# wzx99/DCFP

Measured on AMD Instinct MI355X. Metric: training images/sec at 1024x2048 DeepLabv3-R101, higher is better.
Workload: dtype f32; 1 GPU; DeepLabv3-resnet101+ASPP os8, 4x3x1024x2048 per GPU, CE+0.4*deepsup CE (fused upsample), 3x3 stride-1 convs with >= 256 channels as fp32 Winograd F(2x2,3x3) (fwd / dgrad / wgrad), all other convs direct implicit GEMM, EIC step, SGD m0.9 wd5e-4; global_batch=4, parallelism=dp1

## Files before the change

### dcfp_amd/_lib.py

```python
import ctypes as C
import os
import subprocess
import threading

_HERE = os.path.dirname(os.path.abspath(__file__))
LIB_PATH = os.environ.get("DCFP_LIB") or os.path.join(_HERE, "libdcfp_hip.so")
CSRC = os.path.join(_HERE, "csrc")

_lib = None
_lock = threading.Lock()


class ConvDesc(C.Structure):
    _fields_ = [(n, C.c_int32) for n in
                ("N", "Cin", "H", "W", "Cout", "KH", "KW", "stride", "pad", "dil", "Hout", "Wout",
                 "x_pitch", "dy_pitch")]


class ConvF16Desc(C.Structure):
    _fields_ = [(n, C.c_int32) for n in
                ("N", "H", "W", "Cin8", "x_pitch", "Cout", "K", "stride", "pad", "dil", "Hout", "Wout",
                 "y_pitch", "y_off", "res_pitch", "res_off", "relu")]


class EicEntry(C.Structure):
    _fields_ = [("gamma", C.c_void_p), ("grad", C.c_void_p), ("eic", C.c_void_p),
                ("n", C.c_int32), ("pad_", C.c_int32)]


class SgdEntry(C.Structure):
    _fields_ = [("param", C.c_void_p), ("grad", C.c_void_p), ("momentum_buf", C.c_void_p),
                ("n", C.c_int64), ("first_chunk", C.c_int64),
                ("weight_decay", C.c_float), ("pad_", C.c_int32)]


class BnRunning(C.Structure):
    _fields_ = [("running_mean", C.c_void_p), ("running_var", C.c_void_p), ("num_batches_tracked", C.c_void_p),
                ("momentum", C.c_float), ("pad_", C.c_int32)]


class WpEntry(C.Structure):
    _fields_ = [("w", C.c_void_p), ("wp", C.c_void_p), ("first_block", C.c_int64), ("n_blocks", C.c_int64)] + \
               [(n, C.c_int32) for n in ("T", "Ck", "CkP", "M", "Mpad", "sAm", "sAc", "perm8")]


class AugTap(C.Structure):
    _fields_ = [(n, C.c_int32) for n in ("src", "c0", "c1", "lsrc")]


class AugSample(C.Structure):
    _fields_ = [("image", C.c_void_p), ("label", C.c_void_p)] + \
               [(n, C.c_int32) for n in ("src_h", "src_w", "col_off", "row_off", "lut_a_off", "lut_b_off",
                                         "hsv_flags", "hue_delta")] + \
               [("sat_alpha", C.c_float), ("pad_", C.c_int32)]


class CcSample(C.Structure):
    _fields_ = [("label", C.c_void_p)] + \
               [(n, C.c_int32) for n in ("src_h", "src_w", "dst_h", "dst_w", "Hp", "Wp", "row_off", "col_off", "cls",
                                         "pad_")] + \
               [("work_off", C.c_int64)]


AUG_SATURATION, AUG_HUE = 1, 2
SGD_CHUNK = 16384
CONV_FWD, CONV_DGRAD, CONV_WGRAD = 0, 1, 2
E_BADDESC, E_UNSUPPORTED, E_WORKSPACE = -1, -2, -3

_P, _I, _L, _F, _Z = C.c_void_p, C.c_int, C.c_int64, C.c_float, C.c_size_t
_D = C.POINTER(ConvDesc)
_R = C.POINTER(BnRunning)
_H = C.POINTER(ConvF16Desc)

SIGNATURES = {
    "dcfp_abi_version": (_I, []),
    "dcfp_conv2d_workspace_bytes": (_Z, [_D, _I]),
    "dcfp_conv2d_wp_layout": (_I, [_D, _I, C.POINTER(WpEntry)]),
    "dcfp_conv2d_permute_weights_multi_f32": (_I, [_P, _I, _L, _P]),
    "dcfp_conv2d_pitch_supported": (_I, [_D]),
    "dcfp_conv2d_kernel_name": (_I, [_D, _I, C.c_char_p, _I]),
    "dcfp_conv2d_executed_fraction": (C.c_double, [_D, _I]),
    "dcfp_conv2d_workspace_is_scratch": (_I, [_D, _I]),
    "dcfp_conv2d_dgrad_fanin_supported": (_I, [_D]),
    "dcfp_conv2d_dgrad_fanin_f32_nchw": (_I, [_D, _P, _L, _P, _P, _P, _P, _P, _Z, _I, _P]),
    "dcfp_conv2d_dgrad_fanin_red_slots": (_L, [_D]),
    "dcfp_conv2d_dgrad_fanin_red_f32_nchw": (_I, [_D, _P, _L, _P, _P, _P, _P, _P, _P, _P, _P, _P, _Z, _I, _P]),
    "dcfp_bn_bwd_sums_from_partials_f32": (_I, [_P, _L, _I, _P, _F, _P, _P, _P, _P, _P]),
    "dcfp_conv2d_xform_bytes": (_Z, [_D]),
    "dcfp_conv2d_fwd_keep_f32_nchw": (_I, [_D, _P, _P, _P, _L, _P, _Z, _P, _P, _Z, _P]),
    "dcfp_conv2d_wgrad_kept_f32_nchw": (_I, [_D, _P, _L, _P, _Z, _P, _P, _Z, _P]),
    "dcfp_conv2d_fwd_f32_nchw": (_I, [_D, _P, _P, _P, _P, _L, _P, _Z, _I, _P]),
    "dcfp_conv2d_fwd_fused_f32_nchw": (_I, [_D, _P, _P, _P, _P, _P, _I, _P, _P, _Z, _I, _P]),
    "dcfp_conv2d_dgrad_f32_nchw": (_I, [_D, _P, _L, _P, _P, _I, _P, _Z, _I, _P]),
    "dcfp_conv2d_wgrad_f32_nchw": (_I, [_D, _P, _L, _P, _P, _P, _P, _Z, _P]),
    "dcfp_bn_workspace_bytes": (_Z, [_I, _I, _I]),
    "dcfp_bn_stats_f32": (_I, [_P, _L, _I, _I, _I, _P, _P, _R, _P, _Z, _P]),
    "dcfp_bn_apply_f32": (_I, [_P, _P, _P, _P, _P, _F, _P, _I, _P, _L, _I, _I, _I, _I, _I, _P]),
    "dcfp_bn_bwd_reduce_f32": (_I, [_P, _L, _P, _P, _L, _P, _P, _P, _P, _F, _I, _I, _I, _I, _P, _P, _P, _P,
                                    _P, _Z, _P]),
    "dcfp_bn_update_running_f32": (_I, [_P, _P, _I, _F, _F, _P, _P, _P, _P]),
    "dcfp_syncbn_combine_f32": (_I, [_P, _I, _I, _P, _P, _P, _R, _P]),
    "dcfp_syncbn_p2p_mailbox_bytes": (_Z, [_I, _I]),
    "dcfp_p2p_alloc": (_I, [_Z, _I, C.POINTER(C.c_void_p)]),
    "dcfp_p2p_free": (_I, [_P]),
    "dcfp_p2p_export": (_I, [_P, _P]),
    "dcfp_p2p_import": (_I, [_P, C.POINTER(C.c_void_p)]),
    "dcfp_p2p_unmap": (_I, [_P]),
    "dcfp_syncbn_p2p_exchange_f32": (_I, [C.POINTER(C.c_void_p), _I, _I, C.c_uint32, _I, _P, _I, _I, _P, _R,
                                          C.c_uint32, _P, _P]),
    "dcfp_bn_apply_relu_mask_f32": (_I, [_P, _P, _P, _P, _P, _F, _P, _P, _P, _I, _I, _I, _P]),
    "dcfp_conv2d_fwd_stat_slots": (_L, [_D, _P, _L]),
    "dcfp_conv2d_fwd_stats_f32_nchw": (_I, [_D, _P, _P, _P, _L, _P, _P, _Z, _I, _P]),
    "dcfp_bn_stats_from_partials_f32": (_I, [_P, _L, _I, _I, _P, _P, _R, _P]),
    "dcfp_bn_bwd_apply_f32": (_I, [_P, _L, _P, _P, _L, _P, _P, _P, _P, _F, _P, _P, _F, _P, _I, _P, _P,
                                   _I, _I, _I, _I, _I, _P]),
    "dcfp_bn_bwd_fused_sync_bytes": (_Z, [_I, _I, _I]),
    "dcfp_bn_bwd_fused_f32": (_I, [_P, _L, _P, _P, _L, _P, _P, _P, _P, _F, _F, _I, _P, _P, _I, _I, _I, _I, _I,
                                   _P, _P, _P, _P, _P, _Z, C.c_uint32, C.c_uint32, _P, _P]),
    "dcfp_maxpool3x3s2_fwd_f32": (_I, [_P, _P, _P, _I, _I, _I, _I, _I, _I, _P]),
    "dcfp_maxpool3x3s2_bwd_f32": (_I, [_P, _P, _P, _I, _I, _I, _I, _I, _I, _P]),
    "dcfp_rowsum_f32": (_I, [_P, _L, _P, _F, _I, _I, _I, _P]),
    "dcfp_broadcast_hw_f32": (_I, [_P, _F, _P, _L, _I, _I, _I, _I, _P]),
    "dcfp_add_f32": (_I, [_P, _P, _P, _L, _P]),
    "dcfp_channel_scale_f32": (_I, [_P, _P, _P, _I, _I, _I, _P]),
    "dcfp_upsample_bilinear_fwd_f32": (_I, [_P, _P, _I, _I, _I, _I, _I, _I, _I, _P]),
    "dcfp_upsample_bilinear_bwd_f32": (_I, [_P, _P, _I, _I, _I, _I, _I, _I, _I, _P]),
    "dcfp_resize_bilinear_into_f32": (_I, [_P, _L, _I, _I, _I, _I, _P, _L, _I, _I, _I, _I, _P]),
    "dcfp_resize_bilinear_adjoint_f32": (_I, [_P, _L, _I, _I, _I, _I, _I, _P, _L, _I, _I, _I, _I, _P]),
    "dcfp_ppm_pool_f32": (_I, [_P, _I, _I, _I, _I, _I, _P, _P, _I, _P, _L, _I, _P]),
    "dcfp_ppm_pool_adjoint_f32": (_I, [_P, _I, _I, _I, _I, _I, _P, _P, _L, _I, _P, _P]),
    "dcfp_ppm_resize_adjoint_f32": (_I, [_P, _L, _I, _I, _I, _I, _I, _P, _P, _I, _P]),
    "dcfp_upsample_ce_workspace_bytes": (_Z, [_I, _I, _I]),
    "dcfp_upsample_ce_fwd_f32": (_I, [_P, _P, _P, _I, _I, _I, _I, _I, _I, _I, _I, _P, _P, _P, _P,
                                      _Z, _P]),
    "dcfp_upsample_ce_bwd_f32": (_I, [_P, _P, _P, _I, _I, _I, _I, _I, _I, _I, _I, _P, _P, _P, _P]),
    "dcfp_ohem_zoom_gt_prob_f32": (_I, [_P, _P, _P, _I, _I, _I, _I, _I, _I, _I, _I, _I, _P, _P, _P]),
    "dcfp_ohem_threshold_f32": (_I, [_P, _P, _L, _I, _F, _L, _P, _P]),
    "dcfp_ohem_keep_mask_u8": (_I, [_P, _P, _L, _P, _P]),
    "dcfp_upsample_margin_f32": (_I, [_P, _I, _I, _I, _I, _I, _I, _I, _P, _P]),
    "dcfp_maxfilter2d_s1_f32": (_I, [_P, _P, _I, _I, _I, _I, _P]),
    "dcfp_upsample_wce_workspace_bytes": (_Z, [_I, _I, _I]),
    "dcfp_upsample_wce_fwd_f32": (_I, [_P, _P, _P, _I, _I, _I, _I, _I, _I, _I, _I, _P, _P, _P, _Z, _P]),
    "dcfp_upsample_wce_bwd_f32": (_I, [_P, _P, _P, _I, _I, _I, _I, _I, _I, _I, _I, _P, _P, _P, _P]),
    "dcfp_upsample_argmax_f32": (_I, [_P, _I, _I, _I, _I, _I, _I, _I, _P, _P]),
    "dcfp_confusion_matrix_i64": (_I, [_P, _P, _I, _L, _I, _P, _P]),
    "dcfp_label_boundary_workspace_bytes": (_Z, [_I, _I, _I]),
    "dcfp_label_boundary_i32": (_I, [_P, _P, _I, _I, _I, _I, _I, _I, _P, _Z, _P]),
    "dcfp_label_boundary_i64": (_I, [_P, _P, _I, _I, _I, _I, _I, _I, _P, _Z, _P]),
    "dcfp_augment_u8_to_f32_nchw": (_I, [C.POINTER(AugSample), _I, _I, _I, _P, _L, _P, _L, _P, _L, _P, _I, _P, _P, _P, _P]),
    "dcfp_balance_weight_f32": (_I, [_P, _P, _P, _I, _L, _I, _I, _I, C.c_double, _P, _P]),
    "dcfp_components_workspace_bytes": (_Z, [_I, _I]),
    "dcfp_label_components_u8": (_I, [C.POINTER(CcSample), _I, _P, _L, _P, _P, _Z, _P, _P]),
    "dcfp_component_pixel_i32": (_I, [C.POINTER(CcSample), _I, _P, _Z, _P, _P, _P, _P, _P]),
    "dcfp_eic_update_f32": (_I, [_P, _I, _F, _F, _P]),
    "dcfp_sgd_momentum_f32": (_I, [_P, _I, _L, _F, _F, _I, _P]),
    "dcfp_conv2d_fwd_f16_nhwc": (_I, [_H, _P, _P, _P, _P, _P, _P]),
    "dcfp_conv2d_fwd_f16_nhwc_to_f32_nchw": (_I, [_H, _P, _P, _P, _P, _P]),
    "dcfp_maxpool3x3s2_nhwc_f16": (_I, [_P, _P, _I, _I, _I, _I, _I, _I, _I, _I, _P]),
    "dcfp_avgpool_nhwc_f16_workspace_bytes": (_Z, [_I, _I, _L]),
    "dcfp_avgpool_nhwc_f16": (_I, [_P, _P, _I, _L, _I, _I, _I, _P, _Z, _P]),
    "dcfp_broadcast_nhwc_f16": (_I, [_P, _I, _P, _I, _L, _I, _I, _I, _P]),
    "dcfp_nchw_f32_to_nhwc_f16": (_I, [_P, _P, _I, _I, _I, _I, _I, _P]),
    "dcfp_resize_bilinear_nhwc_f16": (_I, [_P, _I, _I, _I, _I, _I, _P, _I, _I, _I, _I, _I, _P]),
    "dcfp_pyramid_pool_nhwc_f16_workspace_bytes": (_Z, [_I, _I, _I, _I, _I, _P]),
    "dcfp_pyramid_pool_nhwc_f16": (_I, [_P, _I, _I, _I, _I, _I, _I, _I, _P, _P, _P, _P, _Z, _P]),
}


def build(verbose=False):
    cmd = ["make", "-C", CSRC, "-j", str(min(8, os.cpu_count() or 1))]
    r = subprocess.run(cmd, capture_output=True, text=True)
    if verbose or r.returncode != 0:
        print(r.stdout[-4000:])
        print(r.stderr[-4000:])
    if r.returncode != 0:
        raise RuntimeError("building libdcfp_hip.so failed")
    return LIB_PATH


def lib():
    global _lib
    if _lib is not None:
        return _lib
    with _lock:
        if _lib is not None:
            return _lib
        if not os.path.exists(LIB_PATH):
            raise RuntimeError(
                f"{LIB_PATH} not found: run `python -c 'import __graft_entry__ as g; g.build()'` "
                "(or `make -C dcfp_amd/csrc`). dcfp_amd has no non-HIP fallback.")
        try:
            import torch
        except Exception:
            pass
        handle = C.CDLL(LIB_PATH, mode=C.RTLD_GLOBAL)
        for name, (res, args) in SIGNATURES.items():
            fn = getattr(handle, name)
            fn.restype = res
            fn.argtypes = args
        _lib = handle
    return _lib


def check(status, what):
    if status != 0:
        kind = "descriptor/shape" if status < 0 else "hipError_t"
        raise RuntimeError(f"{what} failed: status {status} ({kind})")
```

### dcfp_amd/csrc/bn.hip

```cpp
#include "common.h"
#include <stdlib.h>

namespace {

constexpr int kThreads = 256;

__device__ __forceinline__ float bn_val(float v, float mu, float istd, float g, float b) {
    return fmaf((v - mu) * istd, g, b);
}

struct BnPlan {
    int chunks;
    int chunk_elems;
};

constexpr int kChunkElems = 8192;

BnPlan bn_plan(int N, int C, int HW) {
    const long long E = (long long)N * HW;
    long long chunks = (E + kChunkElems - 1) / kChunkElems;
    if (E <= kChunkElems) {
        const long long by_size = (E + 2047) / 2048;
        long long by_grid = 4096 / (C > 0 ? C : 1);
        if (by_grid < 1) by_grid = 1;
        chunks = by_size < by_grid ? by_size : by_grid;
    }
    if (chunks < 1) chunks = 1;
    long long ce = (E + chunks - 1) / chunks;
    ce = (ce + 1023) / 1024 * 1024;
    chunks = (E + ce - 1) / ce;
    if (chunks < 1) chunks = 1;
    BnPlan p;
    p.chunks = (int)chunks;
    p.chunk_elems = (int)ce;
    return p;
}

__device__ __forceinline__ void bwd_accumulate(const float4& g, const float4& xv, float mu, float& s1, float& s2) {
#pragma clang fp contract(off)
    s1 += (g.x + g.y) + (g.z + g.w);
    const float a = fmaf(g.x, xv.x - mu, g.y * (xv.y - mu));
    const float b = fmaf(g.z, xv.z - mu, g.w * (xv.w - mu));
    s2 += a + b;
}
__device__ __forceinline__ float bwd_dx(float g, float xv, float mu, float mean_dy, float k, float gi) {
#pragma clang fp contract(off)
    return fmaf(-(xv - mu), k, g - mean_dy) * gi;
}

template <bool VEC>
__global__ void __launch_bounds__(kThreads)
bn_stats_partial_kernel(const float* __restrict__ x, long long nstride, int HW, long long E,
                        int chunk_elems, int chunks, float* __restrict__ part) {
    __shared__ float red[4];
    const int c = blockIdx.y, chunk = blockIdx.x;
    const float* xc = x + (long long)c * HW;
    const float K = xc[0];
    const long long e0 = (long long)chunk * chunk_elems;
    long long e1 = e0 + chunk_elems;
    if (e1 > E) e1 = E;
    float s1 = 0.f, s2 = 0.f;
    if (VEC) {
        for (long long e = e0 + 4 * threadIdx.x; e < e1; e += 4 * kThreads) {
            const long long n = e / HW;
            const int i = (int)(e - n * HW);
            const float4 v = *reinterpret_cast<const float4*>(xc + n * nstride + i);
            const float a = v.x - K, b = v.y - K, cc = v.z - K, d = v.w - K;
            s1 += (a + b) + (cc + d);
            s2 += (a * a + b * b) + (cc * cc + d * d);
        }
    } else {
        for (long long e = e0 + threadIdx.x; e < e1; e += kThreads) {
            const long long n = e / HW;
            const int i = (int)(e - n * HW);
            const float a = xc[n * nstride + i] - K;
            s1 += a;
            s2 += a * a;
        }
    }
    const float t1 = block_sum_256(s1, red);
    const float t2 = block_sum_256(s2, red);
    if (threadIdx.x == 0) {
        part[((long long)c * chunks + chunk) * 2 + 0] = t1;
        part[((long long)c * chunks + chunk) * 2 + 1] = t2;
    }
}

__global__ void bn_stats_final_kernel(const float* __restrict__ x, int HW, long long E, int C,
                                      int chunks, const float* __restrict__ part,
                                      float* __restrict__ mean, float* __restrict__ var, DcfpBnRunning run) {
    const int c = blockIdx.x * blockDim.x + threadIdx.x;
    if (c >= C) return;
    double S1 = 0.0, S2 = 0.0;
    for (int k = 0; k < chunks; ++k) {
        S1 += (double)part[((long long)c * chunks + k) * 2 + 0];
        S2 += (double)part[((long long)c * chunks + k) * 2 + 1];
    }
    const double K = (double)x[(long long)c * HW];
    const double m1 = S1 / (double)E;
    double v = S2 / (double)E - m1 * m1;
    if (v < 0.0) v = 0.0;
    mean[c] = (float)(K + m1);
    var[c] = (float)v;
    running_update(run, c, (float)(K + m1), (float)v, (float)E);
}

__device__ __forceinline__ bool mask_bit(const unsigned long long* __restrict__ row_words, int i_wave, int k) {
    const unsigned long long wv = row_words[(i_wave >> 8) * 4 + k];
    return (wv >> (threadIdx.x & 63)) & 1ull;
}

template <bool VEC, bool MASK = false>
__global__ void __launch_bounds__(kThreads)
bn_apply_kernel(const float* __restrict__ x, const float* __restrict__ mean,
                const float* __restrict__ var, const float* __restrict__ gamma,
                const float* __restrict__ beta, float eps, const float* __restrict__ res,
                int relu, float* __restrict__ y, long long y_nstride, int C, int HW,
                int colchunks, int cols_per_block, unsigned long long* __restrict__ mask = nullptr,
                int W = 0, int y_pitch = 0) {
    const long long row = blockIdx.x / colchunks;
    const int chunk = blockIdx.x - (int)(row * colchunks);
    const int n = (int)(row / C), c = (int)(row - (long long)n * C);
    const float istd = 1.0f / sqrtf(var[c] + eps);
    const float mu = mean[c], g = gamma[c], b = beta[c];
    const float* xr = x + row * HW;
    const float* rr = res ? res + row * HW : nullptr;
    float* yr = y + (long long)n * y_nstride + (long long)c * (y_pitch ? (long long)(HW / W) * y_pitch : HW);
    const int i0 = chunk * cols_per_block;
    int i1 = i0 + cols_per_block;
    if (i1 > HW) i1 = HW;
    if (VEC) {
        for (int i = i0 + 4 * threadIdx.x; i < i1; i += 4 * kThreads) {
            const float4 v = *reinterpret_cast<const float4*>(xr + i);
            float4 o;
            o.x = bn_val(v.x, mu, istd, g, b);
            o.y = bn_val(v.y, mu, istd, g, b);
            o.z = bn_val(v.z, mu, istd, g, b);
            o.w = bn_val(v.w, mu, istd, g, b);
            if (rr) {
                const float4 r = *reinterpret_cast<const float4*>(rr + i);
                o.x += r.x; o.y += r.y; o.z += r.z; o.w += r.w;
            }
            if (relu) {
                o.x = o.x > 0.f ? o.x : 0.f; o.y = o.y > 0.f ? o.y : 0.f;
                o.z = o.z > 0.f ? o.z : 0.f; o.w = o.w > 0.f ? o.w : 0.f;
            }
            if constexpr (MASK) {
                const unsigned long long b0 = __ballot(o.x > 0.f), b1 = __ballot(o.y > 0.f);
                const unsigned long long b2 = __ballot(o.z > 0.f), b3 = __ballot(o.w > 0.f);
                if ((threadIdx.x & 63) == 0) {
                    unsigned long long* mw = mask + row * (HW >> 6) + (i >> 8) * 4;
                    mw[0] = b0; mw[1] = b1; mw[2] = b2; mw[3] = b3;
                }
            }
            if (y_pitch) { const int h = i / W; *reinterpret_cast<float4*>(yr + h * y_pitch + (i - h * W)) = o; }
            else *reinterpret_cast<float4*>(yr + i) = o;
        }
    } else {
        for (int i = i0 + threadIdx.x; i < i1; i += kThreads) {
            float o = bn_val(xr[i], mu, istd, g, b);
            if (rr) o += rr[i];
            if (relu) o = o > 0.f ? o : 0.f;
            if (y_pitch) { const int h = i / W; yr[h * y_pitch + (i - h * W)] = o; }
            else yr[i] = o;
        }
    }
}

template <bool VEC, int RELU>
__global__ void __launch_bounds__(kThreads)
bn_bwd_reduce_partial_kernel(const float* __restrict__ dy, long long dy_nstride,
                             const float* __restrict__ x, const float* __restrict__ y,
                             long long y_nstride, const float* __restrict__ mean,
                             const float* __restrict__ var, const float* __restrict__ gamma,
                             const float* __restrict__ beta, float eps, int C, int HW,
                             long long E, int chunk_elems, int chunks, float* __restrict__ part) {
    __shared__ float red[4];
    const int c = blockIdx.y, chunk = blockIdx.x;
    const float mu = mean[c];
    float istd = 0.f, gm = 0.f, bt = 0.f;
    if (RELU == 2) { istd = 1.0f / sqrtf(var[c] + eps); gm = gamma[c]; bt = beta[c]; }
    const long long e0 = (long long)chunk * chunk_elems;
    long long e1 = e0 + chunk_elems;
    if (e1 > E) e1 = E;
    const long long coff = (long long)c * HW;
    const long long x_nstride = (long long)C * HW;
    float s1 = 0.f, s2 = 0.f;
    if (VEC) {
        for (long long e = e0 + 4 * threadIdx.x; e < e1; e += 4 * kThreads) {
            const long long n = e / HW;
            const int i = (int)(e - n * HW);
            float4 g = *reinterpret_cast<const float4*>(dy + n * dy_nstride + coff + i);
            const float4 xv = *reinterpret_cast<const float4*>(x + n * x_nstride + coff + i);
            if (RELU == 1) {
                const float4 yv = *reinterpret_cast<const float4*>(y + n * y_nstride + coff + i);
                g.x = yv.x > 0.f ? g.x : 0.f; g.y = yv.y > 0.f ? g.y : 0.f;
                g.z = yv.z > 0.f ? g.z : 0.f; g.w = yv.w > 0.f ? g.w : 0.f;
            } else if (RELU == 2) {
                g.x = bn_val(xv.x, mu, istd, gm, bt) > 0.f ? g.x : 0.f;
                g.y = bn_val(xv.y, mu, istd, gm, bt) > 0.f ? g.y : 0.f;
                g.z = bn_val(xv.z, mu, istd, gm, bt) > 0.f ? g.z : 0.f;
                g.w = bn_val(xv.w, mu, istd, gm, bt) > 0.f ? g.w : 0.f;
            } else if (RELU == 3) {
                const unsigned long long* mw = reinterpret_cast<const unsigned long long*>(y) +
                                               (n * C + c) * (long long)(HW >> 6);
                const int iw = i - 4 * (int)(threadIdx.x & 63);
                g.x = mask_bit(mw, iw, 0) ? g.x : 0.f; g.y = mask_bit(mw, iw, 1) ? g.y : 0.f;
                g.z = mask_bit(mw, iw, 2) ? g.z : 0.f; g.w = mask_bit(mw, iw, 3) ? g.w : 0.f;
            }
            bwd_accumulate(g, xv, mu, s1, s2);
        }
    } else {
        for (long long e = e0 + threadIdx.x; e < e1; e += kThreads) {
            const long long n = e / HW;
            const int i = (int)(e - n * HW);
            float g = dy[n * dy_nstride + coff + i];
            const float xv = x[n * x_nstride + coff + i];
            if (RELU == 1) g = y[n * y_nstride + coff + i] > 0.f ? g : 0.f;
            else if (RELU == 2) g = bn_val(xv, mu, istd, gm, bt) > 0.f ? g : 0.f;
            s1 += g;
            s2 += g * (xv - mu);
        }
    }
    const float t1 = block_sum_256(s1, red);
    const float t2 = block_sum_256(s2, red);
    if (threadIdx.x == 0) {
        part[((long long)c * chunks + chunk) * 2 + 0] = t1;
        part[((long long)c * chunks + chunk) * 2 + 1] = t2;
    }
}

template <class F>
__device__ __forceinline__ double wave_pair_totals(int n2, int lane, F value_of) {
    double acc = 0.0;
    for (int j = 0; lane + 64 * j < n2; ++j) acc += (double)value_of(j);
#pragma unroll
    for (int off = 2; off < 64; off <<= 1) acc += __shfl_xor(acc, off, 64);
    return acc;
}

__global__ void __launch_bounds__(64) bn_pair_final_kernel(int C, int chunks, const float* __restrict__ part,
                                     float* __restrict__ o1, float* __restrict__ o2,
                                     const float* __restrict__ var, float eps, float* __restrict__ o3,
                                     float* __restrict__ o4) {
    const int c = blockIdx.x, lane = threadIdx.x;
    const float* pc = part + (long long)c * chunks * 2;
    const double t = wave_pair_totals(2 * chunks, lane, [&](int j) { return pc[lane + 64 * j]; });
    const double S1 = __shfl(t, 0, 64), S2 = __shfl(t, 1, 64);
    if (lane == 0) {
        o1[c] = (float)S1;
        o2[c] = (float)S2;
        if (o3) o3[c] = (float)S2 * rsqrtf(var[c] + eps);
        if (o4) o4[c] = (float)S1;
    }
}

__global__ void syncbn_combine_kernel(const float* __restrict__ allv, int world, int C,
                                      float* __restrict__ gmean, float* __restrict__ gvar,
                                      float* __restrict__ total, DcfpBnRunning run) {
#pragma clang fp contract(off)
    const int c = blockIdx.x * blockDim.x + threadIdx.x;
    if (c >= C) return;
    const int S = 2 * C + 1;
    double tot = 0.0, m = 0.0, v = 0.0;
    for (int r = 0; r < world; ++r) {
        const double n = (double)allv[(long long)r * S + 2 * C];
        tot = __dadd_rn(tot, n);
        m = __dadd_rn(m, __dmul_rn((double)allv[(long long)r * S + c], n));
    }
    m /= tot;
    for (int r = 0; r < world; ++r) {
        const double n = (double)allv[(long long)r * S + 2 * C];
        const double d = __dadd_rn((double)allv[(long long)r * S + c], -m);
        v = __dadd_rn(v, __dmul_rn(__dadd_rn((double)allv[(long long)r * S + C + c], __dmul_rn(d, d)), n));
    }
    gmean[c] = (float)m;
    gvar[c] = (float)(v / tot);
    if (c == 0) total[0] = (float)tot;
    running_update(run, c, (float)m, (float)(v / tot), (float)tot);
}

constexpr int kSfpThreads = 1024;
template <int kSfpCh>
__global__ void __launch_bounds__(kSfpThreads)
bn_stats_from_partials_kernel(const float* __restrict__ part, long long S, int cnt, int C,
                              float* __restrict__ mean, float* __restrict__ var, DcfpBnRunning run) {
    constexpr int kSfpGroups = kSfpThreads / kSfpCh;
    __shared__ double red[kSfpGroups][kSfpCh];
    __shared__ double mu_s[kSfpCh];
    const int l = threadIdx.x % kSfpCh, g = threadIdx.x / kSfpCh;
    const int c = blockIdx.x * kSfpCh + l;
    const bool on = c < C;
    const float2* p2 = reinterpret_cast<const float2*>(part);
    constexpr int U = 4;
    double a[U] = {0.0, 0.0, 0.0, 0.0};
    if (on) {
        long long s = g;
        for (; s + (U - 1) * kSfpGroups < S; s += U * kSfpGroups) {
            float v[U];
#pragma unroll
            for (int u = 0; u < U; ++u) v[u] = p2[(s + u * kSfpGroups) * C + c].x;
#pragma unroll
            for (int u = 0; u < U; ++u) a[u] += (double)v[u];
        }
        for (; s < S; s += kSfpGroups) a[0] += (double)p2[s * C + c].x;
    }
    red[g][l] = (a[0] + a[1]) + (a[2] + a[3]);
    __syncthreads();
    if (g == 0) {
        double t = 0.0;
#pragma unroll
        for (int k = 0; k < kSfpGroups; ++k) t += red[k][l];
        mu_s[l] = t / (double)S;
    }
    __syncthreads();
    const double mu = mu_s[l];
    double b[U] = {0.0, 0.0, 0.0, 0.0};
    if (on) {
        long long s = g;
// ... 307 lines not shown
}

template <int RELU, bool DRES, bool PITCH>
__global__ void __launch_bounds__(kThreads, 5) bn_bwd_fusedu_kernel(const BnFusedParams p) {
    __shared__ float red[4];
    __shared__ float tot[2];
    __shared__ int failed;
    __shared__ float parts[2 * kFusedMaxChunks];
    const int c = blockIdx.x / p.chunks, chunk = blockIdx.x - c * p.chunks;
    const int HW = p.HW, C = p.C;
    const float mu = p.mean[c];
    const float istd = 1.0f / sqrtf(p.var[c] + p.eps);
    const float gm = p.gamma[c];
    const float bt = RELU == 2 ? p.beta[c] : 0.f;
    const int e0 = chunk * kChunkElems;
    const int n = e0 / HW, i0 = e0 - n * HW;
    const long long row = (long long)n * C + c;
    const float* dyb = p.dy + (long long)n * p.dy_nstride + (long long)c * HW + i0;
    const float* xb = p.x + row * HW + i0;
    const unsigned lo = 4u * threadIdx.x;
    if (threadIdx.x == 0) failed = 0;

    float4 g[kFusedIters], xv[kFusedIters];
#pragma unroll
    for (int k = 0; k < kFusedIters; ++k) {
        g[k] = *reinterpret_cast<const float4*>(dyb + 4 * kThreads * k + lo);
        xv[k] = *reinterpret_cast<const float4*>(xb + 4 * kThreads * k + lo);
    }
    float s1 = 0.f, s2 = 0.f;
#pragma unroll
    for (int k = 0; k < kFusedIters; ++k) {
        if (RELU == 1) {
            const float4 yv = *reinterpret_cast<const float4*>(p.y + (long long)n * p.y_nstride + (long long)c * HW + i0 +
                                                               4 * kThreads * k + lo);
            g[k].x = yv.x > 0.f ? g[k].x : 0.f; g[k].y = yv.y > 0.f ? g[k].y : 0.f;
            g[k].z = yv.z > 0.f ? g[k].z : 0.f; g[k].w = yv.w > 0.f ? g[k].w : 0.f;
        } else if (RELU == 2) {
            g[k].x = bn_val(xv[k].x, mu, istd, gm, bt) > 0.f ? g[k].x : 0.f;
            g[k].y = bn_val(xv[k].y, mu, istd, gm, bt) > 0.f ? g[k].y : 0.f;
            g[k].z = bn_val(xv[k].z, mu, istd, gm, bt) > 0.f ? g[k].z : 0.f;
            g[k].w = bn_val(xv[k].w, mu, istd, gm, bt) > 0.f ? g[k].w : 0.f;
        } else if (RELU == 3) {
            const unsigned long long* mw = reinterpret_cast<const unsigned long long*>(p.y) + row * (long long)(HW >> 6) +
                                           ((i0 + 4 * kThreads * k + 256 * (int)(threadIdx.x >> 6)) >> 8) * 4;
            const int sh = (int)(threadIdx.x & 63);
            g[k].x = ((mw[0] >> sh) & 1ull) ? g[k].x : 0.f; g[k].y = ((mw[1] >> sh) & 1ull) ? g[k].y : 0.f;
            g[k].z = ((mw[2] >> sh) & 1ull) ? g[k].z : 0.f; g[k].w = ((mw[3] >> sh) & 1ull) ? g[k].w : 0.f;
        }
        bwd_accumulate(g[k], xv[k], mu, s1, s2);
    }
    const float t1 = block_sum_256(s1, red);
    const float t2 = block_sum_256(s2, red);
    bn_fused_handoff(p, c, chunk, t1, t2, tot, &failed, parts);
    const bool bad = failed != 0;
    const float S1f = tot[0], S2f = tot[1];
    const float nanv = __uint_as_float(0x7fc00000u);
    if (chunk == 0 && threadIdx.x == 0) {
        p.sum_dy[c] = bad ? nanv : S1f;
        p.sum_dy_xmu[c] = bad ? nanv : S2f;
        if (p.dgamma) p.dgamma[c] = bad ? nanv : S2f * rsqrtf(p.var[c] + p.eps);
        if (p.dbeta) p.dbeta[c] = bad ? nanv : S1f;
    }
    const float mean_dy = S1f * p.inv_count;
    const float kk = S2f * p.inv_count * istd * istd;
    const float gi = bad ? nanv : gm * istd;
    float* dxb = p.dx + row * (PITCH ? (long long)(HW / p.W) * p.dx_pitch : (long long)HW) + (PITCH ? 0 : i0);
    float* drb = DRES ? p.dres + row * HW + i0 : nullptr;
#pragma unroll
    for (int k = 0; k < kFusedIters; ++k) {
        float4 o;
        o.x = bwd_dx(g[k].x, xv[k].x, mu, mean_dy, kk, gi);
        o.y = bwd_dx(g[k].y, xv[k].y, mu, mean_dy, kk, gi);
        o.z = bwd_dx(g[k].z, xv[k].z, mu, mean_dy, kk, gi);
        o.w = bwd_dx(g[k].w, xv[k].w, mu, mean_dy, kk, gi);
        if (PITCH) {
            const int i = i0 + 4 * kThreads * k + (int)lo;
            const int h = i / p.W;
            *reinterpret_cast<float4*>(dxb + h * p.dx_pitch + (i - h * p.W)) = o;
        } else {
            *reinterpret_cast<float4*>(dxb + 4 * kThreads * k + lo) = o;
        }
        if (DRES) *reinterpret_cast<float4*>(drb + 4 * kThreads * k + lo) = g[k];
    }
}

static const int kColsPerBlock = [] { const char* e = getenv("DCFP_BN_COLS"); const int v = e ? atoi(e) : 2048; return v >= 1024 && v % 1024 == 0 ? v : 2048; }();

}

extern "C" size_t dcfp_bn_workspace_bytes(int N, int C, int HW) {
    if (N <= 0 || C <= 0 || HW <= 0) return 0;
    const BnPlan p = bn_plan(N, C, HW);
    return (size_t)C * p.chunks * 2 * sizeof(float);
}

static int run_arg(const DcfpBnRunning* run, DcfpBnRunning* out) {
    DcfpBnRunning none = {nullptr, nullptr, nullptr, 0.f, 0};
    *out = run ? *run : none;
    if (out->running_mean && !out->running_var) return DCFP_E_BADDESC;
    return DCFP_OK;
}

extern "C" int dcfp_bn_stats_f32(const float* x, int64_t x_nstride, int N, int C, int HW,
                                 float* mean, float* var, const DcfpBnRunning* run, void* workspace,
                                 size_t workspace_bytes, dcfp_stream_t stream) {
    if (!x || !mean || !var || N <= 0 || C <= 0 || HW <= 0) return DCFP_E_BADDESC;
    DcfpBnRunning rn;
    if (run_arg(run, &rn)) return DCFP_E_BADDESC;
    if (x_nstride == 0) x_nstride = (int64_t)C * HW;
    const BnPlan p = bn_plan(N, C, HW);
    if (!workspace || workspace_bytes < (size_t)C * p.chunks * 2 * sizeof(float))
        return DCFP_E_WORKSPACE;
    float* part = static_cast<float*>(workspace);
    const long long E = (long long)N * HW;
    const bool vec = (HW % 4 == 0) && (x_nstride % 4 == 0) && dcfp_aligned16(x);
    dim3 grid(p.chunks, C);
    if (vec)
        hipLaunchKernelGGL(bn_stats_partial_kernel<true>, grid, dim3(kThreads), 0, dcfp_s(stream), x,
                           (long long)x_nstride, HW, E, p.chunk_elems, p.chunks, part);
    else
        hipLaunchKernelGGL(bn_stats_partial_kernel<false>, grid, dim3(kThreads), 0, dcfp_s(stream),
                           x, (long long)x_nstride, HW, E, p.chunk_elems, p.chunks, part);
    hipLaunchKernelGGL(bn_stats_final_kernel, dim3((C + 255) / 256), dim3(256), 0, dcfp_s(stream),
                       x, HW, E, C, p.chunks, part, mean, var, rn);
    DCFP_RETURN_LAUNCH();
}

extern "C" int dcfp_bn_apply_f32(const float* x, const float* mean, const float* var,
                                 const float* gamma, const float* beta, float eps,
                                 const float* residual, int relu, float* y, int64_t y_nstride,
                                 int N, int C, int HW, int W, int y_pitch, dcfp_stream_t stream) {
    if (!x || !mean || !var || !gamma || !beta || !y || N <= 0 || C <= 0 || HW <= 0)
        return DCFP_E_BADDESC;
    if (y_pitch && (W <= 0 || HW % W != 0 || y_pitch < W)) return DCFP_E_BADDESC;
    if (y_pitch == W) y_pitch = 0;
    if (y_nstride == 0) y_nstride = (int64_t)C * (y_pitch ? (int64_t)(HW / W) * y_pitch : HW);
    const int colchunks = (HW + kColsPerBlock - 1) / kColsPerBlock;
    const long long blocks = (long long)N * C * colchunks;
    if (blocks > 0x7fffffffLL) return DCFP_E_UNSUPPORTED;
    const bool vec = (HW % 4 == 0) && (y_nstride % 4 == 0) && dcfp_aligned16(x) &&
                     dcfp_aligned16(y) && (!residual || dcfp_aligned16(residual)) &&
                     (!y_pitch || (W % 4 == 0 && y_pitch % 4 == 0));
    if (vec)
        hipLaunchKernelGGL(bn_apply_kernel<true>, dim3((unsigned)blocks), dim3(kThreads), 0,
                           dcfp_s(stream), x, mean, var, gamma, beta, eps, residual, relu, y,
                           (long long)y_nstride, C, HW, colchunks, kColsPerBlock, nullptr, W, y_pitch);
    else
        hipLaunchKernelGGL(bn_apply_kernel<false>, dim3((unsigned)blocks), dim3(kThreads), 0,
                           dcfp_s(stream), x, mean, var, gamma, beta, eps, residual, relu, y,
                           (long long)y_nstride, C, HW, colchunks, kColsPerBlock, nullptr, W, y_pitch);
    DCFP_RETURN_LAUNCH();
}

extern "C" int dcfp_bn_apply_relu_mask_f32(const float* x, const float* mean, const float* var,
                                           const float* gamma, const float* beta, float eps,
                                           const float* residual, float* y, void* relu_mask,
                                           int N, int C, int HW, dcfp_stream_t stream) {
    if (!x || !mean || !var || !gamma || !beta || !y || !relu_mask || N <= 0 || C <= 0 || HW <= 0)
        return DCFP_E_BADDESC;
    const bool vec = dcfp_aligned16(x) && dcfp_aligned16(y) && (!residual || dcfp_aligned16(residual));
    if (!vec || HW % 256 != 0 || (reinterpret_cast<uintptr_t>(relu_mask) & 7u)) return DCFP_E_UNSUPPORTED;
    const int colchunks = (HW + kColsPerBlock - 1) / kColsPerBlock;
    const long long blocks = (long long)N * C * colchunks;
    if (blocks > 0x7fffffffLL) return DCFP_E_UNSUPPORTED;
    hipLaunchKernelGGL((bn_apply_kernel<true, true>), dim3((unsigned)blocks), dim3(kThreads), 0, dcfp_s(stream),
                       x, mean, var, gamma, beta, eps, residual, 1, y, (long long)C * HW, C, HW, colchunks,
                       kColsPerBlock, static_cast<unsigned long long*>(relu_mask));
    DCFP_RETURN_LAUNCH();
}

extern "C" int dcfp_bn_bwd_reduce_f32(const float* dy, int64_t dy_nstride, const float* x,
                                      const float* y, int64_t y_nstride, const float* mean,
                                      const float* var, const float* gamma, const float* beta,
                                      float eps, int relu, int N, int C, int HW, float* sum_dy,
                                      float* sum_dy_xmu, float* dgamma, float* dbeta, void* workspace,
                                      size_t workspace_bytes, dcfp_stream_t stream) {
    if (dgamma && !var) return DCFP_E_BADDESC;
    if (!dy || !x || !mean || !sum_dy || !sum_dy_xmu || N <= 0 || C <= 0 || HW <= 0)
        return DCFP_E_BADDESC;
    if (relu < 0 || relu > 3) return DCFP_E_BADDESC;
    if ((relu == 1 || relu == 3) && !y) return DCFP_E_BADDESC;
    if (relu == 2 && (!var || !gamma || !beta)) return DCFP_E_BADDESC;
    if (dy_nstride == 0) dy_nstride = (int64_t)C * HW;
    if (y_nstride == 0) y_nstride = (int64_t)C * HW;
    const BnPlan p = bn_plan(N, C, HW);
    if (!workspace || workspace_bytes < (size_t)C * p.chunks * 2 * sizeof(float))
        return DCFP_E_WORKSPACE;
    float* part = static_cast<float*>(workspace);
    const long long E = (long long)N * HW;
    const bool vec = (HW % 4 == 0) && (dy_nstride % 4 == 0) && (y_nstride % 4 == 0) &&
                     dcfp_aligned16(dy) && dcfp_aligned16(x) && (relu != 1 || dcfp_aligned16(y));
    dim3 grid(p.chunks, C);
#define LAUNCH_RED(V, R)                                                                          \
    hipLaunchKernelGGL((bn_bwd_reduce_partial_kernel<V, R>), grid, dim3(kThreads), 0,             \
                       dcfp_s(stream), dy, (long long)dy_nstride, x, y, (long long)y_nstride,     \
                       mean, var, gamma, beta, eps, C, HW, E, p.chunk_elems, p.chunks, part)
    if (relu == 3 && !(vec && HW % 256 == 0 && dy_nstride == (int64_t)C * HW)) return DCFP_E_UNSUPPORTED;
    if (vec) { if (relu == 3) LAUNCH_RED(true, 3); else if (relu == 2) LAUNCH_RED(true, 2); else if (relu == 1) LAUNCH_RED(true, 1); else LAUNCH_RED(true, 0); }
    else     { if (relu == 2) LAUNCH_RED(false, 2); else if (relu == 1) LAUNCH_RED(false, 1); else LAUNCH_RED(false, 0); }
#undef LAUNCH_RED
    hipLaunchKernelGGL(bn_pair_final_kernel, dim3((unsigned)C), dim3(64), 0, dcfp_s(stream), C,
                       p.chunks, part, sum_dy, sum_dy_xmu, var, eps, dgamma, dbeta);
    DCFP_RETURN_LAUNCH();
}

extern "C" int dcfp_bn_update_running_f32(const float* mean, const float* var, int C, float momentum,
                                          float count, const float* count_dev, float* running_mean,
                                          float* running_var, dcfp_stream_t stream) {
    if (!mean || !var || !running_mean || !running_var || C <= 0 || (!count_dev && !(count > 0.f)))
        return DCFP_E_BADDESC;
    hipLaunchKernelGGL(bn_running_kernel, dim3((C + 255) / 256), dim3(256), 0, dcfp_s(stream), C, mean,
                       var, momentum, count, count_dev, running_mean, running_var);
    DCFP_RETURN_LAUNCH();
}

extern "C" int dcfp_bn_bwd_apply_f32(const float* dy, int64_t dy_nstride, const float* x,
                                     const float* y, int64_t y_nstride, const float* mean,
                                     const float* var, const float* gamma, const float* beta,
                                     float eps, const float* sum_dy, const float* sum_dy_xmu,
                                     float count, const float* count_dev, int relu, float* dx,
                                     float* d_residual, int N, int C, int HW, int W, int dx_pitch,
                                     dcfp_stream_t stream) {
    if (!dy || !x || !mean || !var || !gamma || !sum_dy || !sum_dy_xmu || !dx || N <= 0 ||
        C <= 0 || HW <= 0 || (!count_dev && !(count > 0.f)))
        return DCFP_E_BADDESC;
    if (relu < 0 || relu > 3 || ((relu == 1 || relu == 3) && !y) || (relu == 2 && !beta)) return DCFP_E_BADDESC;
    if (dx_pitch && (W <= 0 || HW % W != 0 || dx_pitch < W)) return DCFP_E_BADDESC;
    if (dx_pitch == W) dx_pitch = 0;
    if (dy_nstride == 0) dy_nstride = (int64_t)C * HW;
    if (y_nstride == 0) y_nstride = (int64_t)C * HW;
    const int colchunks = (HW + kColsPerBlock - 1) / kColsPerBlock;
    const long long blocks = (long long)N * C * colchunks;
    if (blocks > 0x7fffffffLL) return DCFP_E_UNSUPPORTED;
    const bool vec = (HW % 4 == 0) && (dy_nstride % 4 == 0) && (y_nstride % 4 == 0) &&
                     dcfp_aligned16(dy) && dcfp_aligned16(x) && dcfp_aligned16(dx) &&
                     (relu != 1 || dcfp_aligned16(y)) && (!d_residual || dcfp_aligned16(d_residual)) &&
                     (!dx_pitch || (W % 4 == 0 && dx_pitch % 4 == 0));
    const float inv_count = count > 0.f ? 1.0f / count : 0.f;
#define LAUNCH_APP(V, R)                                                                          \
    hipLaunchKernelGGL((bn_bwd_apply_kernel<V, R>), dim3((unsigned)blocks), dim3(kThreads), 0,    \
                       dcfp_s(stream), dy, (long long)dy_nstride, x, y, (long long)y_nstride,     \
                       mean, var, gamma, beta, eps, sum_dy, sum_dy_xmu, inv_count, count_dev, dx, \
                       d_residual, C,                                                             \
                       HW, colchunks, kColsPerBlock, W, dx_pitch)
    if (relu == 3 && !(vec && HW % 256 == 0)) return DCFP_E_UNSUPPORTED;
    if (vec) { if (relu == 3) LAUNCH_APP(true, 3); else if (relu == 2) LAUNCH_APP(true, 2); else if (relu == 1) LAUNCH_APP(true, 1); else LAUNCH_APP(true, 0); }
    else     { if (relu == 2) LAUNCH_APP(false, 2); else if (relu == 1) LAUNCH_APP(false, 1); else LAUNCH_APP(false, 0); }
#undef LAUNCH_APP
    DCFP_RETURN_LAUNCH();
}

extern "C" size_t dcfp_bn_bwd_fused_sync_bytes(int N, int C, int HW) {
    if (N <= 0 || C <= 0 || HW <= 0 || HW % 4 != 0) return 0;
    const long long E = (long long)N * HW;
    if (E >= 0x7fffffffLL - kChunkElems) return 0;
    const BnPlan p = bn_plan(N, C, HW);
    if (p.chunks > kFusedMaxChunks || p.chunk_elems > kChunkElems) return 0;
    if ((long long)C * p.chunks > 0x7fffffffLL) return 0;
    return (size_t)C * (p.chunks * 2 + 2) * sizeof(unsigned long long);
}

extern "C" int dcfp_bn_bwd_fused_f32(const float* dy, int64_t dy_nstride, const float* x, const float* y,
                                     int64_t y_nstride, const float* mean, const float* var, const float* gamma,
                                     const float* beta, float eps, float count, int relu, float* dx, float* d_residual,
                                     int N, int C, int HW, int W, int dx_pitch, float* sum_dy, float* sum_dy_xmu,
                                     float* dgamma, float* dbeta, void* sync, size_t sync_bytes, uint32_t epoch,
                                     uint32_t spin_limit, int32_t* status, dcfp_stream_t stream) {
    if (!dy || !x || !mean || !var || !gamma || !dx || !sum_dy || !sum_dy_xmu || !sync || N <= 0 || C <= 0 || HW <= 0 ||
        !(count > 0.f) || epoch == 0)
        return DCFP_E_BADDESC;
    if (relu < 0 || relu > 3 || ((relu == 1 || relu == 3) && !y) || (relu == 2 && !beta)) return DCFP_E_BADDESC;
    if (dx_pitch && (W <= 0 || HW % W != 0 || dx_pitch < W)) return DCFP_E_BADDESC;
    if (dx_pitch == W) dx_pitch = 0;
    if (dy_nstride == 0) dy_nstride = (int64_t)C * HW;
    if (y_nstride == 0) y_nstride = (int64_t)C * HW;
    const size_t need = dcfp_bn_bwd_fused_sync_bytes(N, C, HW);
    if (need == 0) return DCFP_E_UNSUPPORTED;
    if (sync_bytes < need || (reinterpret_cast<uintptr_t>(sync) & 7u)) return DCFP_E_WORKSPACE;
    const bool vec = (dy_nstride % 4 == 0) && (y_nstride % 4 == 0) && dcfp_aligned16(dy) && dcfp_aligned16(x) &&
                     dcfp_aligned16(dx) && (relu != 1 || dcfp_aligned16(y)) &&
                     (!d_residual || dcfp_aligned16(d_residual)) && (!dx_pitch || (W % 4 == 0 && dx_pitch % 4 == 0));
    if (!vec) return DCFP_E_UNSUPPORTED;
    if (relu == 3 && !(HW % 256 == 0 && dy_nstride == (int64_t)C * HW)) return DCFP_E_UNSUPPORTED;
    const BnPlan pl = bn_plan(N, C, HW);
    BnFusedParams p;
    p.dy = dy; p.dy_nstride = dy_nstride; p.x = x; p.y = y; p.y_nstride = y_nstride;
    p.mean = mean; p.var = var; p.gamma = gamma; p.beta = beta; p.eps = eps; p.inv_count = 1.0f / count;
    p.dx = dx; p.dres = d_residual; p.C = C; p.HW = HW; p.E = (int)((long long)N * HW);
    p.chunk_elems = pl.chunk_elems; p.chunks = pl.chunks; p.W = W; p.dx_pitch = dx_pitch;
    p.sync = static_cast<unsigned long long*>(sync); p.epoch = epoch;
    p.spin_limit = spin_limit ? spin_limit : (1u << 18); p.status = status;
    p.sum_dy = sum_dy; p.sum_dy_xmu = sum_dy_xmu; p.dgamma = dgamma; p.dbeta = dbeta;
    const size_t lds = 0;
    const dim3 grid((unsigned)((long long)C * pl.chunks));
    static const bool uni_on = [] { const char* e = getenv("DCFP_BN_FUSED_UNI"); return !e || atoi(e) != 0; }();
    if (uni_on && pl.chunk_elems == kChunkElems && HW % kChunkElems == 0) {
#define LAUNCH_FUSEDU2(R, D, P) hipLaunchKernelGGL((bn_bwd_fusedu_kernel<R, D, P>), grid, dim3(kThreads), lds, dcfp_s(stream), p)
#define LAUNCH_FUSEDU(R)                                                                                       \
    do {                                                                                                       \
        if (d_residual) { if (dx_pitch) LAUNCH_FUSEDU2(R, true, true); else LAUNCH_FUSEDU2(R, true, false); }  \
        else { if (dx_pitch) LAUNCH_FUSEDU2(R, false, true); else LAUNCH_FUSEDU2(R, false, false); }           \
    } while (0)
        if (relu == 3) LAUNCH_FUSEDU(3); else if (relu == 2) LAUNCH_FUSEDU(2); else if (relu == 1) LAUNCH_FUSEDU(1); else LAUNCH_FUSEDU(0);
#undef LAUNCH_FUSEDU
#undef LAUNCH_FUSEDU2
        DCFP_RETURN_LAUNCH();
// ... 43 lines not shown
```

### dcfp_amd/csrc/conv_igemm2.hip

```cpp
#include "igemm2_common.h"
#include <queue>
#include <vector>
#include <stdio.h>
#include <stdlib.h>

namespace {

__device__ __forceinline__ int wp_row(int m, int perm8) {
    if (!perm8) return m;
    const int j = m & 255;
    return (m & ~255) + 32 * (j & 7) + (j >> 3);
}

__global__ void __launch_bounds__(256)
permute_weights_kernel(const float* __restrict__ w, float* __restrict__ wp, int T, int Ck, int CkP,
                       int M, int Mpad, int sAm, int sAc, int perm8) {
    const long long total = (long long)T * CkP * Mpad;
    for (long long i = (long long)blockIdx.x * 256 + threadIdx.x; i < total;
         i += (long long)gridDim.x * 256) {
        const int m = wp_row((int)(i % Mpad), perm8);
        const long long r = i / Mpad;
        const int c = (int)(r % CkP);
        const int t = (int)(r / CkP);
        float v = 0.f;
        if (m < M && c < Ck) v = w[(long long)m * sAm + (long long)c * sAc + t];
        wp[i] = v;
    }
}

constexpr int kWpBlockElems = DCFP_WP_BLOCK_ELEMS;
__global__ void __launch_bounds__(256)
permute_weights_multi_kernel(const DcfpWpEntry* __restrict__ table, int n) {
    const long long blk = blockIdx.x;
    int lo = 0, hi = n - 1;
    while (lo < hi) {
        const int mid = (lo + hi + 1) >> 1;
        if (table[mid].first_block <= blk) lo = mid; else hi = mid - 1;
    }
    const DcfpWpEntry e = table[lo];
    const long long base = (blk - e.first_block) * kWpBlockElems;
    if (e.perm8 >= 2) {
        const long long pairs = (long long)e.CkP * e.Mpad;
#pragma unroll 1
        for (int u = 0; u < kWpBlockElems / 256; ++u) {
            const long long i = base + u * 256 + threadIdx.x;
            if (i >= pairs) return;
            wino_filter2_pair(e.w, e.sAm, e.sAc, e.perm8 == 3, e.M, e.Ck, e.Mpad, i, e.wp);
        }
        return;
    }
    const long long total = (long long)e.T * e.CkP * e.Mpad;
#pragma unroll
    for (int u = 0; u < kWpBlockElems / 256; ++u) {
        const long long i = base + u * 256 + threadIdx.x;
        if (i >= total) return;
        const int m = wp_row((int)(i % e.Mpad), e.perm8);
        const long long r = i / e.Mpad;
        const int c = (int)(r % e.CkP);
        const int t = (int)(r / e.CkP);
        float v = 0.f;
        if (m < e.M && c < e.Ck) v = e.w[(long long)m * e.sAm + (long long)c * e.sAc + t];
        e.wp[i] = v;
    }
}

__device__ __forceinline__ float half_xor(float v, int mask) {
    switch (mask) {
        case 1: return __builtin_bit_cast(float, __builtin_amdgcn_ds_swizzle(__builtin_bit_cast(int, v), (1 << 10) | 0x1f));
        case 2: return __builtin_bit_cast(float, __builtin_amdgcn_ds_swizzle(__builtin_bit_cast(int, v), (2 << 10) | 0x1f));
        case 4: return __builtin_bit_cast(float, __builtin_amdgcn_ds_swizzle(__builtin_bit_cast(int, v), (4 << 10) | 0x1f));
        case 8: return __builtin_bit_cast(float, __builtin_amdgcn_ds_swizzle(__builtin_bit_cast(int, v), (8 << 10) | 0x1f));
        default: return __builtin_bit_cast(float, __builtin_amdgcn_ds_swizzle(__builtin_bit_cast(int, v), (16 << 10) | 0x1f));
    }
}

template <int TAPS, int TM, int TN, int WM, int WN, bool SD, bool ACC, int KB = 16>
__global__ void __launch_bounds__(64 * WM * WN, (TM * TN <= 8 && WM * WN == 4 && !ACC) ? 2 : 1)
igemm2_kernel(const Igemm2Params p) {
    constexpr int BK = KB;
    constexpr int NPART = BK / 4;
    constexpr int BM = WM * TM * 32, BN = WN * TN * 32, NT = 64 * WM * WN;
    constexpr int AX = BM / 4;
    constexpr int AROWS = (NT / AX) < BK ? (NT / AX) : BK;
    constexpr int APASS = BK / AROWS;
    constexpr int TX = BN / 4, TY = NT / TX, RPT = BK / TY;
    static_assert(APASS >= 1 && APASS * AROWS == BK, "A loader shape");
    static_assert(TY >= 1 && RPT >= 1 && TY * RPT == BK, "B loader shape");

    extern __shared__ __attribute__((aligned(16))) float smem[];
    float* As = smem;
    float* Bs = smem + 2 * BK * BM;

    const int group = 8 * p.tiles_m;
    const int g = blockIdx.x / group, local = blockIdx.x - g * group;
    const int nt = g * 8 + (local & 7);
    const int mt = local >> 3;
    if (nt >= p.tiles_n_total) return;
    const int img = nt / p.tiles_per_img;
    const int ti_img = nt - img * p.tiles_per_img;
    const int phase = SD ? (p.zfold ? p.zfold - 1 : ti_img / p.tiles_per_phase) : 0;
    const int ph_h = SD ? phase / p.sd : 0, ph_w = SD ? phase - ph_h * p.sd : 0;
    const int p0 = (SD && !p.zfold ? ti_img - phase * p.tiles_per_phase : ti_img) * BN;
    const int m0 = mt * BM;

    const int tid = threadIdx.x;
    const int lane = tid & 63, wid = tid >> 6;
    const int wm = wid / WN, wn = wid - wm * WN;
    const int l31 = lane & 31, lhi = lane >> 5;

    const int ax = tid % AX, ay = tid / AX;
    const bool a_on = ay < BK;
    const float* a_src = p.wp + m0 + 4 * ax;

    const int tx = tid % TX, ty = tid / TX;
    int bh[4], bw[4];
    bool pv[4];
#pragma unroll
    for (int e = 0; e < 4; ++e) {
        const int pp = p0 + 4 * tx + e;
        if constexpr (SD) {
            const int a = pp / p.Wc, b = pp - a * p.Wc;
            const int oh = a * p.sd + ph_h, ow = b * p.sd + ph_w;
            pv[e] = a < p.Hc && oh < p.Ho && ow < p.Wo;
            bh[e] = oh * p.sn;
            bw[e] = ow * p.sn;
        } else {
            pv[e] = pp < p.P;
            const int oh = pp / p.Wo;
            const int ow = pp - oh * p.Wo;
            bh[e] = oh * p.sn;
            bw[e] = ow * p.sn;
        }
    }
    const int HiWi = p.Hi * p.Wi;
    const __amdgpu_buffer_rsrc_t b_rsrc = __builtin_amdgcn_make_buffer_rsrc(
        const_cast<float*>(p.in + (long long)img * p.in_nstride), 0, p.Ck * HiWi * 4, 0x00020000);

    const int ksteps_per_tap = p.CkP / BK;
    unsigned long long tap_list = 0;
    int ntaps = TAPS;
    if constexpr (SD) {
        ntaps = 0;
        for (int t = 0; t < TAPS; ++t) {
            const int kh = (TAPS == 9) ? t / 3 : 0, kw = (TAPS == 9) ? t - kh * 3 : 0;
            const int sh = ph_h + p.off0 + kh * p.offstep, sw = ph_w + p.off0 + kw * p.offstep;
            if (sh % p.sd == 0 && sw % p.sd == 0) {
                tap_list |= (unsigned long long)t << (4 * ntaps);
                ++ntaps;
            }
        }
    }
    const int nk = ntaps * ksteps_per_tap;

    unsigned boff[4];
    bool bvec = false;
    f32x4 areg[APASS];
    float breg[RPT][4];

    auto set_tap = [&](int t) {
        const int kh = (TAPS == 9) ? t / 3 : 0;
        const int kw = (TAPS == 9) ? t - kh * 3 : 0;
        const int offh = p.off0 + kh * p.offstep;
        const int offw = p.off0 + kw * p.offstep;
#pragma unroll
        for (int e = 0; e < 4; ++e) {
            int hh = bh[e] + offh, ww = bw[e] + offw;
            bool ok = pv[e] && hh >= 0 && ww >= 0;
            if (SD) {
                ok = ok && (hh % p.sd == 0) && (ww % p.sd == 0);
                hh /= p.sd;
                ww /= p.sd;
            }
            ok = ok && hh < p.Hi && ww < p.Wi;
            boff[e] = ok ? (unsigned)(hh * p.Wi + ww) * 4u : kOob;
        }
        const bool none = boff[0] == kOob && boff[1] == kOob && boff[2] == kOob && boff[3] == kOob;
        const bool run = boff[0] != kOob && boff[1] == boff[0] + 4u && boff[2] == boff[0] + 8u &&
                         boff[3] == boff[0] + 12u;
        bvec = none || run;
    };
    auto load_part = [&](int kt, auto part_) {
        constexpr int PART = decltype(part_)::value;
#ifdef DCFP_TAP_INNER
        const int cb = kt / TAPS;
        const int t = kt - cb * TAPS;
        const int c0 = cb * BK;
        if (PART == 0 && (TAPS > 1 || kt == 0)) set_tap(t);
#else
        const int ti_ = kt / ksteps_per_tap;
        const int c0 = (kt - ti_ * ksteps_per_tap) * BK;
        const int t = SD ? (int)((tap_list >> (4 * ti_)) & 15ull) : ti_;
        if (PART == 0 && c0 == 0) set_tap(t);
#endif
        static_for<0, APASS>([&](auto j_) {
            constexpr int j = decltype(j_)::value;
            if constexpr ((j % NPART) == PART) {
                if (a_on)
                    areg[j] = *reinterpret_cast<const f32x4*>(
                        a_src + (long long)(t * p.CkP + c0 + ay + AROWS * j) * p.Mpad);
            }
        });
        static_for<0, RPT>([&](auto q_) {
            constexpr int q = decltype(q_)::value;
            if constexpr ((q % NPART) == PART) {
                int c = c0 + ty + TY * q;
                c = c < p.Ck ? c : p.Ck - 1;
                const unsigned coff = (unsigned)(c * HiWi) * 4u;
                if (bvec) {
                    const f32x4 v = __builtin_bit_cast(
                        f32x4, __builtin_amdgcn_raw_buffer_load_b128(b_rsrc, boff[0] + coff, 0, 0));
                    static_for<0, 4>([&](auto e_) {
                        constexpr int e = decltype(e_)::value;
                        breg[q][e] = v[e];
                    });
                } else {
// ... 915 lines not shown
```

### dcfp_amd/csrc/conv_wgrad.hip

```cpp
#include "common.h"
#include <stdio.h>
#include <stdlib.h>
#include <string.h>
#include <type_traits>

int dcfp_wgrad3_launch(const float* dy, long long dy_nstride, const float* x, long long x_nstride,
                       float* out, int N, int M, int Cin, int T, int H, int W, int Ho, int Wo, int pad,
                       int dil, int Kpix, int kchunk, int splits, int tiles_m, int tiles_n,
                       hipStream_t stream);

namespace {

typedef float f32x16 __attribute__((ext_vector_type(16)));

constexpr int BK = 16;
constexpr int BKP = 20;

struct WgradParams {
    const float* dy;
    const float* x;
    float* out;
    long long dy_nstride, x_nstride;
    int N, M, Cin, Nn;
    int H, W, Ho, Wo, P, stride, pad, dil;
// ... 768 lines not shown

static bool wgrad_dma_ok(const DcfpConvDesc* d, int cfg) {
    static const bool on = [] { const char* e = getenv("DCFP_WGRAD_DMA"); return !e || atoi(e) != 0; }();
    static const bool mixed_too = [] { const char* e = getenv("DCFP_WGRAD_DMA_MIXED"); return !e || atoi(e) != 0; }();
    const bool mixed = d->KH == 3 && ((d->pad | d->dil) & 3) != 0;
    return on && cfg == 0 && d->stride == 1 && d->Hout == d->H && d->Wout == d->W && d->W % 16 == 0 &&
           (!mixed || mixed_too);
}
static bool wgrad_dma_mixed(const DcfpConvDesc* d) { return d->KH == 3 && ((d->pad | d->dil) & 3) != 0; }

template <int TAPS, bool MIXED, bool WIDE = false, bool BATCH = false, bool HALF = false>
int launch_dma(const WgradParams& p, long long blocks, hipStream_t stream) {
    const size_t lds = (size_t)2 * (HALF ? 384 : 512) * BK * sizeof(float);
    hipLaunchKernelGGL((wgrad_dma_kernel<TAPS, MIXED, WIDE, BATCH, HALF>), dim3((unsigned)blocks), dim3(256), lds, stream, p);
    hipError_t e = hipGetLastError();
    return e == hipSuccess ? DCFP_OK : (int)e;
}

template <int TAPS>
int launch_taps(const WgradParams& p, const Plan& pl, hipStream_t stream) {
    const long long blocks = (long long)pl.tiles_m * pl.tiles_n * pl.splits;
    if (blocks > 0x7fffffffLL) return DCFP_E_UNSUPPORTED;
    switch (pl.cfg) {
        case 0: return launch_cfg<TAPS, 4, 4, 2, 2>(p, blocks, stream);
        case 1: return launch_cfg<TAPS, 2, 4, 2, 2>(p, blocks, stream);
        case 3: return launch_cfg<TAPS, 4, 2, 2, 2>(p, blocks, stream);
        case 4: return launch_cfg<TAPS, 4, 1, 2, 2>(p, blocks, stream);
        case 5: return launch_cfg<TAPS, 2, 3, 2, 2>(p, blocks, stream);
        default: return launch_cfg<TAPS, 2, 2, 1, 1>(p, blocks, stream);
    }
}

}

bool dcfp_gemv_shape(const DcfpConvDesc* d);
bool dcfp_stem_shape(const DcfpConvDesc* d);
size_t dcfp_stem_wgrad_workspace_bytes(const DcfpConvDesc* d);
int dcfp_stem_wgrad(const DcfpConvDesc* d, const float* dy, long long dy_nstride, const float* x, float* dw, void* workspace,
                    size_t workspace_bytes, hipStream_t stream);
int dcfp_gemv_wgrad(const DcfpConvDesc* d, const float* dy, long long dy_nstride, const float* x, float* dw, hipStream_t stream);

bool dcfp_wgrad_pitch_ok(const DcfpConvDesc* d) {
    if (check_desc(d) != DCFP_OK) return false;
    const Plan pl = make_plan(d);
    if (wgrad3_ok(d, pl.cfg)) return false;
    const int xp = d->x_pitch ? d->x_pitch : d->W;
    if (xp != d->W && (d->KH != 3 || d->pad != d->dil || xp < d->W + d->pad)) return false;
    return true;
}

size_t dcfp_wgrad_batched_workspace_bytes(int batch, int M, int C, long long K, int* splits_out) {
    const long long tiles = (long long)((M + 255) / 256) * ((C + 255) / 256) * batch;
    const long long slots = num_cus();
    long long max_splits = K / (BK * 8);
    if (max_splits < 1) max_splits = 1;
    long long splits = 1;
    double best = -1.0;
    for (long long sp = 1; sp <= max_splits && tiles * sp <= 4 * slots; ++sp) {
        const long long blocks = tiles * sp, rounds = (blocks + slots - 1) / slots;
        double eff = (double)blocks / (double)(rounds * slots);
        if (blocks < slots) eff *= 0.999;
        if (eff > best + 0.02) { best = eff; splits = sp; }
    }
    long long kchunk = (K + splits - 1) / splits;
    kchunk = (kchunk + BK - 1) / BK * BK;
    splits = (K + kchunk - 1) / kchunk;
    if (splits_out) *splits_out = (int)splits;
    return splits > 1 ? (size_t)splits * batch * M * C * sizeof(float) : 0;
}

int dcfp_wgrad_batched_run(const float* a, const float* bmat, float* out, int batch, int M, int C, long long K,
                           void* workspace, size_t workspace_bytes, hipStream_t stream) {
    if (K % BK != 0 || K <= 0 || K >= (1LL << 30) || (long long)M * K >= (1LL << 29) || (long long)C * K >= (1LL << 29))
        return DCFP_E_UNSUPPORTED;
    int splits = 1;
    const size_t need = dcfp_wgrad_batched_workspace_bytes(batch, M, C, K, &splits);
    if (need && (!workspace || workspace_bytes < need || !dcfp_aligned16(workspace))) return DCFP_E_WORKSPACE;
    WgradParams p;
    p.dy = a; p.x = bmat;
    p.out = splits > 1 ? static_cast<float*>(workspace) : out;
    p.x_pitch = (int)K; p.dy_pitch = (int)K;
    p.dy_nstride = (long long)M * K; p.x_nstride = (long long)C * K;
    p.N = 1; p.M = M; p.Cin = C; p.Nn = C;
    p.H = 1; p.W = (int)K; p.Ho = 1; p.Wo = (int)K; p.P = (int)K;
    p.stride = 1; p.pad = 0; p.dil = 1;
    p.Kpix = (int)K;
    long long kchunk = (K + splits - 1) / splits;
    kchunk = (kchunk + BK - 1) / BK * BK;
    p.kchunk = (int)kchunk; p.splits = splits;
    p.tiles_m = (M + 255) / 256; p.tiles_n = (C + 255) / 256;
    p.quad_ok = 1;
    p.batch = batch; p.dy_bstride = (long long)M * K; p.x_bstride = (long long)C * K;
    const long long blocks = (long long)p.tiles_m * p.tiles_n * splits * batch;
    if (blocks > 0x7fffffffLL) return DCFP_E_UNSUPPORTED;
    const long long mp = (long long)p.tiles_m * 256, live = (long long)((M + 31) / 32) * 32;
    int rc = (M % 256 != 0 && 10 * live <= 9 * mp) ? launch_dma<1, false, true, true>(p, blocks, stream)
                                                   : launch_dma<1, false, false, true>(p, blocks, stream);
    if (rc) return rc;
    if (splits > 1) {
        const long long wn = (long long)batch * M * C;
        if (wn % 4 == 0 && dcfp_aligned16(out)) {
            const long long n4 = wn / 4;
            hipLaunchKernelGGL(splitk_reduce_vec4_kernel, dim3((unsigned)((n4 + 255) / 256)), dim3(256), 0, stream,
                               static_cast<const float*>(workspace), out, n4, wn, splits);
        } else {
            long long b = (wn + 255) / 256;
            if (b > 4096) b = 4096;
            hipLaunchKernelGGL(splitk_reduce_kernel, dim3((unsigned)b), dim3(256), 0, stream,
                               static_cast<const float*>(workspace), out, wn, splits);
        }
    }
    DCFP_RETURN_LAUNCH();
}

static bool wino_wgrad_pass(const DcfpConvDesc* d);
static int wino_wgrad_kind(const DcfpConvDesc* d);

int dcfp_wgrad_kernel_name(const DcfpConvDesc* d, char* buf, int buf_len) {
    if (dcfp_stem_shape(d)) return snprintf(buf, buf_len, "stem_wgrad_kernel");
    if (const int wk = wino_wgrad_kind(d))
        return wk == 2 ? snprintf(buf, buf_len, "winograd_f2x2_3x3 wgrad fused (wino_wgrad_fused_kernel)")
                       : snprintf(buf, buf_len, "winograd_f2x2_3x3 wgrad (wgrad_dma_kernel<1,false,false,true>)");
    const Plan pl = make_plan(d);
    const char* args = pl.cfg == 0 ? "4,4,2,2" : pl.cfg == 1 ? "2,4,2,2" : pl.cfg == 3 ? "4,2,2,2" :
                       pl.cfg == 4 ? "4,1,2,2" : pl.cfg == 5 ? "2,3,2,2" : "2,2,1,1";
    if (wgrad3_ok(d, pl.cfg)) return snprintf(buf, buf_len, "wgrad3_kernel<%d>", d->KH * d->KW);
    if (pl.wide) return snprintf(buf, buf_len, "wgrad_dma_kernel<%d,false,true>", d->KH * d->KW);
    if (wgrad_dma_ok(d, pl.cfg))
        return snprintf(buf, buf_len, "wgrad_dma_kernel<%d,%s>", d->KH * d->KW,
                        (wgrad_dma_mixed(d) && !(d->x_pitch && d->x_pitch != d->W)) ? "true" : "false");
    return snprintf(buf, buf_len, "wgrad2_kernel<%d,%s>", d->KH * d->KW, args);
}

bool dcfp_wino_wgrad_ok(int N, int H, int W, int d, int M, int C);
size_t dcfp_wino_wgrad_workspace_bytes(int N, int H, int W, int d, int M, int C);
double dcfp_wino_exec_fraction(int N, int H, int W, int d, int M, int Ck);
int dcfp_wino_wgrad_run(const float* dy, long long dy_nstride, int dy_pitch, const float* x, long long x_nstride,
                        int x_pitch, float* dw, int N, int M, int C, int H, int W, int d, void* workspace,
                        size_t workspace_bytes, hipStream_t stream, const float* xform_in = nullptr);
extern "C" size_t dcfp_conv2d_xform_bytes(const DcfpConvDesc* d);

static double wino_wgrad_fused_rate() {
    static const double v = [] { const char* e = getenv("DCFP_WINO_WGRAD_RATE"); return (e ? atof(e) : 118.0) * 1e12; }();
    return v;
}
static bool wino_wgrad_fused_forced() {
    static const bool v = [] { const char* e = getenv("DCFP_WINO_WGRAD_FUSED"); return e && atoi(e) == 2; }();
    return v;
}

bool dcfp_wino_wgrad_fused_ok(int N, int H, int W, int d, int M, int C, long long x_nstride, int x_pitch,
                              long long dy_nstride, int dy_pitch);
size_t dcfp_wino_wgrad_fused_workspace_bytes(int N, int H, int W, int d, int M, int C);
int dcfp_wino_wgrad_fused_run(const float* dy, long long dy_nstride, int dy_pitch, const float* x, long long x_nstride,
                              int x_pitch, float* dw, int N, int M, int C, int H, int W, int d, void* workspace,
                              size_t workspace_bytes, hipStream_t stream);

static int wino_wgrad_kind(const DcfpConvDesc* d) {
    static const int mode = [] { const char* e = getenv("DCFP_CONV_WINOGRAD"); return e ? atoi(e) : 1; }();
    if (mode == 0) return 0;
    if (d->KH != 3 || d->KW != 3 || d->stride != 1 || d->pad != d->dil || d->Hout != d->H || d->Wout != d->W) return 0;
    if (math_bf16x3()) return 0;
    const int xp = d->x_pitch ? d->x_pitch : d->W, dyp = d->dy_pitch ? d->dy_pitch : d->Wout;
    const bool batched = dcfp_wino_wgrad_ok(d->N, d->H, d->W, d->dil, d->Cout, d->Cin);
    const bool fused = dcfp_wino_wgrad_fused_ok(d->N, d->H, d->W, d->dil, d->Cout, d->Cin, (long long)d->Cin * d->H * xp, xp,
                                                (long long)d->Cout * d->Hout * dyp, dyp);
    if (!batched && !fused) return 0;
    if (mode == 2) return fused ? 2 : 1;
    const double pix = (double)d->N * d->H * d->W;
    const double nominal = 2.0 * pix * d->Cout * (double)d->Cin * 9.0;
    const bool dense_d1 = wgrad_dma_mixed(d) && !(d->x_pitch && d->x_pitch != d->W);
    const bool ragged = d->Cout % 256 != 0 || (d->Cin * 9) % 256 != 0;
    const double dpad = ragged ? (double)((d->Cout + 31) / 32 * 32) / d->Cout * (double)((d->Cin * 9 + 255) / 256 * 256) / (d->Cin * 9) * 1.15
                               : 1.0;
    const double t_direct = nominal * dpad / (d->Cout < 128 ? 100e12 : dense_d1 ? 123e12 : 130e12);
    const double f = dcfp_wino_exec_fraction(d->N, d->H, d->W, d->dil, d->Cout, d->Cin);
    double t_b = 1e30, t_f = 1e30;
    if (batched) {
        const double tiles = f * 9.0 / 16.0 * pix;
        const double pad2 = (double)((d->Cout + 255) / 256 * 256) / d->Cout * (double)((d->Cin + 255) / 256 * 256) / d->Cin;
        t_b = nominal * f * pad2 / 125e12 + (4.0 * pix * d->Cin + 64.0 * tiles * d->Cin) / 4.2e12 +
              (4.0 * pix * d->Cout + 64.0 * tiles * d->Cout) / 5.0e12 + 30e-6;
    }
    if (fused) {
        const double pad64 = (double)((d->Cout + 63) / 64 * 64) / d->Cout * (double)((d->Cin + 63) / 64 * 64) / d->Cin;
        t_f = nominal * f * pad64 / wino_wgrad_fused_rate() + 40e-6;
    }
    if (fused && (t_f <= t_b || wino_wgrad_fused_forced())) return t_f < 0.97 * t_direct ? 2 : 0;
    return t_b < 0.97 * t_direct ? 1 : 0;
}
static bool wino_wgrad_pass(const DcfpConvDesc* d) { return wino_wgrad_kind(d) != 0; }

bool dcfp_wgrad_is_winograd(const DcfpConvDesc* d) { return wino_wgrad_pass(d); }
bool dcfp_wgrad_wants_xform(const DcfpConvDesc* d) { return wino_wgrad_kind(d) == 1; }

double dcfp_wgrad_exec_fraction(const DcfpConvDesc* d) {
    return wino_wgrad_pass(d) ? dcfp_wino_exec_fraction(d->N, d->H, d->W, d->dil, d->Cout, d->Cin) : 1.0;
}

size_t dcfp_conv2d_fwd_dgrad_workspace_bytes_(const DcfpConvDesc* d, int pass);

extern "C" size_t dcfp_conv2d_workspace_bytes(const DcfpConvDesc* d, int pass) {
    if (pass == DCFP_CONV_FWD || pass == DCFP_CONV_DGRAD) return dcfp_conv2d_fwd_dgrad_workspace_bytes_(d, pass);
    if (pass != DCFP_CONV_WGRAD || check_desc(d) != DCFP_OK) return 0;
    if (dcfp_stem_shape(d)) return dcfp_stem_wgrad_workspace_bytes(d);
    if (const int wk = wino_wgrad_kind(d)) {
        const size_t b1 = dcfp_wino_wgrad_ok(d->N, d->H, d->W, d->dil, d->Cout, d->Cin)
                              ? dcfp_wino_wgrad_workspace_bytes(d->N, d->H, d->W, d->dil, d->Cout, d->Cin) : 0;
        if (wk == 1) return b1;
        const size_t b2 = dcfp_wino_wgrad_fused_workspace_bytes(d->N, d->H, d->W, d->dil, d->Cout, d->Cin);
        const Plan pl = make_plan(d);
        const size_t b0 = pl.splits > 1 ? (size_t)pl.splits * d->Cout * d->Cin * d->KH * d->KW * sizeof(float) : 0;
        const size_t m = b1 > b0 ? b1 : b0;
        return b2 > m ? b2 : m;
    }
    const Plan pl = make_plan(d);
    if (pl.splits <= 1) return 0;
    return (size_t)pl.splits * d->Cout * d->Cin * d->KH * d->KW * sizeof(float);
}

extern "C" int dcfp_conv2d_wgrad_f32_nchw(const DcfpConvDesc* d, const float* dy,
                                          int64_t dy_nstride, const float* x, float* dw, float* db,
                                          void* workspace, size_t workspace_bytes,
                                          dcfp_stream_t stream) {
    int rc = check_desc(d);
    if (rc) return rc;
    if (!dy || !x || !dw) return DCFP_E_BADDESC;
    if (dcfp_gemv_shape(d) && !db)
        return dcfp_gemv_wgrad(d, dy, dy_nstride, x, dw, dcfp_s(stream));
    if (dcfp_stem_shape(d) && !db)
        return dcfp_stem_wgrad(d, dy, dy_nstride, x, dw, workspace, workspace_bytes, dcfp_s(stream));
    int wk = wino_wgrad_kind(d);
    if (wk == 2) {
        const int dyp = d->dy_pitch ? d->dy_pitch : d->Wout, xp = d->x_pitch ? d->x_pitch : d->W;
        const long long dyn = dy_nstride ? dy_nstride : (long long)d->Cout * d->Hout * dyp;
        if (!dcfp_wino_wgrad_fused_ok(d->N, d->H, d->W, d->dil, d->Cout, d->Cin, (long long)d->Cin * d->H * xp, xp, dyn, dyp))
            wk = dcfp_wino_wgrad_ok(d->N, d->H, d->W, d->dil, d->Cout, d->Cin) ? 1 : 0;
    }
    if (wk) {
        const int dyp = d->dy_pitch ? d->dy_pitch : d->Wout, xp = d->x_pitch ? d->x_pitch : d->W;
        const long long dyn = dy_nstride ? dy_nstride : (long long)d->Cout * d->Hout * dyp;
        if (db && dyp != d->Wout) return DCFP_E_UNSUPPORTED;
        if (wk == 2) {
            rc = dcfp_wino_wgrad_fused_run(dy, dyn, dyp, x, (long long)d->Cin * d->H * xp, xp, dw, d->N, d->Cout, d->Cin, d->H,
                                           d->W, d->dil, workspace, workspace_bytes, dcfp_s(stream));
        } else
            rc = dcfp_wino_wgrad_run(dy, dyn, dyp, x, (long long)d->Cin * d->H * xp, xp, dw, d->N, d->Cout, d->Cin, d->H, d->W,
                                     d->dil, workspace, workspace_bytes, dcfp_s(stream));
        if (rc) return rc;
        if (db)
            hipLaunchKernelGGL(bias_grad_kernel, dim3((unsigned)d->Cout), dim3(1024), 0, dcfp_s(stream), dy, dyn, db, d->N,
                               d->Hout * d->Wout, (int)((d->Hout * d->Wout) % 4 == 0 && dyn % 4 == 0 && dcfp_aligned16(dy)));
        DCFP_RETURN_LAUNCH();
    }
    const Plan pl = make_plan(d);
    const int T = d->KH * d->KW;
    const long long wn = (long long)d->Cout * d->Cin * T;
    const size_t need = pl.splits > 1 ? (size_t)pl.splits * wn * sizeof(float) : 0;
    if (need && (!workspace || workspace_bytes < need)) return DCFP_E_WORKSPACE;
    WgradParams p;
    p.dy = dy; p.x = x;
    p.out = pl.splits > 1 ? static_cast<float*>(workspace) : dw;
    p.x_pitch = d->x_pitch ? d->x_pitch : d->W;
    p.dy_pitch = d->dy_pitch ? d->dy_pitch : d->Wout;
    const bool pitched = p.x_pitch != d->W || p.dy_pitch != d->Wout;
    if (pitched && !dcfp_wgrad_pitch_ok(d)) return DCFP_E_UNSUPPORTED;
    if (db && p.dy_pitch != d->Wout) return DCFP_E_UNSUPPORTED;
    p.dy_nstride = dy_nstride ? dy_nstride : (long long)d->Cout * d->Hout * p.dy_pitch;
    p.x_nstride = (long long)d->Cin * d->H * p.x_pitch;
    p.N = d->N; p.M = d->Cout; p.Cin = d->Cin; p.Nn = d->Cin * T;
    p.H = d->H; p.W = d->W; p.Ho = d->Hout; p.Wo = d->Wout; p.P = d->Hout * d->Wout;
    p.stride = d->stride; p.pad = d->pad; p.dil = d->dil;
    if ((long long)d->N * p.P >= (1LL << 30)) return DCFP_E_UNSUPPORTED;
    p.Kpix = d->N * p.P;
    p.kchunk = pl.kchunk; p.splits = pl.splits; p.tiles_m = pl.tiles_m; p.tiles_n = pl.tiles_n;
    p.quad_ok = (d->Wout % 4 == 0) ? 1 : 0;
    p.batch = 1; p.dy_bstride = p.x_bstride = 0;
    {
        const long long span = (long long)pl.kchunk / p.P + 2;
        const long long big = p.dy_nstride > p.x_nstride ? p.dy_nstride : p.x_nstride;
        if (span * big * 4 >= (1LL << 31)) return DCFP_E_UNSUPPORTED;
    }
    if (wgrad3_ok(d, pl.cfg))
        rc = dcfp_wgrad3_launch(dy, p.dy_nstride, x, p.x_nstride, p.out, d->N, d->Cout, d->Cin, T, d->H, d->W,
                                d->Hout, d->Wout, d->pad, d->dil, p.Kpix, pl.kchunk, pl.splits, pl.tiles_m,
                                pl.tiles_n, dcfp_s(stream));
    else if (pl.wide) {
        const long long blocks = (long long)pl.tiles_m * pl.tiles_n * pl.splits;
        if (blocks > 0x7fffffffLL) return DCFP_E_UNSUPPORTED;
        rc = T == 1 ? launch_dma<1, false, true>(p, blocks, dcfp_s(stream)) : launch_dma<9, false, true>(p, blocks, dcfp_s(stream));
    } else if (wgrad_dma_ok(d, pl.cfg)) {
        const long long blocks = (long long)pl.tiles_m * pl.tiles_n * pl.splits;
        if (blocks > 0x7fffffffLL) return DCFP_E_UNSUPPORTED;
        rc = T == 1 ? (pl.half ? launch_dma<1, false, false, false, true>(p, blocks, dcfp_s(stream)) : launch_dma<1, false>(p, blocks, dcfp_s(stream)))
                    : (wgrad_dma_mixed(d) && p.x_pitch == d->W) ? launch_dma<9, true>(p, blocks, dcfp_s(stream))
                                                                 : launch_dma<9, false>(p, blocks, dcfp_s(stream));
    } else
        rc = T == 1 ? launch_taps<1>(p, pl, dcfp_s(stream)) : launch_taps<9>(p, pl, dcfp_s(stream));
    if (rc) return rc;
    if (pl.splits > 1) {
        if (wn % 4 == 0 && dcfp_aligned16(workspace) && dcfp_aligned16(dw)) {
            const long long n4 = wn / 4;
            hipLaunchKernelGGL(splitk_reduce_vec4_kernel, dim3((unsigned)((n4 + 255) / 256)), dim3(256), 0,
                               dcfp_s(stream), static_cast<const float*>(workspace), dw, n4, wn, pl.splits);
        } else {
            long long b = (wn + 255) / 256;
            if (b > 4096) b = 4096;
            hipLaunchKernelGGL(splitk_reduce_kernel, dim3((unsigned)b), dim3(256), 0, dcfp_s(stream),
                               static_cast<const float*>(workspace), dw, wn, pl.splits);
        }
    }
    if (db) {
        hipLaunchKernelGGL(bias_grad_kernel, dim3((unsigned)d->Cout), dim3(1024), 0, dcfp_s(stream),
                           dy, p.dy_nstride, db, d->N, p.P,
                           (int)(p.P % 4 == 0 && p.dy_nstride % 4 == 0 && dcfp_aligned16(dy) && p.dy_pitch == d->Wout));
    }
    DCFP_RETURN_LAUNCH();
}

extern "C" int dcfp_conv2d_wgrad_kept_f32_nchw(const DcfpConvDesc* d, const float* dy, int64_t dy_nstride,
                                               const float* xform, size_t xform_bytes, float* dw, void* workspace,
                                               size_t workspace_bytes, dcfp_stream_t stream) {
    int rc = check_desc(d);
    if (rc) return rc;
    if (!dy || !xform || !dw) return DCFP_E_BADDESC;
    const size_t need = dcfp_conv2d_xform_bytes(d);
    if (need == 0) return DCFP_E_UNSUPPORTED;
    if (xform_bytes < need || !dcfp_aligned16(xform)) return DCFP_E_WORKSPACE;
    const int dyp = d->dy_pitch ? d->dy_pitch : d->Wout;
    const long long dyn = dy_nstride ? dy_nstride : (long long)d->Cout * d->Hout * dyp;
    return dcfp_wino_wgrad_run(dy, dyn, dyp, nullptr, 0, 0, dw, d->N, d->Cout, d->Cin, d->H, d->W, d->dil, workspace,
                               workspace_bytes, dcfp_s(stream), xform);
}
```

### dcfp_amd/csrc/conv_winograd3.hip

```cpp
#include "wino_patch.h"
#include <stdlib.h>

namespace {

constexpr int GBK = 8;
constexpr int GKH = 144;
constexpr int GHALF = 2 * GKH;
constexpr int GCOMP = 2 * GHALF;
constexpr int GSTAGE = 16 * GCOMP;
constexpr unsigned kSat = 0xffffffffu;

struct WinoWgParams {
    const float* x_base;
    unsigned x_bytes;
    const float* dy_base;
    unsigned dy_bytes;
    const unsigned* table;
    unsigned table_bytes;
    float* out;
    int M, C, mblocks, cblocks, nblk;
    unsigned x_chan_bytes, dy_chan_bytes;
    int kchunk;
    long long T16;
    int d;
// ... 241 lines not shown
    load_entry(nk > 3 ? 3 : nk - 1);
    asm volatile("s_waitcnt vmcnt(0) lgkmcnt(0)" ::: "memory");
    __builtin_amdgcn_s_barrier();

    const int a_lane = wm * GHALF + lhi * GKH + l31 * 4;
    const int b_lane = wn * GHALF + lhi * GKH + l31 * 4;
    f32x4 af[2] = {{0.f, 0.f, 0.f, 0.f}, {0.f, 0.f, 0.f, 0.f}};
    f32x4 bf[2] = {{0.f, 0.f, 0.f, 0.f}, {0.f, 0.f, 0.f, 0.f}};
    auto step = [&](auto prod_, auto par_, int kt) {
        constexpr bool PROD = decltype(prod_)::value;
        constexpr int cur = decltype(par_)::value, rb = cur ^ 1;
        const float* As = smem + cur * 2 * GSTAGE + a_lane;
        const float* Bs = smem + cur * 2 * GSTAGE + GSTAGE + b_lane;
        const int k_entry = kt + 4 < nk ? kt + 4 : nk - 1;
        static_for<0, 16>([&](auto g_) {
            constexpr int g = decltype(g_)::value;
            constexpr int fb = g & 1, pg = (g + 15) & 15;
            af[fb] = *reinterpret_cast<const f32x4*>(As + g * GCOMP);
            bf[fb] = *reinterpret_cast<const f32x4*>(Bs + g * GCOMP);
            f32x2 ox = {0.f, 0.f}, oy = {0.f, 0.f};
            if constexpr (PROD) {
                if constexpr (g < 4) {
                    row_transform_one<DM, g>(R[rb], q);
#pragma unroll
                    for (int c = 0; c < PatchCfg<DM>::NCOL; ++c) asm volatile("" : "+v"(q[g][c]));
                    dy_rows(g_, D[rb]);
                }
                oy = dy_component<DM, g>(U);
                ox = col_transform<DM, g>(q);
                asm volatile("" : "+v"(ox), "+v"(oy));
                if constexpr (g == 7) make_offsets();
            }
            __builtin_amdgcn_sched_barrier(0);
            acc[pg] = __builtin_amdgcn_mfma_f32_32x32x2f32(af[fb ^ 1][0], bf[fb ^ 1][0], acc[pg], 0, 0, 0);
            acc[pg] = __builtin_amdgcn_mfma_f32_32x32x2f32(af[fb ^ 1][1], bf[fb ^ 1][1], acc[pg], 0, 0, 0);
            __builtin_amdgcn_sched_barrier(0);
            if constexpr (PROD) {
                *reinterpret_cast<f32x2*>(smem + rb * 2 * GSTAGE + g * GCOMP + pw) = oy;
                *reinterpret_cast<f32x2*>(smem + rb * 2 * GSTAGE + GSTAGE + g * GCOMP + pw) = ox;
            }
            __builtin_amdgcn_sched_barrier(0);
            acc[pg] = __builtin_amdgcn_mfma_f32_32x32x2f32(af[fb ^ 1][2], bf[fb ^ 1][2], acc[pg], 0, 0, 0);
            __builtin_amdgcn_sched_barrier(0);
            if constexpr (PROD && g >= 8) {
                constexpr int lo = (g - 8) * NT / 8, hi = (g - 7) * NT / 8;
                static_for<lo, hi>([&](auto i_) { vmem_op(i_, std::integral_constant<int, rb>{}, k_entry); });
            }
            acc[pg] = __builtin_amdgcn_mfma_f32_32x32x2f32(af[fb ^ 1][3], bf[fb ^ 1][3], acc[pg], 0, 0, 0);
            __builtin_amdgcn_sched_barrier(0);
        });
    };

    int kt = 0;
    for (; kt + 3 < nk; kt += 2) {
        step(std::true_type{}, even, kt);
        retire();
        step(std::true_type{}, odd, kt + 1);
        retire();
    }
    step(std::true_type{}, even, nk - 2);
    retire();
    step(std::false_type{}, odd, nk - 1);
#pragma unroll
    for (int kk = 0; kk < 4; ++kk)
        acc[15] = __builtin_amdgcn_mfma_f32_32x32x2f32(af[1][kk], bf[1][kk], acc[15], 0, 0, 0);

    const long long mc = (long long)p.M * p.C;
    const __amdgpu_buffer_rsrc_t o_rsrc = __builtin_amdgcn_make_buffer_rsrc(p.out + (long long)split * 16 * mc, 0,
                                                                            (unsigned)(16 * mc * 4), 0x00020000);
    const int m0 = mb * 64 + wm * 32 + 4 * lhi, c0 = cb * 64 + wn * 32 + l31;
    const unsigned ov = (!RAGGED || c0 < p.C) ? (unsigned)(((long long)m0 * p.C + c0) * 4) : kOob;
    const unsigned C4 = (unsigned)p.C * 4u, mc4 = (unsigned)(mc * 4);
    static_for<0, 16>([&](auto xi_) {
        constexpr int XI = decltype(xi_)::value;
        constexpr bool neg = ((XI >> 2) == 3) != ((XI & 3) == 3);
        static_for<0, 16>([&](auto r_) {
            constexpr int r = decltype(r_)::value, mr = (r & 3) + 8 * (r >> 2);
            const unsigned so = __builtin_amdgcn_readfirstlane((unsigned)XI * mc4 + (unsigned)mr * C4);
            const unsigned vo = (!RAGGED || m0 + mr < p.M) ? ov : kOob;
            const float v = neg ? -acc[XI][r] : acc[XI][r];
            __builtin_amdgcn_raw_buffer_store_b32(__builtin_bit_cast(unsigned, v), o_rsrc, vo, so, 0);
        });
    });
}

struct WgPlan {
    int TH, TW, mblocks, cblocks, splits, kchunk, mode, lead;
    long long T, T16, table_floats, slab_floats;
};

int wg_mode(int N, int H, int W, int d, int M, int C, long long x_nstride, int x_pitch, long long dy_nstride, int dy_pitch) {
    const long long xspan = ((long long)(N - 1) * x_nstride + (long long)((C + 63) / 64 * 64) * H * x_pitch + 64) * 4;
    const long long yspan = ((long long)(N - 1) * dy_nstride + (long long)((M + 63) / 64 * 64) * H * dy_pitch + 64) * 4;
    if (xspan >= 0x7fffff00LL || yspan >= 0x7fffff00LL) return -1;
    if ((d == 1 || d == 2) && x_pitch >= W + 4 && W % 4 == 0) return d;
    if (d >= 4 && d % 2 == 0 && W % 2 == 0) return 4;
    return -1;
}

WgPlan wg_plan(int N, int H, int W, int d, int M, int C) {
    WgPlan pl;
    pl.TH = d * ((H + 2 * d - 1) / (2 * d));
    pl.TW = d * ((W + 2 * d - 1) / (2 * d));
    pl.TW = (pl.TW + 3) / 4 * 4;
    pl.T = (long long)N * pl.TH * pl.TW;
    pl.T16 = (pl.T + 15) / 16 * 16;
    pl.mblocks = (M + 63) / 64;
    pl.cblocks = (C + 63) / 64;
    const long long tiles = (long long)pl.mblocks * pl.cblocks, slots = dcfp_num_cus();
    long long max_splits = pl.T16 / (32 * GBK);
    if (max_splits < 1) max_splits = 1;
    long long splits = 1;
    double best = -1.0;
    for (long long sp = 1; sp <= max_splits && tiles * sp <= 2 * slots; ++sp) {
        const long long blocks = tiles * sp, rounds = (blocks + slots - 1) / slots;
        const double eff = (double)blocks / (double)(rounds * slots);
        if (eff > best + 0.02) { best = eff; splits = sp; }
    }
    long long kchunk = (pl.T16 + splits - 1) / splits;
    kchunk = (kchunk + 15) / 16 * 16;
    splits = (pl.T16 + kchunk - 1) / kchunk;
    pl.splits = (int)splits;
    pl.kchunk = (int)kchunk;
    pl.table_floats = (pl.T16 / 2 * 8 + 63) / 64 * 64;
    pl.slab_floats = (long long)pl.splits * 16 * M * C;
    return pl;
}

}

bool dcfp_wino_wgrad_fused_enabled() {
    static const int v = [] { const char* e = getenv("DCFP_WINO_WGRAD_FUSED"); return e ? atoi(e) : 1; }();
    return v != 0;
}

bool dcfp_wino_wgrad_fused_ok(int N, int H, int W, int d, int M, int C, long long x_nstride, int x_pitch,
                              long long dy_nstride, int dy_pitch) {
    if (!dcfp_wino_wgrad_fused_enabled()) return false;
    if (M < 48 || C < 48) return false;
    if (x_pitch <= 0) x_pitch = W;
    if (dy_pitch <= 0) dy_pitch = W;
    if (wg_mode(N, H, W, d, M, C, x_nstride, x_pitch, dy_nstride, dy_pitch) < 0) return false;
    const WgPlan pl = wg_plan(N, H, W, d, M, C);
    if (pl.T16 >= (1LL << 30) || pl.T16 / 2 * 32 >= 0x7fffff00LL) return false;
    if (16LL * M * C * 4 >= 0x7fffff00LL) return false;
    return (long long)pl.mblocks * pl.cblocks * pl.splits < (1LL << 28);
}

size_t dcfp_wino_wgrad_fused_workspace_bytes(int N, int H, int W, int d, int M, int C) {
    const WgPlan pl = wg_plan(N, H, W, d, M, C);
    return (size_t)(pl.table_floats + pl.slab_floats) * sizeof(float);
}

int dcfp_wino_wgrad_fused_run(const float* dy, long long dy_nstride, int dy_pitch, const float* x, long long x_nstride,
                              int x_pitch, float* dw, int N, int M, int C, int H, int W, int d, void* workspace,
                              size_t workspace_bytes, hipStream_t stream) {
    if (x_pitch <= 0) x_pitch = W;
    if (dy_pitch <= 0) dy_pitch = W;
    const int mode = wg_mode(N, H, W, d, M, C, x_nstride, x_pitch, dy_nstride, dy_pitch);
    if (mode < 0) return DCFP_E_UNSUPPORTED;
    const WgPlan pl = wg_plan(N, H, W, d, M, C);
    if (!workspace || !dcfp_aligned16(workspace) || workspace_bytes < dcfp_wino_wgrad_fused_workspace_bytes(N, H, W, d, M, C))
        return DCFP_E_WORKSPACE;
    unsigned* table = static_cast<unsigned*>(workspace);
    float* slabs = static_cast<float*>(workspace) + pl.table_floats;
    const int lead = mode == 4 ? 0 : 4;
    const long long npairs = pl.T16 / 2;
    hipLaunchKernelGGL(wino_wg_table_kernel, dim3((unsigned)((npairs + 255) / 256)), dim3(256), 0, stream, table, npairs, pl.T,
                       N, H, W, d, pl.TH, pl.TW, x_nstride, x_pitch, lead, dy_nstride, dy_pitch, mode);
    WinoWgParams p;
    p.x_base = x - lead;
    p.x_bytes = (unsigned)(((long long)(N - 1) * x_nstride + (long long)C * H * x_pitch + lead) * 4);
    p.dy_base = dy;
    p.dy_bytes = (unsigned)(((long long)(N - 1) * dy_nstride + (long long)M * H * dy_pitch) * 4);
    p.table = table;
    p.table_bytes = (unsigned)(npairs * 32);
    p.out = slabs;
    p.M = M; p.C = C; p.mblocks = pl.mblocks; p.cblocks = pl.cblocks;
    p.nblk = pl.mblocks * pl.cblocks * pl.splits;
    p.x_chan_bytes = (unsigned)((long long)H * x_pitch * 4);
    p.dy_chan_bytes = (unsigned)((long long)H * dy_pitch * 4);
    p.kchunk = pl.kchunk;
    p.T16 = pl.T16;
    p.d = d;
    const unsigned grid = (unsigned)(((p.nblk + 7) / 8) * 8);
    const size_t lds = (size_t)4 * GSTAGE * sizeof(float);
    auto launch = [&](auto kern) -> int {
        hipError_t e = hipFuncSetAttribute(reinterpret_cast<const void*>(kern), hipFuncAttributeMaxDynamicSharedMemorySize,
                                           (int)lds);
        if (e != hipSuccess) return (int)e;
        hipLaunchKernelGGL(kern, dim3(grid), dim3(256), lds, stream, p);
        hipError_t e2 = hipGetLastError();
        return e2 == hipSuccess ? DCFP_OK : (int)e2;
    };
    const bool ragged = (M % 64) != 0 || (C % 64) != 0;
    int rc;
#define DCFP_WG(DM_) (ragged ? launch(wino_wgrad_fused_kernel<DM_, true>) : launch(wino_wgrad_fused_kernel<DM_, false>))
    switch (mode) {
        case 1: rc = DCFP_WG(1); break;
        case 2: rc = DCFP_WG(2); break;
        default: rc = DCFP_WG(4); break;
    }
#undef DCFP_WG
    if (rc) return rc;
    const long long mc = (long long)M * C;
    hipLaunchKernelGGL(wino_dw_reduce_kernel, dim3((unsigned)((mc + 255) / 256)), dim3(256), 0, stream, slabs, pl.splits, mc, dw);
    DCFP_RETURN_LAUNCH();
}
```

### dcfp_amd/csrc/igemm2_common.h

```cpp
#pragma once
#include "common.h"
#include <type_traits>

struct Igemm2Params {
    const float* in;
    const float* wp;
    const float* bias;
    const float* scale;
    const float* shift;
    const float* residual;
    int relu;
    float* out;
    long long in_nstride, out_nstride;
    int N, M, Mpad, Ck, CkP;
    int Hi, Wi, Ho, Wo, P, tiles_per_img, tiles_n_total, tiles_m;
    int sn, sd, off0, offstep;
    int accumulate, vec_store;
    int tile2d;
    int Hc, Wc, tiles_per_phase;
    int in_pitch;
    int zfold;
    const float* fan_src;
    const unsigned long long* fan_mask;
    long long wp_nstride;
    int nt_store;
    int tapskip;
    float* stat_part;
    const float* red_x;
    const unsigned long long* red_mask;
    const float* red_mean;
    float* red_part;
};

namespace {

typedef float f32x16 __attribute__((ext_vector_type(16)));
typedef float f32x4 __attribute__((ext_vector_type(4)));

constexpr int BK = 16;
constexpr unsigned kOob = 0x80000000u;

template <int I, int N, typename F>
__device__ __forceinline__ void static_for(F&& f) {
    if constexpr (I < N) {
        f(std::integral_constant<int, I>{});
        static_for<I + 1, N>(f);
    }
}

__device__ __forceinline__ void wino_filter2_pair(const float* __restrict__ w, int sAm, int sAc, int flip, int M, int Ck,
                                                  int Mpad, long long idx, float* __restrict__ Ug) {
    const int mblocks = Mpad / 64;
    const int c = (int)(idx / Mpad), m = (int)(idx - (long long)c * Mpad);
    float g[9];
    if (m < M && c < Ck) {
        const float* src = w + (long long)m * sAm + (long long)c * sAc;
#pragma unroll
        for (int t = 0; t < 9; ++t) g[t] = src[flip ? 8 - t : t];
    } else {
#pragma unroll
        for (int t = 0; t < 9; ++t) g[t] = 0.f;
    }
    float r[4][3];
#pragma unroll
    for (int k = 0; k < 3; ++k) {
        const float g0 = g[k], g1 = g[3 + k], g2 = g[6 + k];
        r[0][k] = g0;
        r[1][k] = 0.5f * ((g0 + g2) + g1);
        r[2][k] = 0.5f * ((g0 + g2) - g1);
        r[3][k] = g2;
    }
    const int cb = c >> 3, cl = c & 7, mb = m >> 6, ml = m & 63;
    float* dst = Ug + ((((long long)(cb * mblocks + mb) * 16) * 2 + (ml >> 5)) * 64 + (cl & 1) * 32 + (ml & 31)) * 4 + (cl >> 1);
#pragma unroll
    for (int i = 0; i < 4; ++i) {
        const float a = r[i][0], b = r[i][1], cc = r[i][2];
        dst[(4 * i + 0) * 512] = a;
        dst[(4 * i + 1) * 512] = 0.5f * ((a + cc) + b);
        dst[(4 * i + 2) * 512] = 0.5f * ((a + cc) - b);
        dst[(4 * i + 3) * 512] = cc;
    }
}

template <int T>
struct Frag;
template <>
struct Frag<4> {
    static __device__ __forceinline__ void ld(const float* p, float (&f)[4]) {
        const float4 v = *reinterpret_cast<const float4*>(p);
        f[0] = v.x; f[1] = v.y; f[2] = v.z; f[3] = v.w;
    }
};
template <>
struct Frag<2> {
    static __device__ __forceinline__ void ld(const float* p, float (&f)[2]) {
        const float2 v = *reinterpret_cast<const float2*>(p);
        f[0] = v.x; f[1] = v.y;
    }
};
template <>
struct Frag<1> {
    static __device__ __forceinline__ void ld(const float* p, float (&f)[1]) { f[0] = p[0]; }
};

}
```

### dcfp_amd/networks/_exec.py

```python
import os

import torch
import torch.nn as nn

from .. import ops

_BN_TYPES = (nn.BatchNorm2d, nn.SyncBatchNorm)


def conv(m, x):
    if m.groups != 1 or m.kernel_size[0] != m.kernel_size[1] or m.stride[0] != m.stride[1] \
            or m.padding[0] != m.padding[1] or m.dilation[0] != m.dilation[1] \
            or isinstance(m.padding, str) or m.padding_mode != "zeros":
        raise RuntimeError(f"dcfp_amd: unsupported conv configuration {m}")
    return ops.conv2d(x, m.weight, m.bias, m.stride[0], m.padding[0], m.dilation[0])


FUSE_BLOCKS = os.environ.get("DCFP_NO_BLOCK_FUSION") is None


def _bn_args(m):
    training = m.training or (m.running_mean is None)
    sync = False
    if isinstance(m, nn.SyncBatchNorm) and training:
        sync = m.process_group if m.process_group is not None else True
    momentum = m.momentum
    nbt = None
    if training:
        m._dcfp_fold = None
    if training and m.track_running_stats and m.num_batches_tracked is not None:
        if momentum is None:
            m.num_batches_tracked.add_(1)
            momentum = 1.0 / float(m.num_batches_tracked)
        else:
            nbt = m.num_batches_tracked
    if not m.affine:
        raise RuntimeError("dcfp_amd: BatchNorm without affine parameters is not on the DCFP path")
    return (m.running_mean, m.running_var, training, momentum, m.eps, sync, nbt)


def _conv_pitch(cm, xshape):
    if cm is None or cm.kernel_size != (3, 3) or cm.groups != 1 or isinstance(cm.padding, str):
        return 0
    return ops.conv_pitch(tuple(xshape), tuple(cm.weight.shape), cm.stride[0], cm.padding[0], cm.dilation[0])


def bn_act(m, x, relu=False, residual=None, prev_conv=None, next_conv=None):
    rm, rv, training, momentum, eps, sync, nbt = _bn_args(m)
    pitch_cfg = None
    if x.is_cuda and torch.is_grad_enabled() and x.requires_grad and x.dim() == 4:
        y_pitch = _conv_pitch(next_conv, x.shape) if residual is None else 0
        dx_pitch = 0
        if prev_conv is not None and prev_conv.kernel_size == (3, 3):
            in_shape = (x.shape[0], prev_conv.in_channels, x.shape[2], x.shape[3])
            dx_pitch = _conv_pitch(prev_conv, in_shape)
        if y_pitch or dx_pitch:
            pitch_cfg = (m, y_pitch, dx_pitch)
    return ops.batch_norm_act(x, m.weight, m.bias, rm, rv, residual, relu, training, momentum, eps, sync, nbt, pitch_cfg)


def _fold(bn):
    key = (bn.weight._version, bn.bias._version, bn.running_mean._version, bn.running_var._version,
           bn.weight.data_ptr(), bn.running_mean.data_ptr(), ops.WEIGHT_EPOCH[0])
    cached = getattr(bn, "_dcfp_fold", None)
    if cached is None or cached[0] != key:
        with torch.no_grad():
            scale = bn.weight * torch.rsqrt(bn.running_var + bn.eps)
            shift = bn.bias - bn.running_mean * scale
        cached = (key, scale.contiguous(), shift.contiguous())
        bn._dcfp_fold = cached
    return cached[1], cached[2]


def conv_bn_act(cm, bn, x, relu=False, residual=None, next_conv=None):
    if (not bn.training) and bn.running_mean is not None and not torch.is_grad_enabled() \
            and cm.bias is None and cm.groups == 1 and cm.padding_mode == "zeros":
        scale, shift = _fold(bn)
        return ops.conv2d_fused_infer(x, cm.weight, scale, shift, cm.stride[0], cm.padding[0],
                                      cm.dilation[0], residual, relu)
    return bn_act(bn, conv(cm, x), relu=relu, residual=residual, prev_conv=cm, next_conv=next_conv)


def _plain_conv(m, k):
    ok = (m.groups == 1 and m.bias is None and m.kernel_size == (k, k) and m.padding_mode == "zeros"
          and not isinstance(m.padding, str))
    if not ok:
        raise RuntimeError(f"dcfp_amd: unsupported conv configuration in Bottleneck: {m}")


def bottleneck(blk, x):
    _plain_conv(blk.conv1, 1); _plain_conv(blk.conv2, 3); _plain_conv(blk.conv3, 1)
    bns = [blk.bn1, blk.bn2, blk.bn3]
    tensors = [blk.conv1.weight, blk.bn1.weight, blk.bn1.bias, blk.conv2.weight, blk.bn2.weight,
               blk.bn2.bias, blk.conv3.weight, blk.bn3.weight, blk.bn3.bias]
    stride, dil = blk.conv2.stride[0], blk.conv2.dilation[0]
    if blk.conv2.padding[0] != dil or blk.conv1.stride[0] != 1 or blk.conv3.stride[0] != 1:
        raise RuntimeError("dcfp_amd: unexpected Bottleneck geometry")
    if blk.downsample is not None:
        dconv, dbn = blk.downsample[0], blk.downsample[1]
        _plain_conv(dconv, 1)
        if dconv.stride[0] != stride:
            raise RuntimeError("dcfp_amd: downsample stride differs from conv2 stride")
        tensors += [dconv.weight, dbn.weight, dbn.bias]
        bns.append(dbn)
    cfg = {"stride": stride, "dil": dil, "bn": [_bn_args(b) for b in bns], "owner": blk}
    return ops.bottleneck(x, cfg, tensors)


def run_sequential(seq, x, tail_conv=None):
    mods = list(seq.children())
    i = 0
    while i < len(mods):
        m = mods[i]
        if isinstance(m, nn.Conv2d) and i + 1 < len(mods) and isinstance(mods[i + 1], _BN_TYPES):
            fuse = i + 2 < len(mods) and isinstance(mods[i + 2], nn.ReLU)
            nxt = None
            if fuse:
                nxt = mods[i + 3] if i + 3 < len(mods) else (tail_conv if i + 3 == len(mods) else None)
            x = conv_bn_act(m, mods[i + 1], x, relu=fuse, next_conv=nxt if isinstance(nxt, nn.Conv2d) else None)
            i += 2 if fuse else 1
        elif isinstance(m, nn.Conv2d):
            x = conv(m, x)
        elif isinstance(m, _BN_TYPES):
            fuse = i + 1 < len(mods) and isinstance(mods[i + 1], nn.ReLU)
            x = bn_act(m, x, relu=fuse)
            if fuse:
                i += 1
        elif isinstance(m, nn.ReLU):
            raise RuntimeError("dcfp_amd: bare ReLU outside a BN+ReLU pair is not on the DCFP path")
        elif isinstance(m, nn.Dropout2d):
            x = ops.dropout2d(x, m.p, m.training, getattr(m, "fixed_mask", None))
        elif isinstance(m, nn.AdaptiveAvgPool2d):
            size = m.output_size
            size = (size, size) if isinstance(size, int) else tuple(size)
            if None in size:
                raise RuntimeError(f"dcfp_amd: no HIP path for {m} (a None output size)")
            x = ops.global_avg_pool(x) if size == (1, 1) else ops.adaptive_avg_pool(x, size)
        elif isinstance(m, nn.Identity):
            pass
        else:
            raise RuntimeError(f"dcfp_amd: no HIP path for module {type(m).__name__}")
        i += 1
    return x


def require_device(x):
    if not x.is_cuda:
        raise RuntimeError(
            "dcfp_amd networks run on the MI355X HIP kernels only: move the model and inputs to "
            "cuda (the CPU restatement used for checking lives under oracle/, not in the product)")
```

### dcfp_amd/networks/backbone/resnet.py

```python
import torch.nn as nn

from .. import _exec
from ... import ops

BatchNorm2d = nn.BatchNorm2d

_DEPTHS = {"50": [3, 4, 6, 3], "101": [3, 4, 23, 3], "152": [3, 8, 36, 3]}
_OS_CFG = {16: ([1, 2, 2, 1], [1, 1, 1, 2]), 8: ([1, 2, 1, 1], [1, 1, 2, 4]),
           32: ([1, 2, 2, 2], [1, 1, 1, 1])}


class Bottleneck(nn.Module):
    expansion = 4

    def __init__(self, inplanes, planes, stride=1, dilation=1, downsample=None):
        super().__init__()
        self.conv1 = nn.Conv2d(inplanes, planes, kernel_size=1, bias=False)
        self.bn1 = BatchNorm2d(planes)
        self.conv2 = nn.Conv2d(planes, planes, kernel_size=3, stride=stride, dilation=dilation,
                               padding=dilation, bias=False)
        self.bn2 = BatchNorm2d(planes)
        self.conv3 = nn.Conv2d(planes, planes * 4, kernel_size=1, bias=False)
        self.bn3 = BatchNorm2d(planes * 4)
        self.relu = nn.ReLU(inplace=True)
        self.relu_inplace = nn.ReLU(inplace=True)
        self.downsample = downsample
        self.stride = stride
        self.dilation = dilation

    def forward(self, x):
        if _exec.FUSE_BLOCKS and x.requires_grad:
            return _exec.bottleneck(self, x)
        out = _exec.conv_bn_act(self.conv1, self.bn1, x, relu=True)
        out = _exec.conv_bn_act(self.conv2, self.bn2, out, relu=True)
        residual = x if self.downsample is None else _exec.run_sequential(self.downsample, x)
        return _exec.conv_bn_act(self.conv3, self.bn3, out, relu=True, residual=residual)


class ResNet(nn.Module):
    def __init__(self, block, layers, output_stride, inplanes=128, mg_unit=(1, 1, 1),
                 out_index=(1, 3, 4)):
        super().__init__()
        if output_stride not in _OS_CFG:
            raise NotImplementedError
        strides, dilations = _OS_CFG[output_stride]
        self.inplanes = inplanes
        self.out_index = list(out_index)
        self.conv1 = nn.Sequential(
            nn.Conv2d(3, 64, 3, 2, 1, bias=False), BatchNorm2d(64), nn.ReLU(inplace=True),
            nn.Conv2d(64, 64, 3, 1, 1, bias=False), BatchNorm2d(64), nn.ReLU(inplace=True),
            nn.Conv2d(64, inplanes, 3, 1, 1, bias=False))
        self.bn1 = BatchNorm2d(inplanes)
        self.relu1 = nn.ReLU(inplace=True)
        self.maxpool = nn.MaxPool2d(kernel_size=3, stride=2, padding=1)
        self.layer1 = self._stage(block, 64, [dilations[0]] * layers[0], strides[0])
        self.layer2 = self._stage(block, 128, [dilations[1]] * layers[1], strides[1])
        self.layer3 = self._stage(block, 256, [dilations[2]] * layers[2], strides[2])
        self.layer4 = self._stage(block, 512, [g * dilations[3] for g in mg_unit], strides[3])

    def _stage(self, block, planes, block_dilations, stride):
        downsample = None
        if stride != 1 or self.inplanes != planes * block.expansion:
            downsample = nn.Sequential(
                nn.Conv2d(self.inplanes, planes * block.expansion, kernel_size=1, stride=stride,
                          bias=False),
                BatchNorm2d(planes * block.expansion))
        blocks = [block(self.inplanes, planes, stride, block_dilations[0], downsample)]
        self.inplanes = planes * block.expansion
        for d in block_dilations[1:]:
            blocks.append(block(self.inplanes, planes, dilation=d))
        return nn.Sequential(*blocks)

    def forward(self, input):
        _exec.require_device(input)
        stem = list(self.conv1.children())
        x = _exec.run_sequential(nn.Sequential(*stem[:-1]), input, tail_conv=stem[-1])
        x = _exec.conv_bn_act(stem[-1], self.bn1, x, relu=True)
        x = ops.maxpool3x3s2(x)
        outs = []
        for i in range(1, 5):
            for blk in getattr(self, "layer" + str(i)):
                x = blk(x)
            if i in self.out_index:
                if i < 4:
                    tap, x = ops.fork(x)
                    outs.append(tap)
                else:
                    outs.append(x)
        return tuple(outs)


def build_resnet(name, para):
    para = para if para is not None else {}
    for key, layers in _DEPTHS.items():
        if name.endswith(key):
            break
    else:
        raise NotImplementedError(f"{name}: the reference builds resnet50/101/152 only")
    model = ResNet(Bottleneck, layers, para.get("os", 8), inplanes=para.get("inplanes", 128),
                   mg_unit=para.get("mg_unit", [1, 2, 4]), out_index=para.get("out_index", [1, 3, 4]))
    if para.get("pretrained", True):
        path = para.get("pretrained_path")
        if path is None:
            raise FileNotFoundError(
                "backbone_para['pretrained'] is true but no 'pretrained_path' was given; pass "
                "{'pretrained': False} for random init (reference: mypath.py:2-5 expects downloaded .pth)")
        from ...utils.pyt_utils import load_model
        load_model(model, path)
    return model
```

### dcfp_amd/ops.py

```python
import ctypes as C
import os
import weakref

import torch
import torch.distributed as dist

from . import _lib, arena, syncbn_p2p
from ._lib import ConvDesc, BnRunning, check

_ws_cache = {}
WEIGHT_EPOCH = [0]

_PROFILE = None


def profile_start():
    global _PROFILE
    _PROFILE = []


def profile_stop():
    global _PROFILE
    recs, _PROFILE = _PROFILE, None
    torch.cuda.synchronize()
# ... 237 lines not shown
    r.num_batches_tracked = nbt.data_ptr() if nbt is not None else None
    r.momentum = float(momentum) if upd else 0.0
    return r


def _rp(run):
    return C.byref(run) if run is not None else None


FANIN_RED_USED = [0]
FANIN_BN_SUMS = os.environ.get("DCFP_FANIN_BN_SUMS", "1") not in ("0",)
FANIN_BN_SUMS_ALWAYS = os.environ.get("DCFP_FANIN_BN_SUMS", "1") == "2"
KEEP_XFORM = os.environ.get("DCFP_KEEP_XFORM", "1") not in ("0",)


def conv2d_fwd(x, w, bias=None, stride=1, pad=0, dil=1, want_stats=False, bn_run=None, out=None, keep=None):
    _require(x, "x"); _require(w, "weight")
    xp = _pitch_of(x)
    if not xp:
        x = x.contiguous()
    w = w if w.is_contiguous() else w.contiguous()
    d = _desc(x.shape, w.shape, stride, pad, dil, xp, 0)
    yns = 0
    if out is None:
        y = torch.empty((d.N, d.Cout, d.Hout, d.Wout), dtype=torch.float32, device=x.device)
    else:
        y = out
        st = y.stride()
        if tuple(y.shape) != (d.N, d.Cout, d.Hout, d.Wout) or st[3] != 1 or st[2] != d.Wout or st[1] != d.Hout * d.Wout:
            raise RuntimeError("conv2d_fwd: out must be [N,Cout,Ho,Wo] with dense images (a channel slice is fine)")
        yns = st[0]
    if bias is not None:
        _require(bias, "bias"); bias = bias.contiguous()
    L = _lib.lib()
    variant = "bias" if (bias is not None and d.KH == 3 and conv_kernel_name(d, _lib.CONV_FWD).startswith("winograd")) else ""
    ws, valid = _conv_workspace(w, _lib.CONV_FWD, d, variant)
    if keep is not None and KEEP_XFORM and bias is None:
        xb = L.dcfp_conv2d_xform_bytes(C.byref(d))
        if xb > 0:
            xf = torch.empty(xb, dtype=torch.uint8, device=x.device)
            slots = L.dcfp_conv2d_fwd_stat_slots(C.byref(d), _p(y), yns) if want_stats else 0
            part = _workspace("bn_stat_partials", slots * d.Cout * 2 * 4, x.device) if slots > 0 else None
            _timed("conv_fwd", d, _conv_flops(d), lambda: check(
                L.dcfp_conv2d_fwd_keep_f32_nchw(C.byref(d), _p(x), _p(w), _p(y), yns, _p(xf), xb, _p(part), _p(ws),
                                                ws.numel(), _stream()), "conv2d_fwd_keep"))
            keep["xform"] = xf
            if part is not None:
                mv = torch.empty((2, d.Cout), dtype=torch.float32, device=x.device)
                check(L.dcfp_bn_stats_from_partials_f32(_p(part), slots, 128, d.Cout, _p(mv[0]), _p(mv[1]),
                                                        _rp(bn_run), _stream()), "bn_stats_from_partials")
                return y, (mv[0], mv[1], bn_run is not None)
            return (y, None) if want_stats else y
    if want_stats and bias is None:
        slots = L.dcfp_conv2d_fwd_stat_slots(C.byref(d), _p(y), yns)
        if slots > 0:
            part = _workspace("bn_stat_partials", slots * d.Cout * 2 * 4, x.device)
            _timed("conv_fwd", d, _conv_flops(d), lambda: check(
                L.dcfp_conv2d_fwd_stats_f32_nchw(C.byref(d), _p(x), _p(w), _p(y), yns, _p(part), _p(ws),
                                                 ws.numel(), valid, _stream()), "conv2d_fwd_stats"))
            mv = torch.empty((2, d.Cout), dtype=torch.float32, device=x.device)
            check(L.dcfp_bn_stats_from_partials_f32(_p(part), slots, 128, d.Cout, _p(mv[0]), _p(mv[1]),
                                                    _rp(bn_run), _stream()), "bn_stats_from_partials")
            return y, (mv[0], mv[1], bn_run is not None)
    _timed("conv_fwd", d, _conv_flops(d), lambda: check(
        L.dcfp_conv2d_fwd_f32_nchw(C.byref(d), _p(x), _p(w), _p(bias), _p(y), yns, _p(ws), ws.numel(), valid,
                                   _stream()), "conv2d_fwd"))
    return (y, None) if want_stats else y


def conv2d_dgrad(dy, w, xshape, stride, pad, dil, out=None, accumulate=False):
    _require(dy, "dy")
    w = w if w.is_contiguous() else w.contiguous()
    dp = _pitch_of(dy)
    d = _desc(xshape, w.shape, stride, pad, dil, 0, dp)
    if dp:
        ns = dy.stride(0)
    else:
        dy, ns = _batch_strided(dy)
    if out is not None:
        if tuple(out.shape) != tuple(xshape) or not out.is_contiguous():
            raise RuntimeError("conv2d_dgrad: out must be a contiguous tensor of the input shape")
        dx = out
    else:
        dx = torch.empty(xshape, dtype=torch.float32, device=dy.device)
        accumulate = False
    L = _lib.lib()
    ws, valid = _conv_workspace(w, _lib.CONV_DGRAD, d)
    _timed("conv_dgrad", d, _conv_flops(d), lambda: check(
        L.dcfp_conv2d_dgrad_f32_nchw(C.byref(d), _p(dy), ns, _p(w), _p(dx), int(bool(accumulate)),
                                     _p(ws), ws.numel(), valid, _stream()), "conv2d_dgrad"))
    return dx


MASKED_FANIN = os.environ.get("DCFP_MASKED_FANIN", "1") not in ("0",)


def conv2d_dgrad_fanin_ok(dyshape, w, xshape):
    d = _desc(xshape, w.shape, 1, 0, 1)
    return MASKED_FANIN and bool(_lib.lib().dcfp_conv2d_dgrad_fanin_supported(C.byref(d)))


def conv2d_dgrad_fanin(dy, w, xshape, fan_src, fan_mask):
    _require(dy, "dy"); _require(fan_src, "fan_src")
    w = w if w.is_contiguous() else w.contiguous()
    d = _desc(xshape, w.shape, 1, 0, 1)
    dy, ns = _batch_strided(dy)
    if tuple(fan_src.shape) != tuple(xshape) or not fan_src.is_contiguous():
        raise RuntimeError("conv2d_dgrad_fanin: fan_src must be a contiguous tensor of the input shape")
    dx = torch.empty(xshape, dtype=torch.float32, device=dy.device)
    ws, valid = _conv_workspace(w, _lib.CONV_DGRAD, d)
    _timed("conv_dgrad", d, _conv_flops(d), lambda: check(
        _lib.lib().dcfp_conv2d_dgrad_fanin_f32_nchw(C.byref(d), _p(dy), ns, _p(w), _p(dx), _p(fan_src), _p(fan_mask),
                                                    _p(ws), ws.numel(), valid, _stream()), "conv2d_dgrad_fanin"))
    return dx


def conv2d_dgrad_fanin_red_slots(w, xshape):
    if not (MASKED_FANIN and FANIN_BN_SUMS):
        return 0
    d = _desc(xshape, w.shape, 1, 0, 1)
    return int(_lib.lib().dcfp_conv2d_dgrad_fanin_red_slots(C.byref(d)))


def conv2d_dgrad_fanin_red(dy, w, xshape, fan_src, fan_mask, red_x, red_mask, red_mean, slots):
    _require(dy, "dy"); _require(fan_src, "fan_src"); _require(red_x, "red_x")
    w = w if w.is_contiguous() else w.contiguous()
    d = _desc(xshape, w.shape, 1, 0, 1)
    dy, ns = _batch_strided(dy)
    if tuple(fan_src.shape) != tuple(xshape) or not fan_src.is_contiguous():
        raise RuntimeError("conv2d_dgrad_fanin_red: fan_src must be a contiguous tensor of the input shape")
    if tuple(red_x.shape) != tuple(xshape) or not red_x.is_contiguous() or red_mean.numel() != xshape[1]:
        raise RuntimeError("conv2d_dgrad_fanin_red: red_x / red_mean must match the input shape")
    dx = torch.empty(xshape, dtype=torch.float32, device=dy.device)
    part = torch.empty((slots, xshape[1], 2), dtype=torch.float32, device=dy.device)
    ws, valid = _conv_workspace(w, _lib.CONV_DGRAD, d)
    _timed("conv_dgrad_red", d, _conv_flops(d), lambda: check(
        _lib.lib().dcfp_conv2d_dgrad_fanin_red_f32_nchw(C.byref(d), _p(dy), ns, _p(w), _p(dx), _p(fan_src), _p(fan_mask),
                                                        _p(red_x), _p(red_mask), _p(red_mean), _p(part), _p(ws),
                                                        ws.numel(), valid, _stream()), "conv2d_dgrad_fanin_red"))
    return dx, part


def bn_bwd_sums_from_partials(part, var, eps, dgamma=None, dbeta=None):
    slots, Cc, _ = part.shape
    s = torch.empty((2, Cc), dtype=torch.float32, device=part.device)
    if dgamma is None:
        dgamma = torch.empty(Cc, dtype=torch.float32, device=part.device)
    _timed("bn_bwd_reduce", None, 8.0 * part.numel() / 2, lambda: check(
        _lib.lib().dcfp_bn_bwd_sums_from_partials_f32(_p(part), slots, Cc, _p(var), float(eps), _p(s[0]), _p(s[1]),
                                                      _p(dgamma), _p(dbeta), _stream()), "bn_bwd_sums_from_partials"))
    return s[0], s[1], dgamma


def conv2d_wgrad(dy, x, wshape, stride, pad, dil, need_bias=False, dw=None, db=None, xform=None):
    _require(dy, "dy"); _require(x, "x")
    xp, dp = _pitch_of(x), _pitch_of(dy)
    if not xp:
        x = x.contiguous()
    d = _desc(x.shape, wshape, stride, pad, dil, xp, dp)
    if dp:
        ns = dy.stride(0)
    else:
        dy, ns = _batch_strided(dy)
    L = _lib.lib()
    nbytes = L.dcfp_conv2d_workspace_bytes(C.byref(d), _lib.CONV_WGRAD)
    ws = _workspace("conv_scratch", nbytes, x.device)
    if dw is None:
        dw = torch.empty(wshape, dtype=torch.float32, device=x.device)
    elif tuple(dw.shape) != tuple(wshape) or not dw.is_contiguous():
        raise RuntimeError("conv2d_wgrad: dw must be a contiguous tensor of the weight shape")
    if need_bias and db is None:
        db = torch.empty((wshape[0],), dtype=torch.float32, device=x.device)
    if xform is not None and not need_bias and L.dcfp_conv2d_xform_bytes(C.byref(d)) == xform.numel():
        _timed("conv_wgrad", d, _conv_flops(d), lambda: check(
            L.dcfp_conv2d_wgrad_kept_f32_nchw(C.byref(d), _p(dy), ns, _p(xform), xform.numel(), _p(dw), _p(ws), ws.numel(),
                                              _stream()), "conv2d_wgrad_kept"))
        return dw, None
    _timed("conv_wgrad", d, _conv_flops(d), lambda: check(
        L.dcfp_conv2d_wgrad_f32_nchw(C.byref(d), _p(dy), ns, _p(x), _p(dw), _p(db) if need_bias else None, _p(ws),
                                     ws.numel(), _stream()), "conv2d_wgrad"))
    return dw, (db if need_bias else None)


def add_into(dst, src):
    check(_lib.lib().dcfp_add_f32(_p(dst), _p(src), _p(dst), dst.numel(), _stream()), "add")


def wgrad_into_param(dy, x, w, bias, stride, pad, dil, keep=None):
    tw, kw = arena.grad_target(w)
    tb, kb = arena.grad_target(bias) if bias is not None else (None, 0)
    xform = keep.pop("xform", None) if keep else None
    conv2d_wgrad(dy, x, tuple(w.shape), stride, pad, dil, need_bias=bias is not None, dw=tw, db=tb, xform=xform)
    dw = arena.grad_commit(w, tw, kw, add_into)
    db = arena.grad_commit(bias, tb, kb, add_into) if bias is not None else None
    return dw, db


class Conv2dFn(torch.autograd.Function):

    @staticmethod
    def forward(ctx, x, w, bias, stride, pad, dil):
        ctx.keep = {} if ctx.needs_input_grad[1] else None
        y = conv2d_fwd(x, w, bias, stride, pad, dil, keep=ctx.keep)
        ctx.save_for_backward(x)
        ctx.params = (w, bias)
        ctx.cfg = (stride, pad, dil)
        return y

    @staticmethod
    def backward(ctx, dy):
        (x,) = ctx.saved_tensors
        w, bias = ctx.params
        stride, pad, dil = ctx.cfg
        dx = dw = db = None
        if ctx.needs_input_grad[0]:
            dx = conv2d_dgrad(dy, w, tuple(x.shape), stride, pad, dil)
        if ctx.needs_input_grad[1] or (bias is not None and ctx.needs_input_grad[2]):
            dw, db = wgrad_into_param(dy, x, w, bias, stride, pad, dil, keep=ctx.keep)
        return dx, dw, db, None, None, None


def conv2d(x, w, bias=None, stride=1, pad=0, dil=1):
    return Conv2dFn.apply(x, w, bias, stride, pad, dil)


def bn_stats(x, run=None):
    _require(x, "x")
    N, Cc, H, W = x.shape
    x, ns = _batch_strided(x)
    L = _lib.lib()
    ws = _workspace("bn", L.dcfp_bn_workspace_bytes(N, Cc, H * W), x.device)
    mean = torch.empty(Cc, dtype=torch.float32, device=x.device)
    var = torch.empty(Cc, dtype=torch.float32, device=x.device)
    _timed("bn_stats", None, 4.0 * x.numel(), lambda: check(
        L.dcfp_bn_stats_f32(_p(x), ns, N, Cc, H * W, _p(mean), _p(var), _rp(run), _p(ws), ws.numel(), _stream()),
        "bn_stats"))
    return mean, var


def bn_apply(x, mean, var, gamma, beta, eps, residual=None, relu=False, out=None):
    N, Cc, H, W = x.shape
    x = x.contiguous()
    if residual is not None:
        residual = residual.contiguous()
    yns, ypitch = 0, 0
    if out is None:
        y = torch.empty_like(x)
    else:
        y = out
        st = y.stride()
        ypitch = _pitch_of(y)
        if not ypitch and st[3] == 1 and st[2] > W and st[2] % 4 == 0 and st[1] == H * st[2]:
            ypitch = st[2]
        if tuple(y.shape) != tuple(x.shape) or (not ypitch and (st[3] != 1 or st[2] != W or st[1] != H * W)):
            raise RuntimeError("bn_apply: out must have dense images or be a row-pitched buffer")
        yns = st[0]
    nbytes = (8.0 + (4.0 if residual is not None else 0.0)) * x.numel()
    _timed("bn_apply", None, nbytes, lambda: check(
        _lib.lib().dcfp_bn_apply_f32(_p(x), _p(mean), _p(var), _p(gamma), _p(beta), float(eps),
                                     _p(residual), int(relu), _p(y), yns, N, Cc, H * W, W, ypitch, _stream()),
        "bn_apply"))
    return y


def bn_apply_relu_mask(x, mean, var, gamma, beta, eps, residual):
    N, Cc, H, W = x.shape
    if (H * W) % 256 != 0:
        return None
    x = x.contiguous(); residual = residual.contiguous()
    y = torch.empty_like(x)
    mask = torch.empty(x.numel() // 64, dtype=torch.int64, device=x.device)
    rc = [0]

    def run():
        rc[0] = _lib.lib().dcfp_bn_apply_relu_mask_f32(_p(x), _p(mean), _p(var), _p(gamma), _p(beta), float(eps),
                                                       _p(residual), _p(y), _p(mask), N, Cc, H * W, _stream())
    _timed("bn_apply", None, 12.125 * x.numel(), run)
    if rc[0] == _lib.E_UNSUPPORTED:
        return None
    check(rc[0], "bn_apply_relu_mask")
    return y, mask


def bn_bwd_reduce(dy, x, y, mean, var, gamma, beta, eps, relu, dgamma=None, dbeta=None):
    N, Cc, H, W = x.shape
    dy, dns = _batch_strided(dy)
    L = _lib.lib()
    ws = _workspace("bn", L.dcfp_bn_workspace_bytes(N, Cc, H * W), x.device)
    s = torch.empty((2, Cc), dtype=torch.float32, device=x.device)
    s1, s2 = s[0], s[1]
    if dgamma is None:
        dgamma = torch.empty(Cc, dtype=torch.float32, device=x.device)
    _timed("bn_bwd_reduce", None, (8.0 + (4.0 if relu == 1 else 0.125 if relu == 3 else 0.0)) * x.numel(), lambda: check(
        L.dcfp_bn_bwd_reduce_f32(_p(dy), dns, _p(x), _p(y) if relu in (1, 3) else None, 0, _p(mean), _p(var),
                                 _p(gamma), _p(beta), float(eps), int(relu), N, Cc, H * W, _p(s1), _p(s2),
                                 _p(dgamma), _p(dbeta), _p(ws), ws.numel(), _stream()),
        "bn_bwd_reduce"))
    return s1, s2, dgamma


def bn_bwd_apply(dy, x, y, mean, var, gamma, beta, eps, s1, s2, count, relu, want_residual, dx_out=None):
    N, Cc, H, W = x.shape
    dy, dns = _batch_strided(dy)
    dxp = 0
    if dx_out is not None:
        dxp = _pitch_of(dx_out)
        if tuple(dx_out.shape) != tuple(x.shape) or not dxp:
            raise RuntimeError("bn_bwd_apply: dx_out must be a row-pitched buffer of x's shape")
        dx = dx_out
    else:
        dx = torch.empty_like(x)
    dres = torch.empty_like(x) if want_residual else None
    nbytes = (12.0 + (4.0 if relu == 1 else 0.125 if relu == 3 else 0.0) + (4.0 if want_residual else 0.0)) * x.numel()
    count_dev = count if isinstance(count, torch.Tensor) else None
    count_host = 0.0 if count_dev is not None else float(count)
    _timed("bn_bwd_apply", None, nbytes, lambda: check(
        _lib.lib().dcfp_bn_bwd_apply_f32(_p(dy), dns, _p(x), _p(y) if relu in (1, 3) else None, 0, _p(mean),
                                         _p(var), _p(gamma), _p(beta), float(eps), _p(s1), _p(s2), count_host,
                                         _p(count_dev), int(relu), _p(dx), _p(dres), N, Cc, H * W, W, dxp,
                                         _stream()),
        "bn_bwd_apply"))
    return dx, dres


BN_BWD_FUSED = os.environ.get("DCFP_BN_FUSED", "1") != "0"
FUSED_BN_USED = [0]
_FUSED_SYNC = {}


def _fused_sync(nbytes, device):
# ... 1 lines not shown
    st = _FUSED_SYNC.get(key)
    if st is None:
        st = [None, 0, torch.zeros(1, dtype=torch.int32, device=device)]
        _FUSED_SYNC[key] = st
    if st[0] is None or st[0].numel() < nbytes or st[1] >= 0xfffffff0:
        st[0] = torch.zeros(max(int(nbytes), 1 << 20), dtype=torch.uint8, device=device)
        st[1] = 0
    st[1] += 1
    return st[0], st[1], st[2]


def check_fused_status():
    for (dev, _), st in _FUSED_SYNC.items():
        v = int(st[2].item())
        if v != 0:
            raise RuntimeError("dcfp_amd: fused BatchNorm backward (call %d on device %s) gave up waiting for the blocks of "
                               "a channel; its outputs are NaN.  DCFP_BN_FUSED=0 selects the two-kernel path" % (v, dev))


def bn_bwd_fused(dy, x, y, mean, var, gamma, beta, eps, count, relu, want_residual, dx_out=None, dgamma=None, dbeta=None):
    N, Cc, H, W = x.shape
    L = _lib.lib()
    need = L.dcfp_bn_bwd_fused_sync_bytes(N, Cc, H * W)
    if need == 0:
        return None
    dy, dns = _batch_strided(dy)
    dxp = 0
    if dx_out is not None:
        dxp = _pitch_of(dx_out)
        if tuple(dx_out.shape) != tuple(x.shape) or not dxp:
            raise RuntimeError("bn_bwd_fused: dx_out must be a row-pitched buffer of x's shape")
        dx = dx_out
    else:
        dx = torch.empty_like(x)
    dres = torch.empty_like(x) if want_residual else None
    s = torch.empty((2, Cc), dtype=torch.float32, device=x.device)
    if dgamma is None:
        dgamma = torch.empty(Cc, dtype=torch.float32, device=x.device)
    sync, epoch, status = _fused_sync(need, x.device)
    nbytes = (12.0 + (4.0 if relu == 1 else 0.125 if relu == 3 else 0.0) + (4.0 if want_residual else 0.0)) * x.numel()
    rc = [0]

    def run():
        rc[0] = L.dcfp_bn_bwd_fused_f32(_p(dy), dns, _p(x), _p(y) if relu in (1, 3) else None, 0, _p(mean), _p(var),
                                        _p(gamma), _p(beta), float(eps), float(count), int(relu), _p(dx), _p(dres),
                                        N, Cc, H * W, W, dxp, _p(s[0]), _p(s[1]), _p(dgamma), _p(dbeta), _p(sync),
                                        sync.numel(), epoch, 0, _p(status), _stream())
    _timed("bn_bwd_fused", None, nbytes, run)
    if rc[0] == _lib.E_UNSUPPORTED:
        return None
    check(rc[0], "bn_bwd_fused")
    FUSED_BN_USED[0] += 1
    return s[0], s[1], dgamma, dx, dres


def _sync_group(group):
    if group is False or not dist.is_available() or not dist.is_initialized():
        return None
    g = None if group is True else group
    if dist.get_world_size(g) <= 1 and not os.environ.get("DCFP_FORCE_SYNCBN"):
        return None
    return g if g is not None else dist.group.WORLD


_COUNT_CACHE = {}


def _count_tensor(count, device):
    key = (float(count), str(device))
    t = _COUNT_CACHE.get(key)
    if t is None:
        t = torch.tensor([float(count)], device=device, dtype=torch.float32)
        _COUNT_CACHE[key] = t
    return t


def syncbn_combine_reference(allv, Cc):
    a = allv.double()
    world = a.shape[0]
    n = a[:, 2 * Cc]
    tot = torch.zeros((), dtype=torch.float64, device=a.device)
    m = torch.zeros(Cc, dtype=torch.float64, device=a.device)
    for r in range(world):
        tot = tot + n[r]
        m = m + a[r, :Cc] * n[r]
    m = m / tot
    v = torch.zeros(Cc, dtype=torch.float64, device=a.device)
    for r in range(world):
        dlt = a[r, :Cc] - m
        v = v + (a[r, Cc:2 * Cc] + dlt * dlt) * n[r]
    return m.float(), (v / tot).float(), tot.float().reshape(1)


def sync_bn_stats(mean, var, count, group, run=None, running=None):
    Cc = mean.numel()
    world = dist.get_world_size(group)
    local = torch.cat([mean, var, _count_tensor(count, mean.device)])
    px = syncbn_p2p.for_group(group) if mean.is_cuda else None
    if px is not None:
        out = torch.empty(2 * Cc + 1, device=mean.device, dtype=torch.float32)
        _timed("syncbn_p2p_fwd", None, 4.0 * local.numel() * world, lambda: px.exchange(local, out, 2, _rp(run)))
        return out[:Cc], out[Cc:2 * Cc], out[2 * Cc:]
    allv = torch.empty(world, local.numel(), device=mean.device, dtype=mean.dtype)
    if mean.is_cuda:
        _timed("syncbn_allgather", None, 4.0 * local.numel() * world,
               lambda: dist.all_gather_into_tensor(allv, local.unsqueeze(0), group=group))
    else:
        dist.all_gather_into_tensor(allv, local.unsqueeze(0), group=group)
    if mean.is_cuda:
        out = torch.empty(2 * Cc + 1, device=mean.device, dtype=torch.float32)
        check(_lib.lib().dcfp_syncbn_combine_f32(_p(allv), world, Cc, _p(out), _p(out[Cc:]), _p(out[2 * Cc:]),
                                                 _rp(run), _stream()), "syncbn_combine")
        return out[:Cc], out[Cc:2 * Cc], out[2 * Cc:]
    gmean, gvar, total = syncbn_combine_reference(allv, Cc)
    if running is not None:
        rm, rv, momentum, nbt = running
        if rm is not None and momentum is not None:
            n = float(total)
            rm.mul_(1.0 - momentum).add_(gmean, alpha=momentum)
            rv.mul_(1.0 - momentum).add_(gvar * (n / max(n - 1.0, 1.0)), alpha=momentum)
        if nbt is not None:
            nbt.add_(1)
    return gmean.contiguous(), gvar.contiguous(), total.contiguous()


def sync_bn_bwd_sums(s1, s2, group, async_op=False):
    Cc = s1.numel()
    adjacent = (s1.is_contiguous() and s2.is_contiguous()
                and s1.untyped_storage().data_ptr() == s2.untyped_storage().data_ptr()
                and s2.storage_offset() == s1.storage_offset() + Cc)
    px = syncbn_p2p.for_group(group) if s1.is_cuda else None
    if px is not None:
        both = s1.as_strided((2 * Cc,), (1,), s1.storage_offset()) if adjacent else torch.cat([s1, s2])
        out = torch.empty_like(both)
        if async_op:
            work = px.exchange_async(both, out, 1)
            return out[:Cc], out[Cc:], work
        _timed("syncbn_p2p_bwd", None, 8.0 * Cc * px.world, lambda: px.exchange(both, out, 1))
        return out[:Cc], out[Cc:]
    if adjacent:
        both = s1.as_strided((2 * Cc,), (1,), s1.storage_offset())
        work = dist.all_reduce(both, group=group, async_op=async_op)
        return (s1, s2, work) if async_op else (s1, s2)
    both = torch.cat([s1, s2])
    work = dist.all_reduce(both, group=group, async_op=async_op)
    r1, r2 = both[:Cc], both[Cc:]
    return (r1, r2, work) if async_op else (r1.contiguous(), r2.contiguous())


def bn_forward_impl(x, gamma, beta, running_mean, running_var, residual, relu, training,
                    momentum, eps, sync, nbt=None, stats=None, want_mask=False, out=None):
    _require(x, "x")
    x = x.contiguous()
    N, Cc, H, W = x.shape
    count = float(N * H * W)
    group = _sync_group(sync) if training else None
    if training:
        run = _bn_run(running_mean, running_var, momentum, nbt)
        if stats is not None:
            mean, var, applied = stats
            if applied:
                run = None
        elif group is None:
            mean, var = bn_stats(x, run)
            run = None
        else:
            mean, var = bn_stats(x)
        if group is not None:
            mean, var, count = sync_bn_stats(mean, var, count, group, run)
        elif run is not None:
            if running_mean is not None and momentum is not None:
                check(_lib.lib().dcfp_bn_update_running_f32(
                    _p(mean), _p(var), Cc, float(momentum), float(count), None, _p(running_mean),
                    _p(running_var), _stream()), "bn_update_running")
            if nbt is not None:
                nbt.add_(1)
    else:
        mean, var = running_mean, running_var
    if want_mask and relu and residual is not None and BN_RELU_BITMASK and out is None:
        ym = bn_apply_relu_mask(x, mean, var, gamma, beta, eps, residual)
        if ym is not None:
            return ym[0], (mean, var, count, group, ym[1])
    y = bn_apply(x, mean, var, gamma, beta, eps, residual, relu, out=out)
    return y, (mean, var, count, group)


def _bn_bwd_preface(relu, y, state, gamma, beta, gparam, bparam):
    mask = state[4] if len(state) > 4 else None
    if relu and mask is not None:
        relu, y = 3, mask
    else:
        relu = (1 if y is not None else 2) if relu else 0
    gp = gparam if gparam is not None else gamma
    bp = bparam if bparam is not None else beta
    return (relu, y, gp) + tuple(arena.grad_target(gp)) + (bp,) + tuple(arena.grad_target(bp))


def bn_backward_reduce(dy, x, y, gamma, beta, state, relu, training, gparam=None, bparam=None, eps=1e-5, pre=None):
    mean, var, count, group = state[:4]
    relu, y, gp, tg, kg, bp, tb, kb = _bn_bwd_preface(relu, y, state, gamma, beta, gparam, bparam)
    if pre is not None:
        s1, s2, _ = bn_bwd_sums_from_partials(pre, var, eps, dgamma=tg, dbeta=tb)
    else:
        s1, s2, _ = bn_bwd_reduce(dy, x, y, mean, var, gamma, beta, eps, relu, dgamma=tg, dbeta=tb)
    dgamma = arena.grad_commit(gp, tg, kg, add_into)
    dbeta = arena.grad_commit(bp, tb, kb, add_into)
    work = None
    if training and group is not None:
        s1, s2, work = sync_bn_bwd_sums(s1, s2, group, async_op=SYNCBN_ASYNC)[:3] if SYNCBN_ASYNC else \
            sync_bn_bwd_sums(s1, s2, group) + (None,)
    elif not training:
        s1 = torch.zeros_like(s1); s2 = torch.zeros_like(s2)
    return (s1, s2, work, relu, y, dgamma, dbeta)


def bn_backward_apply(dy, x, gamma, beta, state, red, eps, want_res, dx_out=None):
    s1, s2, work, relu, y, dgamma, dbeta = red
    if work is not None:
        _timed("syncbn_bwd_wait", None, 0.0, work.wait)
    mean, var, count = state[:3]
    dx, dres = bn_bwd_apply(dy, x, y, mean, var, gamma, beta, eps, s1, s2, count, relu, want_res, dx_out)
    return dx, dgamma, dbeta, dres


def bn_backward_impl(dy, x, y, gamma, beta, state, relu, training, eps, want_res, gparam=None, bparam=None,
                     between=None, dx_out=None, pre=None):
    if BN_BWD_FUSED and training and pre is None and state[3] is None and not isinstance(state[2], torch.Tensor):
        frelu, fy, gp, tg, kg, bp, tb, kb = _bn_bwd_preface(relu, y, state, gamma, beta, gparam, bparam)
        out = bn_bwd_fused(dy, x, fy, state[0], state[1], gamma, beta, eps, state[2], frelu, want_res, dx_out,
                           dgamma=tg, dbeta=tb)
        if out is not None:
            dgamma = arena.grad_commit(gp, tg, kg, add_into)
            dbeta = arena.grad_commit(bp, tb, kb, add_into)
            mid = between() if between is not None else None
            return (out[3], dgamma, dbeta, out[4]) + ((mid,) if between is not None else ())
    red = bn_backward_reduce(dy, x, y, gamma, beta, state, relu, training, gparam, bparam, eps, pre=pre)
    mid = between() if between is not None else None
    out = bn_backward_apply(dy, x, gamma, beta, state, red, eps, want_res, dx_out)
    return out + ((mid,) if between is not None else ())


def _conv_bn_fwd(inp, w, bnargs, g, b, stride=1, pad=0, dil=1, relu=True, res=None, want_mask=False, out=None, keep=None):
    rm, rv, training, momentum, eps, sync, nbt = bnargs
    stats = None
    if FUSE_BN_STATS and training:
        run = _bn_run(rm, rv, momentum, nbt) if _sync_group(sync) is None else None
        c, stats = conv2d_fwd(inp, w, None, stride, pad, dil, want_stats=True, bn_run=run, keep=keep)
    else:
        c = conv2d_fwd(inp, w, None, stride, pad, dil, keep=keep)
    y, state = bn_forward_impl(c, g, b, rm, rv, res, relu, training, momentum, eps, sync, nbt=nbt,
                               stats=stats, want_mask=want_mask, out=out)
    return c, y, state


def _pack_bn_states(states):
    flat, meta = [], []
    for st in states:
        if st is None:
            meta.append(None)
            continue
        mean, var, count, group = st[:4]
        mask = st[4] if len(st) > 4 else None
        is_t = isinstance(count, torch.Tensor)
        meta.append((len(flat), is_t, None if is_t else count, group, mask is not None))
        flat += [mean, var] + ([count] if is_t else []) + ([mask] if mask is not None else [])
    return flat, meta


def _bn_state(meta, flat, i):
    if meta[i] is None:
        return None
    pos, is_t, count, group, has_mask = meta[i]
    st = (flat[pos], flat[pos + 1], flat[pos + 2] if is_t else count, group)
    return st + ((flat[pos + 2 + is_t],) if has_mask else ())


def _concat_buffer(ctx, cfg, shape, device):
    ctx.pitch_slot = None
    if cfg["pitch"]:
        cat, ctx.pitch_slot = owner_pitched(cfg["owner"], shape, cfg["pitch"], device)
        return cat
    return torch.empty(shape, dtype=torch.float32, device=device)


def _release_pitch(ctx):
    if ctx.pitch_slot is not None:
        ctx.pitch_slot.release()


class BatchNormActFn(torch.autograd.Function):

    @staticmethod
    def forward(ctx, x, gamma, beta, running_mean, running_var, residual, relu, training,
                momentum, eps, sync, nbt, pitch_cfg):
        x = x.contiguous()
        out, ctx.pitch_slot, ctx.dx_pitch, ctx.dx_key = None, None, 0, "bn_dx"
        if pitch_cfg is not None:
            owner, y_pitch, ctx.dx_pitch = pitch_cfg
            ctx.dx_key = ("bn_dx", id(owner))
            if y_pitch and residual is None:
                out, ctx.pitch_slot = owner_pitched(owner, tuple(x.shape), y_pitch, x.device,
                                                    track=torch.is_grad_enabled())
        y, state = bn_forward_impl(x, gamma, beta, running_mean, running_var, residual, relu,
                                   training, momentum, eps, sync, nbt=nbt, out=out)
        flat, ctx.meta = _pack_bn_states([state])
        ctx.save_for_backward(x, y if (relu and residual is not None) else None, *flat)
        ctx.params = (gamma, beta)
        ctx.cfg = (relu, training, eps, residual is not None)
        return y

    @staticmethod
    def backward(ctx, dy):
        x, y = ctx.saved_tensors[:2]
        gamma, beta = ctx.params
        relu, training, eps, has_res = ctx.cfg
        state = _bn_state(ctx.meta, ctx.saved_tensors[2:], 0)
        need_res = has_res and ctx.needs_input_grad[5]
        dx_out = pitched_buffer(tuple(x.shape), ctx.dx_pitch, ctx.dx_key, x.device) if ctx.dx_pitch else None
        dx, dgamma, dbeta, dres = bn_backward_impl(dy, x, y, gamma, beta, state, relu, training, eps, need_res,
                                                   dx_out=dx_out)
        _release_pitch(ctx)
        return dx, dgamma, dbeta, None, None, dres, None, None, None, None, None, None, None


class BottleneckFn(torch.autograd.Function):

    @staticmethod
    def forward(ctx, x, cfg, *tensors):
        ctx.prev_rec = getattr(x, "_dcfp_bn3_rec", None) if FANIN_BN_SUMS else None
        x = x.contiguous()
        has_ds = len(tensors) == 12
        w1, g1, b1, w2, g2, b2, w3, g3, b3 = tensors[:9]
        bnargs = cfg["bn"]
        stride, dil = cfg["stride"], cfg["dil"]

        N_, _, H_, W_ = x.shape
        y1_shape = (N_, w1.shape[0], H_, W_)
# ... 317 lines not shown
    _timed("ppm_pool_adjoint", None, 4.0 * dx.numel() * (2 if g is not None else 1), lambda: check(
        _lib.lib().dcfp_ppm_pool_adjoint_f32(_p(dp), N, Cc, H, W, len(levels),
                                             _int_array(v for hw in levels for v in hw), _p(g), gns, gpitch, _p(dx),
                                             _stream()), "ppm_pool_adjoint"))
    return dx


def ppm_resize_adjoint(dy, widths, levels, align_corners):
    _require(dy, "dy")
    levels = _pool_levels(levels)
    dy, dns, dpitch = _rows_or_copy(dy)
    N, Ct, H, W = dy.shape
    if Ct != sum(widths) or len(widths) != len(levels):
        raise RuntimeError("ppm_resize_adjoint: dy must hold the levels' channels in order")
    buf = torch.empty(sum(N * c * a * b for c, (a, b) in zip(widths, levels)), dtype=torch.float32, device=dy.device)
    chw = [v for c, (a, b) in zip(widths, levels) for v in (c, a, b)]
    _timed("ppm_resize_adjoint", None, 4.0 * (dy.numel() + buf.numel()), lambda: check(
        _lib.lib().dcfp_ppm_resize_adjoint_f32(_p(dy), dns, dpitch, N, H, W, len(levels), _int_array(chw), _p(buf),
                                               int(bool(align_corners)), _stream()), "ppm_resize_adjoint"))
    return _level_views(buf, N, widths, levels)


class AdaptiveAvgPoolFn(torch.autograd.Function):

    @staticmethod
    def forward(ctx, x, sh, sw):
        _require(x, "x")
        ctx.shape = tuple(x.shape)
        ctx.hw = (sh, sw)
        return ppm_pool(x, [(sh, sw)])[0]

    @staticmethod
    def backward(ctx, dy):
        return ppm_pool_adjoint(dy.contiguous().reshape(-1), [ctx.hw], ctx.shape), None, None


def adaptive_avg_pool(x, size):
    sh, sw = (size, size) if isinstance(size, int) else size
    return AdaptiveAvgPoolFn.apply(x, int(sh), int(sw))


class PyramidPoolingFn(torch.autograd.Function):

    @staticmethod
    def forward(ctx, feats, cfg, *tensors):
        _require(feats, "feats")
        feats = feats.contiguous()
        N, Cf, H, W = feats.shape
        nst = len(tensors) // 3
        widths = [int(t.shape[0]) for t in tensors[0::3]]
        levels = [(int(s), int(s)) for s in cfg["sizes"]]
        offs = [sum(widths[:k]) for k in range(nst + 1)]
        cat = _concat_buffer(ctx, cfg, (N, offs[nst] + Cf, H, W), feats.device)
        align = cfg["align"]
        pooled = ppm_pool(feats, levels, True, dst=cat[:, offs[nst]:])
        cs, states = [], []
        for k in range(nst):
            w, g, b = tensors[3 * k:3 * k + 3]
            rm, rv, training, momentum, eps, sync, nbt = cfg["bn"][k]
            c = conv2d_fwd(pooled[k], w, None, 1, 0, 1)
            y, st = bn_forward_impl(c, g, b, rm, rv, None, True, training, momentum, eps, sync, nbt=nbt)
            resize_bilinear_into(y, cat[:, offs[k]:offs[k + 1]], align)
            cs.append(c); states.append(st)
        flat, ctx.meta = _pack_bn_states(states)
        ctx.params = tensors
        ctx.cfg = (levels, widths, offs, (N, Cf, H, W), align, [a[2] for a in cfg["bn"]], [a[4] for a in cfg["bn"]])
        ctx.save_for_backward(*pooled, *cs, *flat)
        return cat

    @staticmethod
    def backward(ctx, dcat):
        levels, widths, offs, fshape, align, training, eps = ctx.cfg
        nst = len(widths)
        saved = ctx.saved_tensors
        pooled, cs, flat = saved[:nst], saved[nst:2 * nst], saved[2 * nst:]
        tensors = ctx.params
        N, Cf, H, W = fshape
        need_dx = ctx.needs_input_grad[0]
        grads = [None] * (3 * nst)
        dys = ppm_resize_adjoint(dcat[:, :offs[nst]], widths, levels, align)
        dp = torch.empty(sum(N * Cf * a * b for a, b in levels), dtype=torch.float32, device=dcat.device) \
            if need_dx else None
        dps = _level_views(dp, N, [Cf] * nst, levels) if need_dx else None
        pending = None
        for k in range(nst):
            w, g, b = tensors[3 * k:3 * k + 3]
            res = bn_backward_impl(dys[k], cs[k], None, g, b, _bn_state(ctx.meta, flat, k), True, training[k], eps[k], False,
                                   between=pending)
            d_c, grads[3 * k + 1], grads[3 * k + 2] = res[0], res[1], res[2]
            if pending is not None:
                grads[3 * (k - 1)] = res[4]
            if need_dx:
                conv2d_dgrad(d_c, w, tuple(pooled[k].shape), 1, 0, 1, out=dps[k])
            pending = (lambda d_c=d_c, w=w, x=pooled[k]: wgrad_into_param(d_c, x, w, None, 1, 0, 1)[0])
        grads[3 * (nst - 1)] = pending()
        dfeats = ppm_pool_adjoint(dp, levels, fshape, g=dcat[:, offs[nst]:]) if need_dx else None
        _release_pitch(ctx)
        return (dfeats, None) + tuple(grads)


def pyramid_pooling(feats, cfg, tensors):
    return PyramidPoolingFn.apply(feats, cfg, *tensors)


class ForkFn(torch.autograd.Function):

    @staticmethod
    def forward(ctx, x):
        ctx.set_materialize_grads(False)
        return x.view_as(x), x.view_as(x)

    @staticmethod
    def backward(ctx, ga, gb):
        if ga is None or gb is None:
            return ga if gb is None else gb
        return add(ga, gb)


def fork(x):
    return ForkFn.apply(x) if (torch.is_grad_enabled() and x.requires_grad) else (x, x)


class MaxPool3x3s2Fn(torch.autograd.Function):

    @staticmethod
    def forward(ctx, x):
        _require(x, "x")
        x = x.contiguous()
        N, Cc, H, W = x.shape
        Ho, Wo = (H + 2 - 3) // 2 + 1, (W + 2 - 3) // 2 + 1
        y = torch.empty((N, Cc, Ho, Wo), dtype=torch.float32, device=x.device)
        idx = torch.empty((N, Cc, Ho, Wo), dtype=torch.int32, device=x.device)
        check(_lib.lib().dcfp_maxpool3x3s2_fwd_f32(_p(x), _p(y), _p(idx), N, Cc, H, W, Ho, Wo, _stream()),
              "maxpool_fwd")
        ctx.save_for_backward(idx)
        ctx.shape = (N, Cc, H, W, Ho, Wo)
        return y

    @staticmethod
    def backward(ctx, dy):
        (idx,) = ctx.saved_tensors
        N, Cc, H, W, Ho, Wo = ctx.shape
        dy = dy.contiguous()
        dx = torch.empty((N, Cc, H, W), dtype=torch.float32, device=dy.device)
        check(_lib.lib().dcfp_maxpool3x3s2_bwd_f32(_p(dy), _p(idx), _p(dx), N, Cc, H, W, Ho, Wo, _stream()),
              "maxpool_bwd")
        return dx


def maxpool3x3s2(x):
    return MaxPool3x3s2Fn.apply(x)


def rowsum(x, scale):
    N, Cc, H, W = x.shape
    x, ns = _batch_strided(x)
    y = torch.empty((N, Cc, 1, 1), dtype=torch.float32, device=x.device)
    check(_lib.lib().dcfp_rowsum_f32(_p(x), ns, _p(y), float(scale), N, Cc, H * W, _stream()), "rowsum")
    return y


def broadcast_hw(v, H, W, scale=1.0, out=None, accumulate=False):
    N, Cc = v.shape[0], v.shape[1]
    v = v.contiguous()
    yns = 0
    if out is None:
        y = torch.empty((N, Cc, H, W), dtype=torch.float32, device=v.device)
        accumulate = False
    else:
        y = out
        st = y.stride()
        if tuple(y.shape) != (N, Cc, H, W) or st[3] != 1 or st[2] != W or st[1] != H * W:
            raise RuntimeError("broadcast_hw: out must be [N,C,H,W] with dense images")
        yns = st[0]
    check(_lib.lib().dcfp_broadcast_hw_f32(_p(v), float(scale), _p(y), yns, int(bool(accumulate)), N, Cc, H * W,
                                           _stream()), "broadcast_hw")
    return y


class GlobalAvgPoolFn(torch.autograd.Function):

    @staticmethod
    def forward(ctx, x):
        _require(x, "x")
        ctx.hw = (x.shape[2], x.shape[3])
        return rowsum(x, 1.0 / (x.shape[2] * x.shape[3]))

    @staticmethod
    def backward(ctx, dy):
        H, W = ctx.hw
        return broadcast_hw(dy, H, W, 1.0 / (H * W))


class BroadcastHWFn(torch.autograd.Function):

    @staticmethod
    def forward(ctx, v, H, W):
        _require(v, "v")
        return broadcast_hw(v, H, W)

    @staticmethod
    def backward(ctx, dy):
        return rowsum(dy, 1.0), None, None


def global_avg_pool(x):
    return GlobalAvgPoolFn.apply(x)


def broadcast_to_hw(v, H, W):
    return BroadcastHWFn.apply(v, H, W)


class ChannelScaleFn(torch.autograd.Function):

    @staticmethod
    def forward(ctx, x, mask):
        _require(x, "x")
        x = x.contiguous()
        N, Cc, H, W = x.shape
        mask = mask.contiguous()
        y = torch.empty_like(x)
        check(_lib.lib().dcfp_channel_scale_f32(_p(x), _p(mask), _p(y), N, Cc, H * W, _stream()),
              "channel_scale")
        ctx.save_for_backward(mask)
        return y

    @staticmethod
    def backward(ctx, dy):
        (mask,) = ctx.saved_tensors
        dy = dy.contiguous()
        N, Cc, H, W = dy.shape
        dx = torch.empty_like(dy)
        check(_lib.lib().dcfp_channel_scale_f32(_p(dy), _p(mask), _p(dx), N, Cc, H * W, _stream()),
              "channel_scale")
        return dx, None


def dropout2d(x, p, training, fixed_mask=None):
    if not training or p == 0.0:
        return x
    if fixed_mask is not None:
        mask = fixed_mask.to(device=x.device, dtype=torch.float32)
    else:
        mask = torch.empty(x.shape[0], x.shape[1], device=x.device).bernoulli_(1.0 - p).div_(1.0 - p)
    return ChannelScaleFn.apply(x, mask)


def add(a, b):
    a = a.contiguous(); b = b.contiguous()
    out = torch.empty_like(a)
    check(_lib.lib().dcfp_add_f32(_p(a), _p(b), _p(out), a.numel(), _stream()), "add")
    return out


class UpsampleBilinearFn(torch.autograd.Function):

    @staticmethod
    def forward(ctx, x, H, W, align_corners):
        _require(x, "x")
        x = x.contiguous()
        N, Cc, h, w = x.shape
        y = torch.empty((N, Cc, H, W), dtype=torch.float32, device=x.device)
        check(_lib.lib().dcfp_upsample_bilinear_fwd_f32(_p(x), _p(y), N, Cc, h, w, H, W,
                                                        int(bool(align_corners)), _stream()),
              "upsample_fwd")
        ctx.cfg = (N, Cc, h, w, H, W, int(bool(align_corners)))
        return y

    @staticmethod
    def backward(ctx, dy):
        N, Cc, h, w, H, W, ac = ctx.cfg
        dy = dy.contiguous()
        dx = torch.empty((N, Cc, h, w), dtype=torch.float32, device=dy.device)
        check(_lib.lib().dcfp_upsample_bilinear_bwd_f32(_p(dy), _p(dx), N, Cc, h, w, H, W, ac, _stream()),
              "upsample_bwd")
        return dx, None, None, None


def upsample_bilinear(x, size, align_corners):
    return UpsampleBilinearFn.apply(x, int(size[0]), int(size[1]), align_corners)


def upsample_ce_forward(logits, labels, size, align_corners, ignore_index, pixel_keep=None,
                        want_gt_prob=False):
    _require(logits, "logits")
    logits = logits.contiguous()
    if labels.dtype != torch.int64 or not labels.is_cuda:
        raise RuntimeError("upsample_ce: labels must be a CUDA int64 tensor [N,H,W]")
    labels = labels.contiguous()
    N, Cc, h, w = logits.shape
    H, W = int(size[0]), int(size[1])
    if tuple(labels.shape) != (N, H, W):
        raise RuntimeError(f"upsample_ce: labels shape {tuple(labels.shape)} != {(N, H, W)}")
    L = _lib.lib()
    ws = _workspace("ce", L.dcfp_upsample_ce_workspace_bytes(N, H, W), logits.device)
    out2 = torch.empty(2, dtype=torch.float32, device=logits.device)
    lse = torch.empty((N, H, W), dtype=torch.float32, device=logits.device)
    gtp = torch.empty((N, H, W), dtype=torch.float32, device=logits.device) if want_gt_prob else None
    if pixel_keep is not None:
        pixel_keep = pixel_keep.to(torch.uint8).contiguous()
    check(L.dcfp_upsample_ce_fwd_f32(_p(logits), _p(labels), _p(pixel_keep), int(ignore_index), N, Cc,
                                     h, w, H, W, int(bool(align_corners)), _p(lse), _p(gtp), _p(out2),
                                     _p(ws), ws.numel(), _stream()), "upsample_ce_fwd")
    return out2, lse, gtp

# ... 285 lines not shown
```

### include/dcfp_hip.h

```cpp
#ifndef DCFP_HIP_H
#define DCFP_HIP_H

#include <stddef.h>
#include <stdint.h>

#ifdef __cplusplus
extern "C" {
#endif

#define DCFP_OK 0
#define DCFP_E_BADDESC (-1)
#define DCFP_E_UNSUPPORTED (-2)
#define DCFP_E_WORKSPACE (-3)

typedef void* dcfp_stream_t;

int dcfp_abi_version(void);

typedef struct DcfpConvDesc {
    int32_t N, Cin, H, W;
    int32_t Cout, KH, KW;
    int32_t stride, pad, dil;
    int32_t Hout, Wout;
    int32_t x_pitch, dy_pitch;
} DcfpConvDesc;

enum { DCFP_CONV_FWD = 0, DCFP_CONV_DGRAD = 1, DCFP_CONV_WGRAD = 2 };

size_t dcfp_conv2d_workspace_bytes(const DcfpConvDesc* d, int pass);

#define DCFP_WP_BLOCK_ELEMS 2048
typedef struct DcfpWpEntry {
    const float* w;
    float* wp;
    int64_t first_block;
    int64_t n_blocks;
    int32_t T, Ck, CkP, M, Mpad, sAm, sAc;
    int32_t perm8;
} DcfpWpEntry;
int dcfp_conv2d_wp_layout(const DcfpConvDesc* d, int pass, DcfpWpEntry* entry);
int dcfp_conv2d_permute_weights_multi_f32(const DcfpWpEntry* table, int n_entries, int64_t total_blocks,
                                          dcfp_stream_t stream);

int dcfp_conv2d_pitch_supported(const DcfpConvDesc* d);

int dcfp_conv2d_workspace_is_scratch(const DcfpConvDesc* d, int pass);

size_t dcfp_conv2d_xform_bytes(const DcfpConvDesc* d);
int dcfp_conv2d_fwd_keep_f32_nchw(const DcfpConvDesc* d, const float* x, const float* w, float* y, int64_t y_nstride,
                                  float* xform_out, size_t xform_bytes,
                                  float* stat_partials ,
                                  void* workspace, size_t workspace_bytes, dcfp_stream_t stream);
int dcfp_conv2d_wgrad_kept_f32_nchw(const DcfpConvDesc* d, const float* dy, int64_t dy_nstride, const float* xform,
                                    size_t xform_bytes, float* dw, void* workspace, size_t workspace_bytes,
                                    dcfp_stream_t stream);

int dcfp_conv2d_dgrad_fanin_supported(const DcfpConvDesc* d);
int dcfp_conv2d_dgrad_fanin_f32_nchw(const DcfpConvDesc* d, const float* dy, int64_t dy_nstride, const float* w, float* dx,
                                     const float* fan_src, const void* fan_mask, void* workspace, size_t workspace_bytes,
                                     int wp_valid, dcfp_stream_t stream);
int64_t dcfp_conv2d_dgrad_fanin_red_slots(const DcfpConvDesc* d);
int dcfp_conv2d_dgrad_fanin_red_f32_nchw(const DcfpConvDesc* d, const float* dy, int64_t dy_nstride, const float* w,
                                         float* dx, const float* fan_src, const void* fan_mask, const float* red_x,
                                         const void* red_mask, const float* red_mean, float* red_part, void* workspace,
                                         size_t workspace_bytes, int wp_valid, dcfp_stream_t stream);
int dcfp_bn_bwd_sums_from_partials_f32(const float* partials, int64_t slots, int C, const float* var, float eps,
                                       float* sum_dy, float* sum_dy_xmu, float* dgamma ,
                                       float* dbeta , dcfp_stream_t stream);

int dcfp_conv2d_kernel_name(const DcfpConvDesc* d, int pass, char* buf, int buf_len);

double dcfp_conv2d_executed_fraction(const DcfpConvDesc* d, int pass);

int dcfp_conv2d_fwd_f32_nchw(const DcfpConvDesc* d, const float* x, const float* w,
                             const float* bias, float* y, int64_t y_nstride,
                             void* workspace, size_t workspace_bytes, int wp_valid,
                             dcfp_stream_t stream);
int dcfp_conv2d_fwd_fused_f32_nchw(const DcfpConvDesc* d, const float* x, const float* w,
                                   const float* scale, const float* shift, const float* residual,
                                   int relu, float* y, void* workspace, size_t workspace_bytes,
                                   int wp_valid, dcfp_stream_t stream);
int dcfp_conv2d_dgrad_f32_nchw(const DcfpConvDesc* d, const float* dy, int64_t dy_nstride,
                               const float* w, float* dx, int accumulate,
                               void* workspace, size_t workspace_bytes, int wp_valid,
                               dcfp_stream_t stream);
int dcfp_conv2d_wgrad_f32_nchw(const DcfpConvDesc* d, const float* dy, int64_t dy_nstride,
                               const float* x, float* dw, float* db,
                               void* workspace, size_t workspace_bytes,
                               dcfp_stream_t stream);

typedef struct DcfpBnRunning {
    float* running_mean;
    float* running_var;
    int64_t* num_batches_tracked;
    float momentum;
    int32_t pad_;
} DcfpBnRunning;
size_t dcfp_bn_workspace_bytes(int N, int C, int HW);
int dcfp_bn_stats_f32(const float* x, int64_t x_nstride, int N, int C, int HW,
                      float* mean, float* var, const DcfpBnRunning* run,
                      void* workspace, size_t workspace_bytes, dcfp_stream_t stream);
int dcfp_bn_apply_f32(const float* x, const float* mean, const float* var,
                      const float* gamma, const float* beta, float eps,
                      const float* residual, int relu, float* y, int64_t y_nstride,
                      int N, int C, int HW, int W, int y_pitch, dcfp_stream_t stream);
int dcfp_bn_bwd_reduce_f32(const float* dy, int64_t dy_nstride, const float* x,
                           const float* y, int64_t y_nstride, const float* mean,
                           const float* var, const float* gamma, const float* beta, float eps,
                           int relu, int N, int C, int HW,
                           float* sum_dy, float* sum_dy_xmu, float* dgamma ,
                           float* dbeta ,
                           void* workspace, size_t workspace_bytes, dcfp_stream_t stream);
int64_t dcfp_conv2d_fwd_stat_slots(const DcfpConvDesc* d, const float* y, int64_t y_nstride);
int dcfp_conv2d_fwd_stats_f32_nchw(const DcfpConvDesc* d, const float* x, const float* w, float* y,
                                   int64_t y_nstride, float* stat_partials, void* workspace,
                                   size_t workspace_bytes, int wp_valid, dcfp_stream_t stream);
int dcfp_bn_stats_from_partials_f32(const float* partials, int64_t slots, int slot_count, int C,
                                    float* mean, float* var, const DcfpBnRunning* run , dcfp_stream_t stream);
int dcfp_syncbn_combine_f32(const float* gathered, int world, int C, float* mean, float* var,
                            float* total_count, const DcfpBnRunning* run , dcfp_stream_t stream);
#define DCFP_P2P_HANDLE_BYTES 64
size_t dcfp_syncbn_p2p_mailbox_bytes(int world, int cap_floats);
int dcfp_p2p_alloc(size_t bytes, int kind, void** ptr);
int dcfp_p2p_free(void* ptr);
int dcfp_p2p_export(void* ptr, void* handle64);
int dcfp_p2p_import(const void* handle64, void** ptr);
int dcfp_p2p_unmap(void* ptr);
int dcfp_syncbn_p2p_exchange_f32(void* const* mailboxes, int world, int rank, uint32_t seq, int cap_floats,
                                 const float* local, int n, int mode, float* out, const DcfpBnRunning* run,
                                 uint32_t spin_limit, int32_t* status, dcfp_stream_t stream);
int dcfp_bn_update_running_f32(const float* mean, const float* var, int C, float momentum,
                               float count, const float* count_dev, float* running_mean,
                               float* running_var, dcfp_stream_t stream);
int dcfp_bn_apply_relu_mask_f32(const float* x, const float* mean, const float* var,
                                const float* gamma, const float* beta, float eps,
                                const float* residual, float* y, void* relu_mask,
                                int N, int C, int HW, dcfp_stream_t stream);
int dcfp_bn_bwd_apply_f32(const float* dy, int64_t dy_nstride, const float* x,
                          const float* y, int64_t y_nstride, const float* mean,
                          const float* var, const float* gamma, const float* beta, float eps,
                          const float* sum_dy, const float* sum_dy_xmu, float count,
                          const float* count_dev,
                          int relu, float* dx, float* d_residual,
                          int N, int C, int HW, int W, int dx_pitch ,
                          dcfp_stream_t stream);

size_t dcfp_bn_bwd_fused_sync_bytes(int N, int C, int HW);
int dcfp_bn_bwd_fused_f32(const float* dy, int64_t dy_nstride, const float* x, const float* y,
                          int64_t y_nstride, const float* mean, const float* var, const float* gamma,
                          const float* beta, float eps, float count, int relu, float* dx, float* d_residual,
                          int N, int C, int HW, int W, int dx_pitch, float* sum_dy, float* sum_dy_xmu,
                          float* dgamma, float* dbeta, void* sync, size_t sync_bytes, uint32_t epoch,
                          uint32_t spin_limit, int32_t* status, dcfp_stream_t stream);

int dcfp_maxpool3x3s2_fwd_f32(const float* x, float* y, int32_t* argmax,
                              int N, int C, int H, int W, int Hout, int Wout,
                              dcfp_stream_t stream);
int dcfp_maxpool3x3s2_bwd_f32(const float* dy, const int32_t* argmax, float* dx,
                              int N, int C, int H, int W, int Hout, int Wout,
                              dcfp_stream_t stream);
int dcfp_rowsum_f32(const float* x, int64_t x_nstride, float* y, float scale,
                    int N, int C, int HW, dcfp_stream_t stream);
int dcfp_broadcast_hw_f32(const float* v, float scale, float* y, int64_t y_nstride,
                          int accumulate, int N, int C, int HW, dcfp_stream_t stream);
int dcfp_add_f32(const float* a, const float* b, float* out, int64_t n,
                 dcfp_stream_t stream);
int dcfp_channel_scale_f32(const float* x, const float* mask, float* y,
                           int N, int C, int HW, dcfp_stream_t stream);

int dcfp_upsample_bilinear_fwd_f32(const float* x, float* y, int N, int C,
                                   int h, int w, int H, int W, int align_corners,
                                   dcfp_stream_t stream);
int dcfp_upsample_bilinear_bwd_f32(const float* dy, float* dx, int N, int C,
                                   int h, int w, int H, int W, int align_corners,
                                   dcfp_stream_t stream);
int dcfp_resize_bilinear_into_f32(const float* x, int64_t x_nstride, int N, int C, int h, int w,
                                  float* y, int64_t y_nstride, int y_pitch, int H, int W,
                                  int align_corners, dcfp_stream_t stream);
int dcfp_resize_bilinear_adjoint_f32(const float* dy, int64_t dy_nstride, int dy_pitch, int N, int C, int H, int W,
                                     float* dx, int64_t dx_nstride, int h, int w, int align_corners,
                                     int accumulate, dcfp_stream_t stream);
int dcfp_ppm_pool_f32(const float* x, int N, int C, int H, int W, int nlev, const int* level_hw,
                      float* out, int mean, float* dst, int64_t dst_nstride, int dst_pitch,
                      dcfp_stream_t stream);
int dcfp_ppm_pool_adjoint_f32(const float* dp, int N, int C, int H, int W, int nlev, const int* level_hw,
                              const float* g, int64_t g_nstride, int g_pitch, float* dx, dcfp_stream_t stream);
int dcfp_ppm_resize_adjoint_f32(const float* g, int64_t g_nstride, int g_pitch, int N, int H, int W,
                                int nlev, const int* level_chw, float* dp, int align_corners,
                                dcfp_stream_t stream);
size_t dcfp_upsample_ce_workspace_bytes(int N, int H, int W);
int dcfp_upsample_ce_fwd_f32(const float* logits, const int64_t* labels,
                             const uint8_t* pixel_keep, int ignore_index,
                             int N, int C, int h, int w, int H, int W, int align_corners,
                             float* lse, float* gt_prob, float* out2,
                             void* workspace, size_t workspace_bytes,
                             dcfp_stream_t stream);
int dcfp_upsample_ce_bwd_f32(const float* logits, const int64_t* labels,
                             const uint8_t* pixel_keep, int ignore_index,
                             int N, int C, int h, int w, int H, int W, int align_corners,
                             const float* lse, const float* grad_scale ,
                             float* dlogits, dcfp_stream_t stream);

int dcfp_ohem_zoom_gt_prob_f32(const float* logits, const int64_t* labels, const float* lse,
                               int N, int C, int h, int w, int H, int W, int align_corners,
                               int H8, int W8, float* pred8, int32_t* lab8,
                               dcfp_stream_t stream);

int dcfp_ohem_threshold_f32(const float* pred8, const int32_t* lab8, int64_t n, int ignore_label,
                            float thresh, int64_t min_kept, float* threshold ,
                            dcfp_stream_t stream);
int dcfp_ohem_keep_mask_u8(const float* gt_prob, const float* threshold , int64_t n,
                           uint8_t* keep, dcfp_stream_t stream);

int dcfp_upsample_margin_f32(const float* logits, int N, int C, int h, int w, int H, int W,
                             int align_corners, float* margin, dcfp_stream_t stream);
int dcfp_maxfilter2d_s1_f32(const float* x, float* y, int planes, int H, int W, int k,
                            dcfp_stream_t stream);
size_t dcfp_upsample_wce_workspace_bytes(int N, int H, int W);
int dcfp_upsample_wce_fwd_f32(const float* logits, const int64_t* labels, const float* pix_weight,
                              int ignore_index, int N, int C, int h, int w, int H, int W,
                              int align_corners, float* lse, float* out_per_image,
                              void* workspace, size_t workspace_bytes, dcfp_stream_t stream);
int dcfp_upsample_wce_bwd_f32(const float* logits, const int64_t* labels, const float* pix_weight,
                              int ignore_index, int N, int C, int h, int w, int H, int W,
                              int align_corners, const float* lse,
                              const float* grad_scale_per_image, float* dlogits,
                              dcfp_stream_t stream);

int dcfp_upsample_argmax_f32(const float* logits, int N, int C, int h, int w, int H, int W,
                             int align_corners, int32_t* pred, dcfp_stream_t stream);
int dcfp_confusion_matrix_i64(const int32_t* pred, const int64_t* gt, int ignore_index,
                              int64_t n_pixels, int C, int64_t* conf ,
                              dcfp_stream_t stream);

size_t dcfp_label_boundary_workspace_bytes(int N, int H, int W);
int dcfp_label_boundary_i32(const int32_t* labels, int32_t* out, int N, int H, int W, int num_classes, int d,
                            int background, void* workspace, size_t workspace_bytes, dcfp_stream_t stream);
int dcfp_label_boundary_i64(const int64_t* labels, int64_t* out, int N, int H, int W, int num_classes, int d,
                            int background, void* workspace, size_t workspace_bytes, dcfp_stream_t stream);

#define DCFP_AUG_SATURATION 1
#define DCFP_AUG_HUE 2
typedef struct DcfpAugTap {
    int32_t src, c0, c1, lsrc;
} DcfpAugTap;
typedef struct DcfpAugSample {
    const uint8_t* image;
    const uint8_t* label;
    int32_t src_h, src_w;
    int32_t col_off, row_off;
    int32_t lut_a_off;
    int32_t lut_b_off;
    int32_t hsv_flags;
    int32_t hue_delta;
    float sat_alpha;
    int32_t pad_;
} DcfpAugSample;
int dcfp_augment_u8_to_f32_nchw(const DcfpAugSample* samples, int N, int crop_h, int crop_w, const DcfpAugTap* taps,
                                int64_t n_taps, const uint8_t* lut_a, int64_t lut_a_bytes, const float* lut_b,
                                int64_t lut_b_floats, const uint8_t* id_table, int ignore_label, float* images,
                                int64_t* labels, int32_t* hist, dcfp_stream_t stream);
int dcfp_balance_weight_f32(const int64_t* labels, const int32_t* hist, const int32_t* target_class, int N,
                            int64_t pixels, int num_classes, int ignore_label, int balance, double beta, float* weight,
                            dcfp_stream_t stream);

typedef struct DcfpCcSample {
    const uint8_t* label;
    int32_t src_h, src_w;
    int32_t dst_h, dst_w;
    int32_t Hp, Wp;
    int32_t row_off, col_off;
    int32_t cls;
    int32_t pad_;
    int64_t work_off;
} DcfpCcSample;
size_t dcfp_components_workspace_bytes(int Hp, int Wp);
int dcfp_label_components_u8(const DcfpCcSample* samples, int N, const int32_t* maps, int64_t n_maps,
                             const uint8_t* id_table, void* work, size_t work_bytes, int32_t* counts,
                             dcfp_stream_t stream);
int dcfp_component_pixel_i32(const DcfpCcSample* samples, int N, void* work, size_t work_bytes, const int32_t* counts,
                             const int32_t* n, const int32_t* k, int32_t* yx, dcfp_stream_t stream);

typedef struct DcfpEicEntry {
    const float* gamma;
    const float* grad;
    float* eic;
    int32_t n;
    int32_t pad_;
} DcfpEicEntry;
int dcfp_eic_update_f32(const DcfpEicEntry* table, int n_layers, float r,
                        float one_minus_r ,
                        dcfp_stream_t stream);

typedef struct DcfpSgdEntry {
    float* param;
    const float* grad;
    float* momentum_buf;
    int64_t n;
    int64_t first_chunk;
    float weight_decay;
    int32_t pad_;
} DcfpSgdEntry;
#define DCFP_SGD_CHUNK 16384
int dcfp_sgd_momentum_f32(const DcfpSgdEntry* table, int n_tensors, int64_t total_chunks,
                          float lr, float momentum, int first_step, dcfp_stream_t stream);

typedef struct DcfpConvF16Desc {
    int32_t N, H, W;
    int32_t Cin8, x_pitch;
    int32_t Cout;
    int32_t K, stride, pad, dil;
    int32_t Hout, Wout;
    int32_t y_pitch, y_off;
// ... 27 lines not shown
```

Before: 12.24 images/s.

## Fuse stem BN+ReLU+maxpool, cache wgrad tables, tile weight permutation through LDS

Adds a fused kernel for the stem that applies BN and ReLU, then does the 3x3 stride-2 maxpool without writing the full-resolution activation. Backward recomputes through the saved argmax and the normal BN backward. Caches a precomputed per-shape table for fused Winograd wgrad so it is not rebuilt on every call. Rewrites weight permutation and Winograd filter transform to stage tiles in LDS for coalesced writes. Costs extra code paths and a host-side table cache keyed by shape and stream.

```diff
diff --git a/dcfp_amd/_lib.py b/dcfp_amd/_lib.py
--- a/dcfp_amd/_lib.py
+++ b/dcfp_amd/_lib.py
@@ -93,6 +93,9 @@
     "dcfp_conv2d_fwd_fused_f32_nchw": (_I, [_D, _P, _P, _P, _P, _P, _I, _P, _P, _Z, _I, _P]),
     "dcfp_conv2d_dgrad_f32_nchw": (_I, [_D, _P, _L, _P, _P, _I, _P, _Z, _I, _P]),
     "dcfp_conv2d_wgrad_f32_nchw": (_I, [_D, _P, _L, _P, _P, _P, _P, _Z, _P]),
+    "dcfp_conv2d_wgrad_table_bytes": (_Z, [_D, _L]),
+    "dcfp_conv2d_wgrad_table_build": (_I, [_D, _L, _P, _Z, _P]),
+    "dcfp_conv2d_wgrad_table_f32_nchw": (_I, [_D, _P, _L, _P, _P, _P, _P, _Z, _P, _Z, _P]),
     "dcfp_bn_workspace_bytes": (_Z, [_I, _I, _I]),
     "dcfp_bn_stats_f32": (_I, [_P, _L, _I, _I, _I, _P, _P, _R, _P, _Z, _P]),
     "dcfp_bn_apply_f32": (_I, [_P, _P, _P, _P, _P, _F, _P, _I, _P, _L, _I, _I, _I, _I, _I, _P]),
@@ -119,6 +122,7 @@
                                    _P, _P, _P, _P, _P, _Z, C.c_uint32, C.c_uint32, _P, _P]),
     "dcfp_maxpool3x3s2_fwd_f32": (_I, [_P, _P, _P, _I, _I, _I, _I, _I, _I, _P]),
     "dcfp_maxpool3x3s2_bwd_f32": (_I, [_P, _P, _P, _I, _I, _I, _I, _I, _I, _P]),
+    "dcfp_bn_relu_maxpool3x3s2_f32": (_I, [_P, _P, _P, _P, _P, _F, _P, _P, _I, _I, _I, _I, _I, _I, _P]),
     "dcfp_rowsum_f32": (_I, [_P, _L, _P, _F, _I, _I, _I, _P]),
     "dcfp_broadcast_hw_f32": (_I, [_P, _F, _P, _L, _I, _I, _I, _I, _P]),
     "dcfp_add_f32": (_I, [_P, _P, _P, _L, _P]),
diff --git a/dcfp_amd/csrc/bn.hip b/dcfp_amd/csrc/bn.hip
--- a/dcfp_amd/csrc/bn.hip
+++ b/dcfp_amd/csrc/bn.hip
@@ -1,5 +1,6 @@
 #include "common.h"
 #include <stdlib.h>
+#include <math.h>
 
 namespace {
 
@@ -165,6 +166,92 @@
             else yr[i] = o;
         }
     }
+}
+
+__device__ __forceinline__ float bn_relu_val(float v, float mu, float istd, float g, float b) {
+    const float o = bn_val(v, mu, istd, g, b);
+    return o > 0.f ? o : 0.f;
+}
+
+__global__ void __launch_bounds__(kThreads)
+bn_relu_maxpool_kernel(const float* __restrict__ x, const float* __restrict__ mean, const float* __restrict__ var,
+                       const float* __restrict__ gamma, const float* __restrict__ beta, float eps,
+                       float* __restrict__ y, int32_t* __restrict__ argmax, long long total, int C, int H, int W,
+                       int Hout, int Wout) {
+    for (long long idx = (long long)blockIdx.x * kThreads + threadIdx.x; idx < total;
+         idx += (long long)gridDim.x * kThreads) {
+        const int ow = (int)(idx % Wout);
+        const long long t = idx / Wout;
+        const int oh = (int)(t % Hout);
+        const long long plane = t / Hout;
+        const int c = (int)(plane % C);
+        const float istd = 1.0f / sqrtf(var[c] + eps);
+        const float mu = mean[c], g = gamma[c], b = beta[c];
+        const float* xp = x + plane * (long long)H * W;
+        const int h0 = oh * 2 - 1, w0 = ow * 2 - 1;
+        const int hs = h0 < 0 ? 0 : h0, ws = w0 < 0 ? 0 : w0;
+        const int he = h0 + 3 > H ? H : h0 + 3, we = w0 + 3 > W ? W : w0 + 3;
+        float best = -INFINITY;
+        int bi = hs * W + ws;
+        for (int h = hs; h < he; ++h) {
+            for (int w = ws; w < we; ++w) {
+                const float v = bn_relu_val(xp[h * W + w], mu, istd, g, b);
+                if (v > best || v != v) {
+                    best = v;
+                    bi = h * W + w;
+                }
+            }
+        }
+        y[idx] = best;
+        argmax[idx] = bi;
+    }
+}
+
+__global__ void __launch_bounds__(kThreads)
+bn_relu_maxpool_vec4_kernel(const float* __restrict__ x, const float* __restrict__ mean, const float* __restrict__ var,
+                            const float* __restrict__ gamma, const float* __restrict__ beta, float eps,
+                            float* __restrict__ y, int32_t* __restrict__ argmax, int C, int H, int W, int Hout, int Wout,
+                            int segs) {
+    const long long rowid = blockIdx.x / segs;
+    const int seg = blockIdx.x - (int)(rowid * segs);
+    const long long plane = rowid / Hout;
+    const int oh = (int)(rowid - plane * Hout);
+    const int ow0 = 4 * (seg * kThreads + threadIdx.x);
+    if (ow0 >= Wout) return;
+    const int c = (int)(plane % C);
+    const float istd = 1.0f / sqrtf(var[c] + eps);
+    const float mu = mean[c], g = gamma[c], b = beta[c];
+    const float* xp = x + plane * (long long)H * W;
+    const int h0 = 2 * oh - 1, c0 = 2 * ow0;
+    float best[4] = {-INFINITY, -INFINITY, -INFINITY, -INFINITY};
+    const int hs = h0 < 0 ? 0 : h0;
+    int bi[4];
+#pragma unroll
+    for (int j = 0; j < 4; ++j) bi[j] = hs * W + ((c0 + 2 * j - 1) < 0 ? 0 : (c0 + 2 * j - 1));
+#pragma unroll
+    for (int r = 0; r < 3; ++r) {
+        const int h = h0 + r;
+        if (h < 0 || h >= H) continue;
+        const float* row = xp + (long long)h * W;
+        const float4 a = *reinterpret_cast<const float4*>(row + c0);
+        const float4 q = *reinterpret_cast<const float4*>(row + c0 + 4);
+        const float raw[9] = {c0 > 0 ? row[c0 - 1] : 0.f, a.x, a.y, a.z, a.w, q.x, q.y, q.z, q.w};
+        float v[9];
+#pragma unroll
+        for (int k = 0; k < 9; ++k) v[k] = bn_relu_val(raw[k], mu, istd, g, b);
+#pragma unroll
+        for (int j = 0; j < 4; ++j) {
+#pragma unroll
+            for (int k = 0; k < 3; ++k) {
+                if (k == 0 && j == 0 && c0 == 0) continue;
+                const float t = v[2 * j + k];
+                if (t > best[j] || t != t) { best[j] = t; bi[j] = h * W + c0 + 2 * j + k - 1; }
+            }
+        }
+    }
+    const long long o = rowid * Wout + ow0;
+    *reinterpret_cast<float4*>(y + o) = make_float4(best[0], best[1], best[2], best[3]);
+    *reinterpret_cast<int4*>(argmax + o) = make_int4(bi[0], bi[1], bi[2], bi[3]);
 }
 
 template <bool VEC, int RELU>
@@ -778,6 +865,28 @@
     DCFP_RETURN_LAUNCH();
 }
 
+extern "C" int dcfp_bn_relu_maxpool3x3s2_f32(const float* x, const float* mean, const float* var, const float* gamma,
+                                             const float* beta, float eps, float* y, int32_t* argmax, int N, int C,
+                                             int H, int W, int Hout, int Wout, dcfp_stream_t stream) {
+    if (!x || !mean || !var || !gamma || !beta || !y || !argmax || N <= 0 || C <= 0 || H <= 0 || W <= 0)
+        return DCFP_E_BADDESC;
+    if (Hout != (H + 2 - 3) / 2 + 1 || Wout != (W + 2 - 3) / 2 + 1) return DCFP_E_BADDESC;
+    if ((long long)H * W > 0x7fffffffLL) return DCFP_E_UNSUPPORTED;
+    const long long total = (long long)N * C * Hout * Wout;
+    const long long orows = (long long)N * C * Hout;
+    const int segs = (Wout / 4 + kThreads - 1) / kThreads;
+    if (W % 8 == 0 && dcfp_aligned16(x) && dcfp_aligned16(y) && dcfp_aligned16(argmax) && orows * segs <= 0x7fffffffLL)
+        hipLaunchKernelGGL(bn_relu_maxpool_vec4_kernel, dim3((unsigned)(orows * segs)), dim3(kThreads), 0, dcfp_s(stream),
+                           x, mean, var, gamma, beta, eps, y, argmax, C, H, W, Hout, Wout, segs);
+    else {
+        long long blocks = (total + kThreads - 1) / kThreads;
+        if (blocks > 256 * 16) blocks = 256 * 16;
+        hipLaunchKernelGGL(bn_relu_maxpool_kernel, dim3((unsigned)blocks), dim3(kThreads), 0, dcfp_s(stream), x, mean, var,
+                           gamma, beta, eps, y, argmax, total, C, H, W, Hout, Wout);
+    }
+    DCFP_RETURN_LAUNCH();
+}
+
 extern "C" int dcfp_bn_apply_relu_mask_f32(const float* x, const float* mean, const float* var,
                                            const float* gamma, const float* beta, float eps,
                                            const float* residual, float* y, void* relu_mask,
diff --git a/dcfp_amd/csrc/conv_igemm2.hip b/dcfp_amd/csrc/conv_igemm2.hip
--- a/dcfp_amd/csrc/conv_igemm2.hip
+++ b/dcfp_amd/csrc/conv_igemm2.hip
@@ -29,8 +29,105 @@
 }
 
 constexpr int kWpBlockElems = DCFP_WP_BLOCK_ELEMS;
+constexpr int kWpTM = 32;
+constexpr int kWpRow = kWpTM + 1;
+constexpr int kWpTapSkew = 8;
+constexpr int kWinoRow = 73;
+constexpr int kWpLdsFloats = 64 * kWinoRow + 8192;
+
+template <int T, int TC>
+__device__ __forceinline__ void permute_tiles(const DcfpWpEntry& e, int lb, float* __restrict__ lds) {
+    constexpr int TS = TC * kWpRow + kWpTapSkew;
+    constexpr int ELEMS = kWpTM * TC * T;
+    static_assert(T * TS <= kWpLdsFloats, "LDS image of a tile");
+    const int mt = (e.Mpad + kWpTM - 1) / kWpTM, ct = (e.CkP + TC - 1) / TC;
+    const int units = mt * ct;
+    const bool along_c = e.sAc <= e.sAm;
+    for (int unit = lb; unit < units; unit += (int)e.n_blocks) {
+        const int ci = unit / mt, mi = unit - ci * mt;
+        const int c0 = ci * TC, p0 = mi * kWpTM;
+        for (int i = threadIdx.x; i < ELEMS; i += 256) {
+            int ml, cl, t;
+            if (along_c) {
+                ml = i / (TC * T);
+                const int j = i - ml * (TC * T);
+                cl = j / T; t = j - cl * T;
+            } else {
+                cl = i / (kWpTM * T);
+                const int j = i - cl * (kWpTM * T);
+                ml = j / T; t = j - ml * T;
+            }
+            const int m = wp_row(p0 + ml, e.perm8), c = c0 + cl;
+            float v = 0.f;
+            if (m < e.M && c < e.Ck && p0 + ml < e.Mpad) v = e.w[(long long)m * e.sAm + (long long)c * e.sAc + t];
+            lds[t * TS + cl * kWpRow + ml] = v;
+        }
+        __syncthreads();
+        for (int i = threadIdx.x; i < ELEMS; i += 256) {
+            const int ml = i % kWpTM, r = i / kWpTM;
+            const int cl = r % TC, t = r / TC;
+            if (p0 + ml < e.Mpad && c0 + cl < e.CkP)
+                e.wp[((long long)t * e.CkP + (c0 + cl)) * e.Mpad + (p0 + ml)] = lds[t * TS + cl * kWpRow + ml];
+        }
+        __syncthreads();
+    }
+}
+
+__device__ __forceinline__ void wino_filter2_chunks(const DcfpWpEntry& e, int lb, float* __restrict__ lds) {
+    float* raw = lds;
+    float* chunk = lds + 64 * kWinoRow;
+    const int mblocks = e.Mpad / 64;
+    const int units = (e.CkP / 8) * mblocks;
+    const bool along_c = e.sAc <= e.sAm;
+    const bool flip = e.perm8 == 3;
+    const bool vec = (reinterpret_cast<uintptr_t>(e.wp) & 15u) == 0;
+    for (int unit = lb; unit < units; unit += (int)e.n_blocks) {
+        const int cb = unit / mblocks, mb = unit - cb * mblocks;
+        const int c0 = cb * 8, m0 = mb * 64;
+        for (int i = threadIdx.x; i < 64 * 72; i += 256) {
+            int ml, cl, t;
+            if (along_c) {
+                ml = i / 72;
+                const int j = i - ml * 72;
+                cl = j / 9; t = j - cl * 9;
+            } else {
+                cl = i / 576;
+                const int j = i - cl * 576;
+                ml = j / 9; t = j - ml * 9;
+            }
+            const int m = m0 + ml, c = c0 + cl;
+            float v = 0.f;
+            if (m < e.M && c < e.Ck) v = e.w[(long long)m * e.sAm + (long long)c * e.sAc + t];
+            raw[ml * kWinoRow + cl * 9 + t] = v;
+        }
+        __syncthreads();
+#pragma unroll
+        for (int k = 0; k < 2; ++k) {
+            const int q = threadIdx.x + 256 * k, ml = q & 63, cl = q >> 6;
+            const float* src = raw + ml * kWinoRow + cl * 9;
+            float g[9], u[16];
+#pragma unroll
+            for (int t = 0; t < 9; ++t) g[t] = src[flip ? 8 - t : t];
+            wino_filter2_transform(g, u);
+            float* dst = chunk + wino_filter2_chunk_offset(cl, ml);
+#pragma unroll
+            for (int xi = 0; xi < 16; ++xi) dst[xi * 512] = u[xi];
+        }
+        __syncthreads();
+        float* out = e.wp + (long long)unit * 8192;
+        if (vec) {
+            for (int i = threadIdx.x; i < 2048; i += 256)
+                reinterpret_cast<f32x4*>(out)[i] = reinterpret_cast<const f32x4*>(chunk)[i];
+        } else {
+            for (int i = threadIdx.x; i < 8192; i += 256) out[i] = chunk[i];
+        }
+        __syncthreads();
+    }
+}
+
 __global__ void __launch_bounds__(256)
 permute_weights_multi_kernel(const DcfpWpEntry* __restrict__ table, int n) {
+    __shared__ __attribute__((aligned(16))) float lds[kWpLdsFloats];
     const long long blk = blockIdx.x;
     int lo = 0, hi = n - 1;
     while (lo < hi) {
@@ -38,29 +135,24 @@
         if (table[mid].first_block <= blk) lo = mid; else hi = mid - 1;
     }
     const DcfpWpEntry e = table[lo];
-    const long long base = (blk - e.first_block) * kWpBlockElems;
-    if (e.perm8 >= 2) {
-        const long long pairs = (long long)e.CkP * e.Mpad;
-#pragma unroll 1
-        for (int u = 0; u < kWpBlockElems / 256; ++u) {
-            const long long i = base + u * 256 + threadIdx.x;
-            if (i >= pairs) return;
-            wino_filter2_pair(e.w, e.sAm, e.sAc, e.perm8 == 3, e.M, e.Ck, e.Mpad, i, e.wp);
-        }
-        return;
-    }
-    const long long total = (long long)e.T * e.CkP * e.Mpad;
-#pragma unroll
-    for (int u = 0; u < kWpBlockElems / 256; ++u) {
-        const long long i = base + u * 256 + threadIdx.x;
-        if (i >= total) return;
-        const int m = wp_row((int)(i % e.Mpad), e.perm8);
-        const long long r = i / e.Mpad;
-        const int c = (int)(r % e.CkP);
-        const int t = (int)(r / e.CkP);
-        float v = 0.f;
-        if (m < e.M && c < e.Ck) v = e.w[(long long)m * e.sAm + (long long)c * e.sAc + t];
-        e.wp[i] = v;
+    if (blk - e.first_block >= e.n_blocks) return;
+    const int lb = (int)(blk - e.first_block);
+    if (e.perm8 >= 2)
+        wino_filter2_chunks(e, lb, lds);
+    else if (e.T == 1)
+        permute_tiles<1, 64>(e, lb, lds);
+    else if (e.T == 9)
+        permute_tiles<9, 16>(e, lb, lds);
+    else {
+        const long long total = (long long)e.T * e.CkP * e.Mpad;
+        for (long long i = (long long)lb * kWpBlockElems + threadIdx.x; i < total && i < ((long long)lb + 1) * kWpBlockElems; i += 256) {
+            const int m = wp_row((int)(i % e.Mpad), e.perm8);
+            const long long r = i / e.Mpad;
+            const int c = (int)(r % e.CkP), t = (int)(r / e.CkP);
+            float v = 0.f;
+            if (m < e.M && c < e.Ck) v = e.w[(long long)m * e.sAm + (long long)c * e.sAc + t];
+            e.wp[i] = v;
+        }
     }
 }
 
diff --git a/dcfp_amd/csrc/conv_wgrad.hip b/dcfp_amd/csrc/conv_wgrad.hip
--- a/dcfp_amd/csrc/conv_wgrad.hip
+++ b/dcfp_amd/csrc/conv_wgrad.hip
@@ -944,9 +944,12 @@
 bool dcfp_wino_wgrad_fused_ok(int N, int H, int W, int d, int M, int C, long long x_nstride, int x_pitch,
                               long long dy_nstride, int dy_pitch);
 size_t dcfp_wino_wgrad_fused_workspace_bytes(int N, int H, int W, int d, int M, int C);
+size_t dcfp_wino_wgrad_fused_table_bytes(int N, int H, int W, int d, int M, int C);
+int dcfp_wino_wgrad_fused_table_build(int N, int H, int W, int d, int M, int C, long long x_nstride, int x_pitch,
+                                      long long dy_nstride, int dy_pitch, void* table, size_t table_bytes, hipStream_t stream);
 int dcfp_wino_wgrad_fused_run(const float* dy, long long dy_nstride, int dy_pitch, const float* x, long long x_nstride,
                               int x_pitch, float* dw, int N, int M, int C, int H, int W, int d, void* workspace,
-                              size_t workspace_bytes, hipStream_t stream);
+                              size_t workspace_bytes, hipStream_t stream, const void* kept_table, size_t kept_table_bytes);
 
 static int wino_wgrad_kind(const DcfpConvDesc* d) {
     static const int mode = [] { const char* e = getenv("DCFP_CONV_WINOGRAD"); return e ? atoi(e) : 1; }();
@@ -1011,10 +1014,52 @@
     return (size_t)pl.splits * d->Cout * d->Cin * d->KH * d->KW * sizeof(float);
 }
 
+static int wino_wgrad_kind_real(const DcfpConvDesc* d, int64_t dy_nstride) {
+    int wk = wino_wgrad_kind(d);
+    if (wk == 2) {
+        const int dyp = d->dy_pitch ? d->dy_pitch : d->Wout, xp = d->x_pitch ? d->x_pitch : d->W;
+        const long long dyn = dy_nstride ? dy_nstride : (long long)d->Cout * d->Hout * dyp;
+        if (!dcfp_wino_wgrad_fused_ok(d->N, d->H, d->W, d->dil, d->Cout, d->Cin, (long long)d->Cin * d->H * xp, xp, dyn, dyp))
+            wk = dcfp_wino_wgrad_ok(d->N, d->H, d->W, d->dil, d->Cout, d->Cin) ? 1 : 0;
+    }
+    return wk;
+}
+
+extern "C" size_t dcfp_conv2d_wgrad_table_bytes(const DcfpConvDesc* d, int64_t dy_nstride) {
+    if (check_desc(d) != DCFP_OK || wino_wgrad_kind_real(d, dy_nstride) != 2) return 0;
+    return dcfp_wino_wgrad_fused_table_bytes(d->N, d->H, d->W, d->dil, d->Cout, d->Cin);
+}
+
+extern "C" int dcfp_conv2d_wgrad_table_build(const DcfpConvDesc* d, int64_t dy_nstride, void* table, size_t table_bytes,
+                                             dcfp_stream_t stream) {
+    const int rc = check_desc(d);
+    if (rc) return rc;
+    if (wino_wgrad_kind_real(d, dy_nstride) != 2) return DCFP_E_UNSUPPORTED;
+    const int dyp = d->dy_pitch ? d->dy_pitch : d->Wout, xp = d->x_pitch ? d->x_pitch : d->W;
+    const long long dyn = dy_nstride ? dy_nstride : (long long)d->Cout * d->Hout * dyp;
+    return dcfp_wino_wgrad_fused_table_build(d->N, d->H, d->W, d->dil, d->Cout, d->Cin, (long long)d->Cin * d->H * xp, xp, dyn,
+                                             dyp, table, table_bytes, dcfp_s(stream));
+}
+
+static int wgrad_run(const DcfpConvDesc* d, const float* dy, int64_t dy_nstride, const float* x, float* dw, float* db,
+                     const void* table, size_t table_bytes, void* workspace, size_t workspace_bytes, dcfp_stream_t stream);
+
 extern "C" int dcfp_conv2d_wgrad_f32_nchw(const DcfpConvDesc* d, const float* dy,
                                           int64_t dy_nstride, const float* x, float* dw, float* db,
                                           void* workspace, size_t workspace_bytes,
                                           dcfp_stream_t stream) {
+    return wgrad_run(d, dy, dy_nstride, x, dw, db, nullptr, 0, workspace, workspace_bytes, stream);
+}
+
+extern "C" int dcfp_conv2d_wgrad_table_f32_nchw(const DcfpConvDesc* d, const float* dy, int64_t dy_nstride, const float* x,
+                                                float* dw, float* db, const void* table, size_t table_bytes,
+                                                void* workspace, size_t workspace_bytes, dcfp_stream_t stream) {
+    if (!table) return DCFP_E_BADDESC;
+    return wgrad_run(d, dy, dy_nstride, x, dw, db, table, table_bytes, workspace, workspace_bytes, stream);
+}
+
+static int wgrad_run(const DcfpConvDesc* d, const float* dy, int64_t dy_nstride, const float* x, float* dw, float* db,
+                     const void* table, size_t table_bytes, void* workspace, size_t workspace_bytes, dcfp_stream_t stream) {
     int rc = check_desc(d);
     if (rc) return rc;
     if (!dy || !x || !dw) return DCFP_E_BADDESC;
@@ -1022,20 +1067,15 @@
         return dcfp_gemv_wgrad(d, dy, dy_nstride, x, dw, dcfp_s(stream));
     if (dcfp_stem_shape(d) && !db)
         return dcfp_stem_wgrad(d, dy, dy_nstride, x, dw, workspace, workspace_bytes, dcfp_s(stream));
-    int wk = wino_wgrad_kind(d);
-    if (wk == 2) {
-        const int dyp = d->dy_pitch ? d->dy_pitch : d->Wout, xp = d->x_pitch ? d->x_pitch : d->W;
-        const long long dyn = dy_nstride ? dy_nstride : (long long)d->Cout * d->Hout * dyp;
-        if (!dcfp_wino_wgrad_fused_ok(d->N, d->H, d->W, d->dil, d->Cout, d->Cin, (long long)d->Cin * d->H * xp, xp, dyn, dyp))
-            wk = dcfp_wino_wgrad_ok(d->N, d->H, d->W, d->dil, d->Cout, d->Cin) ? 1 : 0;
-    }
+    const int wk = wino_wgrad_kind_real(d, dy_nstride);
+    if (table && wk != 2) return DCFP_E_UNSUPPORTED;
     if (wk) {
         const int dyp = d->dy_pitch ? d->dy_pitch : d->Wout, xp = d->x_pitch ? d->x_pitch : d->W;
         const long long dyn = dy_nstride ? dy_nstride : (long long)d->Cout * d->Hout * dyp;
         if (db && dyp != d->Wout) return DCFP_E_UNSUPPORTED;
         if (wk == 2) {
             rc = dcfp_wino_wgrad_fused_run(dy, dyn, dyp, x, (long long)d->Cin * d->H * xp, xp, dw, d->N, d->Cout, d->Cin, d->H,
-                                           d->W, d->dil, workspace, workspace_bytes, dcfp_s(stream));
+                                           d->W, d->dil, workspace, workspace_bytes, dcfp_s(stream), table, table_bytes);
         } else
             rc = dcfp_wino_wgrad_run(dy, dyn, dyp, x, (long long)d->Cin * d->H * xp, xp, dw, d->N, d->Cout, d->Cin, d->H, d->W,
                                      d->dil, workspace, workspace_bytes, dcfp_s(stream));
diff --git a/dcfp_amd/csrc/conv_winograd3.hip b/dcfp_amd/csrc/conv_winograd3.hip
--- a/dcfp_amd/csrc/conv_winograd3.hip
+++ b/dcfp_amd/csrc/conv_winograd3.hip
@@ -417,9 +417,29 @@
     return (size_t)(pl.table_floats + pl.slab_floats) * sizeof(float);
 }
 
+size_t dcfp_wino_wgrad_fused_table_bytes(int N, int H, int W, int d, int M, int C) {
+    return (size_t)wg_plan(N, H, W, d, M, C).table_floats * sizeof(float);
+}
+
+int dcfp_wino_wgrad_fused_table_build(int N, int H, int W, int d, int M, int C, long long x_nstride, int x_pitch,
+                                      long long dy_nstride, int dy_pitch, void* table, size_t table_bytes, hipStream_t stream) {
+    if (x_pitch <= 0) x_pitch = W;
+    if (dy_pitch <= 0) dy_pitch = W;
+    const int mode = wg_mode(N, H, W, d, M, C, x_nstride, x_pitch, dy_nstride, dy_pitch);
+    if (mode < 0) return DCFP_E_UNSUPPORTED;
+    const WgPlan pl = wg_plan(N, H, W, d, M, C);
+    if (!table || !dcfp_aligned16(table) || table_bytes < (size_t)pl.table_floats * sizeof(float)) return DCFP_E_WORKSPACE;
+    const int lead = mode == 4 ? 0 : 4;
+    const long long npairs = pl.T16 / 2;
+    hipLaunchKernelGGL(wino_wg_table_kernel, dim3((unsigned)((npairs + 255) / 256)), dim3(256), 0, stream,
+                       static_cast<unsigned*>(table), npairs, pl.T, N, H, W, d, pl.TH, pl.TW, x_nstride, x_pitch, lead,
+                       dy_nstride, dy_pitch, mode);
+    DCFP_RETURN_LAUNCH();
+}
+
 int dcfp_wino_wgrad_fused_run(const float* dy, long long dy_nstride, int dy_pitch, const float* x, long long x_nstride,
                               int x_pitch, float* dw, int N, int M, int C, int H, int W, int d, void* workspace,
-                              size_t workspace_bytes, hipStream_t stream) {
+                              size_t workspace_bytes, hipStream_t stream, const void* kept_table, size_t kept_table_bytes) {
     if (x_pitch <= 0) x_pitch = W;
     if (dy_pitch <= 0) dy_pitch = W;
     const int mode = wg_mode(N, H, W, d, M, C, x_nstride, x_pitch, dy_nstride, dy_pitch);
@@ -427,12 +447,17 @@
     const WgPlan pl = wg_plan(N, H, W, d, M, C);
     if (!workspace || !dcfp_aligned16(workspace) || workspace_bytes < dcfp_wino_wgrad_fused_workspace_bytes(N, H, W, d, M, C))
         return DCFP_E_WORKSPACE;
-    unsigned* table = static_cast<unsigned*>(workspace);
+    if (kept_table && (!dcfp_aligned16(kept_table) || kept_table_bytes < (size_t)pl.table_floats * sizeof(float)))
+        return DCFP_E_WORKSPACE;
+    const unsigned* table = kept_table ? static_cast<const unsigned*>(kept_table) : static_cast<const unsigned*>(workspace);
     float* slabs = static_cast<float*>(workspace) + pl.table_floats;
     const int lead = mode == 4 ? 0 : 4;
     const long long npairs = pl.T16 / 2;
-    hipLaunchKernelGGL(wino_wg_table_kernel, dim3((unsigned)((npairs + 255) / 256)), dim3(256), 0, stream, table, npairs, pl.T,
-                       N, H, W, d, pl.TH, pl.TW, x_nstride, x_pitch, lead, dy_nstride, dy_pitch, mode);
+    if (!kept_table) {
+        const int rc = dcfp_wino_wgrad_fused_table_build(N, H, W, d, M, C, x_nstride, x_pitch, dy_nstride, dy_pitch, workspace,
+                                                         (size_t)pl.table_floats * sizeof(float), stream);
+        if (rc) return rc;
+    }
     WinoWgParams p;
     p.x_base = x - lead;
     p.x_bytes = (unsigned)(((long long)(N - 1) * x_nstride + (long long)C * H * x_pitch + lead) * 4);
diff --git a/dcfp_amd/csrc/igemm2_common.h b/dcfp_amd/csrc/igemm2_common.h
--- a/dcfp_amd/csrc/igemm2_common.h
+++ b/dcfp_amd/csrc/igemm2_common.h
@@ -48,6 +48,30 @@
     }
 }
 
+__device__ __forceinline__ void wino_filter2_transform(const float (&g)[9], float (&u)[16]) {
+    float r[4][3];
+#pragma unroll
+    for (int k = 0; k < 3; ++k) {
+        const float g0 = g[k], g1 = g[3 + k], g2 = g[6 + k];
+        r[0][k] = g0;
+        r[1][k] = 0.5f * ((g0 + g2) + g1);
+        r[2][k] = 0.5f * ((g0 + g2) - g1);
+        r[3][k] = g2;
+    }
+#pragma unroll
+    for (int i = 0; i < 4; ++i) {
+        const float a = r[i][0], b = r[i][1], cc = r[i][2];
+        u[4 * i + 0] = a;
+        u[4 * i + 1] = 0.5f * ((a + cc) + b);
+        u[4 * i + 2] = 0.5f * ((a + cc) - b);
+        u[4 * i + 3] = cc;
+    }
+}
+
+__device__ __forceinline__ int wino_filter2_chunk_offset(int cl, int ml) {
+    return ((ml >> 5) * 64 + (cl & 1) * 32 + (ml & 31)) * 4 + (cl >> 1);
+}
+
 __device__ __forceinline__ void wino_filter2_pair(const float* __restrict__ w, int sAm, int sAc, int flip, int M, int Ck,
                                                   int Mpad, long long idx, float* __restrict__ Ug) {
     const int mblocks = Mpad / 64;
@@ -61,25 +85,12 @@
 #pragma unroll
         for (int t = 0; t < 9; ++t) g[t] = 0.f;
     }
-    float r[4][3];
+    float u[16];
+    wino_filter2_transform(g, u);
+    const int cb = c >> 3, mb = m >> 6;
+    float* dst = Ug + (long long)(cb * mblocks + mb) * 8192 + wino_filter2_chunk_offset(c & 7, m & 63);
 #pragma unroll
-    for (int k = 0; k < 3; ++k) {
-        const float g0 = g[k], g1 = g[3 + k], g2 = g[6 + k];
-        r[0][k] = g0;
-        r[1][k] = 0.5f * ((g0 + g2) + g1);
-        r[2][k] = 0.5f * ((g0 + g2) - g1);
-        r[3][k] = g2;
-    }
-    const int cb = c >> 3, cl = c & 7, mb = m >> 6, ml = m & 63;
-    float* dst = Ug + ((((long long)(cb * mblocks + mb) * 16) * 2 + (ml >> 5)) * 64 + (cl & 1) * 32 + (ml & 31)) * 4 + (cl >> 1);
-#pragma unroll
-    for (int i = 0; i < 4; ++i) {
-        const float a = r[i][0], b = r[i][1], cc = r[i][2];
-        dst[(4 * i + 0) * 512] = a;
-        dst[(4 * i + 1) * 512] = 0.5f * ((a + cc) + b);
-        dst[(4 * i + 2) * 512] = 0.5f * ((a + cc) - b);
-        dst[(4 * i + 3) * 512] = cc;
-    }
+    for (int xi = 0; xi < 16; ++xi) dst[xi * 512] = u[xi];
 }
 
 template <int T>
diff --git a/dcfp_amd/networks/_exec.py b/dcfp_amd/networks/_exec.py
--- a/dcfp_amd/networks/_exec.py
+++ b/dcfp_amd/networks/_exec.py
@@ -81,6 +81,21 @@
     return bn_act(bn, conv(cm, x), relu=relu, residual=residual, prev_conv=cm, next_conv=next_conv)
 
 
+def conv_bn_relu_pool(cm, bn, x):
+    if (not bn.training) and bn.running_mean is not None and not torch.is_grad_enabled():
+        return ops.maxpool3x3s2(conv_bn_act(cm, bn, x, relu=True))
+    y = conv(cm, x)
+    if not (y.is_cuda and y.dim() == 4):
+        return ops.maxpool3x3s2(bn_act(bn, y, relu=True, prev_conv=cm))
+    rm, rv, training, momentum, eps, sync, nbt = _bn_args(bn)
+    pitch_cfg = None
+    if torch.is_grad_enabled() and y.requires_grad and cm.kernel_size == (3, 3):
+        dx_pitch = _conv_pitch(cm, (y.shape[0], cm.in_channels, y.shape[2], y.shape[3]))
+        if dx_pitch:
+            pitch_cfg = (bn, 0, dx_pitch)
+    return ops.batch_norm_relu_maxpool3x3s2(y, bn.weight, bn.bias, rm, rv, training, momentum, eps, sync, nbt, pitch_cfg)
+
+
 def _plain_conv(m, k):
     ok = (m.groups == 1 and m.bias is None and m.kernel_size == (k, k) and m.padding_mode == "zeros"
           and not isinstance(m.padding, str))
diff --git a/dcfp_amd/networks/backbone/resnet.py b/dcfp_amd/networks/backbone/resnet.py
--- a/dcfp_amd/networks/backbone/resnet.py
+++ b/dcfp_amd/networks/backbone/resnet.py
@@ -75,8 +75,7 @@
         _exec.require_device(input)
         stem = list(self.conv1.children())
         x = _exec.run_sequential(nn.Sequential(*stem[:-1]), input, tail_conv=stem[-1])
-        x = _exec.conv_bn_act(stem[-1], self.bn1, x, relu=True)
-        x = ops.maxpool3x3s2(x)
+        x = _exec.conv_bn_relu_pool(stem[-1], self.bn1, x)
         outs = []
         for i in range(1, 5):
             for blk in getattr(self, "layer" + str(i)):
diff --git a/dcfp_amd/ops.py b/dcfp_amd/ops.py
--- a/dcfp_amd/ops.py
+++ b/dcfp_amd/ops.py
@@ -413,6 +413,25 @@
     return s[0], s[1], dgamma
 
 
+_WG_TABLES = {}
+
+
+def _wgrad_table(d, ns, device):
+    L = _lib.lib()
+    nbytes = L.dcfp_conv2d_wgrad_table_bytes(C.byref(d), ns)
+    if not nbytes:
+        return None
+    key = tuple(getattr(d, f[0]) for f in ConvDesc._fields_) + (int(ns), device.index, torch.cuda.current_stream().cuda_stream)
+    t = _WG_TABLES.get(key)
+    if t is None:
+        if len(_WG_TABLES) > 256:
+            _WG_TABLES.clear()
+        t = torch.empty(int(nbytes), dtype=torch.uint8, device=device)
+        check(L.dcfp_conv2d_wgrad_table_build(C.byref(d), ns, _p(t), t.numel(), _stream()), "conv2d_wgrad_table_build")
+        _WG_TABLES[key] = t
+    return t
+
+
 def conv2d_wgrad(dy, x, wshape, stride, pad, dil, need_bias=False, dw=None, db=None, xform=None):
     _require(dy, "dy"); _require(x, "x")
     xp, dp = _pitch_of(x), _pitch_of(dy)
@@ -437,6 +456,12 @@
             L.dcfp_conv2d_wgrad_kept_f32_nchw(C.byref(d), _p(dy), ns, _p(xform), xform.numel(), _p(dw), _p(ws), ws.numel(),
                                               _stream()), "conv2d_wgrad_kept"))
         return dw, None
+    table = _wgrad_table(d, ns, x.device)
+    if table is not None:
+        _timed("conv_wgrad", d, _conv_flops(d), lambda: check(
+            L.dcfp_conv2d_wgrad_table_f32_nchw(C.byref(d), _p(dy), ns, _p(x), _p(dw), _p(db) if need_bias else None,
+                                               _p(table), table.numel(), _p(ws), ws.numel(), _stream()), "conv2d_wgrad_table"))
+        return dw, (db if need_bias else None)
     _timed("conv_wgrad", d, _conv_flops(d), lambda: check(
         L.dcfp_conv2d_wgrad_f32_nchw(C.byref(d), _p(dy), ns, _p(x), _p(dw), _p(db) if need_bias else None, _p(ws),
                                      ws.numel(), _stream()), "conv2d_wgrad"))
@@ -744,6 +769,16 @@
                     momentum, eps, sync, nbt=None, stats=None, want_mask=False, out=None):
     _require(x, "x")
     x = x.contiguous()
+    mean, var, count, group = _bn_forward_stats(x, running_mean, running_var, training, momentum, sync, nbt, stats)
+    if want_mask and relu and residual is not None and BN_RELU_BITMASK and out is None:
+        ym = bn_apply_relu_mask(x, mean, var, gamma, beta, eps, residual)
+        if ym is not None:
+            return ym[0], (mean, var, count, group, ym[1])
+    y = bn_apply(x, mean, var, gamma, beta, eps, residual, relu, out=out)
+    return y, (mean, var, count, group)
+
+
+def _bn_forward_stats(x, running_mean, running_var, training, momentum, sync, nbt=None, stats=None):
     N, Cc, H, W = x.shape
     count = float(N * H * W)
     group = _sync_group(sync) if training else None
@@ -769,12 +804,7 @@
                 nbt.add_(1)
     else:
         mean, var = running_mean, running_var
-    if want_mask and relu and residual is not None and BN_RELU_BITMASK and out is None:
-        ym = bn_apply_relu_mask(x, mean, var, gamma, beta, eps, residual)
-        if ym is not None:
-            return ym[0], (mean, var, count, group, ym[1])
-    y = bn_apply(x, mean, var, gamma, beta, eps, residual, relu, out=out)
-    return y, (mean, var, count, group)
+    return mean, var, count, group
 
 
 def _bn_bwd_preface(relu, y, state, gamma, beta, gparam, bparam):
@@ -1398,6 +1428,50 @@
     return MaxPool3x3s2Fn.apply(x)
 
 
+class BatchNormReluMaxPoolFn(torch.autograd.Function):
+
+    @staticmethod
+    def forward(ctx, x, gamma, beta, running_mean, running_var, training, momentum, eps, sync, nbt, pitch_cfg):
+        _require(x, "x")
+        x = x.contiguous()
+        ctx.dx_pitch, ctx.dx_key = 0, "bn_dx"
+        if pitch_cfg is not None:
+            ctx.dx_pitch, ctx.dx_key = pitch_cfg[2], ("bn_dx", id(pitch_cfg[0]))
+        mean, var, count, group = _bn_forward_stats(x, running_mean, running_var, training, momentum, sync, nbt)
+        N, Cc, H, W = x.shape
+        Ho, Wo = (H + 2 - 3) // 2 + 1, (W + 2 - 3) // 2 + 1
+        y = torch.empty((N, Cc, Ho, Wo), dtype=torch.float32, device=x.device)
+        idx = torch.empty((N, Cc, Ho, Wo), dtype=torch.int32, device=x.device)
+        _timed("bn_apply", None, 4.0 * x.numel() + 8.0 * y.numel(), lambda: check(
+            _lib.lib().dcfp_bn_relu_maxpool3x3s2_f32(_p(x), _p(mean), _p(var), _p(gamma), _p(beta), float(eps), _p(y), _p(idx),
+                                                     N, Cc, H, W, Ho, Wo, _stream()), "bn_relu_maxpool"))
+        flat, ctx.meta = _pack_bn_states([(mean, var, count, group)])
+        ctx.save_for_backward(x, idx, *flat)
+        ctx.params = (gamma, beta)
+        ctx.cfg = (training, eps, (N, Cc, H, W, Ho, Wo))
+        return y
+
+    @staticmethod
+    def backward(ctx, dy):
+        x, idx = ctx.saved_tensors[:2]
+        gamma, beta = ctx.params
+        training, eps, (N, Cc, H, W, Ho, Wo) = ctx.cfg
+        state = _bn_state(ctx.meta, ctx.saved_tensors[2:], 0)
+        dy = dy.contiguous()
+        dact = torch.empty((N, Cc, H, W), dtype=torch.float32, device=dy.device)
+        check(_lib.lib().dcfp_maxpool3x3s2_bwd_f32(_p(dy), _p(idx), _p(dact), N, Cc, H, W, Ho, Wo, _stream()),
+              "maxpool_bwd")
+        dx_out = pitched_buffer(tuple(x.shape), ctx.dx_pitch, ctx.dx_key, x.device) if ctx.dx_pitch else None
+        dx, dgamma, dbeta, _ = bn_backward_impl(dact, x, None, gamma, beta, state, True, training, eps, False, dx_out=dx_out)
+        return dx, dgamma, dbeta, None, None, None, None, None, None, None, None
+
+
+def batch_norm_relu_maxpool3x3s2(x, gamma, beta, running_mean, running_var, training=True, momentum=0.1, eps=1e-5,
+                                 sync=False, nbt=None, pitch_cfg=None):
+    return BatchNormReluMaxPoolFn.apply(x, gamma, beta, running_mean, running_var, training, momentum, eps, sync, nbt,
+                                        pitch_cfg)
+
+
 def rowsum(x, scale):
     N, Cc, H, W = x.shape
     x, ns = _batch_strided(x)
diff --git a/include/dcfp_hip.h b/include/dcfp_hip.h
--- a/include/dcfp_hip.h
+++ b/include/dcfp_hip.h
@@ -88,6 +88,12 @@
                                const float* x, float* dw, float* db,
                                void* workspace, size_t workspace_bytes,
                                dcfp_stream_t stream);
+size_t dcfp_conv2d_wgrad_table_bytes(const DcfpConvDesc* d, int64_t dy_nstride);
+int dcfp_conv2d_wgrad_table_build(const DcfpConvDesc* d, int64_t dy_nstride, void* table, size_t table_bytes,
+                                  dcfp_stream_t stream);
+int dcfp_conv2d_wgrad_table_f32_nchw(const DcfpConvDesc* d, const float* dy, int64_t dy_nstride, const float* x,
+                                     float* dw, float* db, const void* table, size_t table_bytes,
+                                     void* workspace, size_t workspace_bytes, dcfp_stream_t stream);
 
 typedef struct DcfpBnRunning {
     float* running_mean;
@@ -159,6 +165,9 @@
 int dcfp_maxpool3x3s2_bwd_f32(const float* dy, const int32_t* argmax, float* dx,
                               int N, int C, int H, int W, int Hout, int Wout,
                               dcfp_stream_t stream);
+int dcfp_bn_relu_maxpool3x3s2_f32(const float* x, const float* mean, const float* var, const float* gamma,
+                                  const float* beta, float eps, float* y, int32_t* argmax,
+                                  int N, int C, int H, int W, int Hout, int Wout, dcfp_stream_t stream);
 int dcfp_rowsum_f32(const float* x, int64_t x_nstride, float* y, float scale,
                     int N, int C, int HW, dcfp_stream_t stream);
 int dcfp_broadcast_hw_f32(const float* v, float scale, float* y, int64_t y_nstride,
```

After: 12.24 images/s (median of 2 runs). About the same (+0.0%).
